# Boese0601/RC-MVSNet

Measured on AMD Instinct MI355X. Metric: ref-scenes/sec (DTU 3-view 512x640, D=48/32/8), higher is better.
Workload: dtype f32; 1 GPU; BASELINE configs[1]: CascadeMVSNet_eval.forward, DTU-shaped 3 views 512x640, D=(48,32,8), batch 1 per GPU, fp32, random-init seeded weights; views=3, height=512, width=640, parallelism=scene-per-gpu x1, ranks=1, procs_per_gpu=1, rccl_ranks=0

## Files before the change

rc_mvsnet_amd/_lib.py:

```python
import ast
import ctypes
import os
import re
import subprocess

_HERE = os.path.dirname(os.path.abspath(__file__))
LIB_PATH = os.path.join(_HERE, "librcmvs_hip.so")
CSRC = os.path.join(_HERE, "csrc")
HEADER = os.path.join(os.path.dirname(_HERE), "include", "rcmvs.h")
EXT_HEADERS = (os.path.join(CSRC, "pc_register.h"), os.path.join(CSRC, "view_select.h"), os.path.join(CSRC, "undistort.h"),
               os.path.join(CSRC, "tsdf_mesh.h"), os.path.join(CSRC, "tsdf_sparse.h"), os.path.join(CSRC, "mesh_clean.h"),
               os.path.join(CSRC, "mesh_decimate.h"), os.path.join(CSRC, "mesh_holes.h"),
               os.path.join(CSRC, "mesh_render.h"))

_lib = None


class RcmvsError(RuntimeError):
    pass


_CTYPES = {"int": ctypes.c_int, "float": ctypes.c_float, "double": ctypes.c_double, "long long": ctypes.c_longlong}


def _const_expr(text):
    def ev(node):
        if isinstance(node, ast.Constant) and type(node.value) is int:
            return node.value
        if isinstance(node, ast.BinOp) and isinstance(node.op, ast.LShift):
            return ev(node.left) << ev(node.right)
        raise ValueError(text)
    return ev(ast.parse(text.strip(), mode="eval").body)


def _ctype(decl, what, c_type):
    if c_type not in _CTYPES:
        raise RcmvsError(f"{HEADER}: `{decl}`: {what} type `{c_type}` is outside the ABI's types ({', '.join(_CTYPES)}, pointers)")
    return _CTYPES[c_type]


def parse_header(text):
    text = re.sub(r"/\*.*?\*/|//[^\n]*", " ", text, flags=re.S)
    signatures, restypes, constants, code = {}, {}, {}, []
    for line in text.splitlines():
        if not line.lstrip().startswith("#"):
            code.append(line)
            continue
        m = re.match(r"\s*#\s*define\s+(RCMVS_\w+)\s+(\S.*)", line)
        if m:
            try:
                value = _const_expr(m.group(2))
            except (ValueError, SyntaxError):
                raise RcmvsError(f"{HEADER}: `{line.strip()}`: not an integer expression of literals, << and parentheses") from None
            if m.group(1) in constants:
                raise RcmvsError(f"{HEADER}: {m.group(1)} is defined twice")
            constants[m.group(1)] = value
    for decl in re.sub(r'extern\s+"C"\s*\{', " ", "\n".join(code)).split(";"):
        decl = " ".join(decl.split())
        if "rcmvs_" not in decl:
            continue
        m = re.fullmatch(r"([\w\s*]+?)\s*\b(rcmvs_\w+)\s*\(([^()]*)\)", decl)
        if not m:
            raise RcmvsError(f"{HEADER}: `{decl}` is not a complete `<type> rcmvs_name(<parameters>);` declaration")
        ret, name, params = m.group(1), m.group(2), m.group(3).strip()
        if name in signatures:
            raise RcmvsError(f"{HEADER}: {name} is declared twice")
        if ret.replace("const", "").replace(" ", "") == "char*":
            restypes[name] = ctypes.c_char_p
        elif ret != "int":
            restypes[name] = _ctype(decl, "return", ret)
        argtypes = []
        for param in ([] if params == "void" else params.split(",")):
            if "*" in param:
                argtypes.append(ctypes.c_void_p)
                continue
            words = [w for w in param.split() if w != "const"]
            if len(words) < 2 or not words[-1].isidentifier():
                raise RcmvsError(f"{HEADER}: `{decl}`: parameter `{param.strip()}` is not `<type> <name>`")
            argtypes.append(_ctype(decl, "parameter", " ".join(words[:-1])))
        signatures[name] = argtypes
    return signatures, restypes, constants


def _read_header():
    try:
        with open(HEADER) as f:
            return f.read()
    except FileNotFoundError:
        raise RcmvsError(f"{HEADER} is missing: the ctypes binding is derived from the C header, which was expected there "
                         "(include/rcmvs.h next to the rc_mvsnet_amd package)") from None


SIGNATURES, _RESTYPES, CONSTANTS = parse_header(_read_header())
REQUIRED_VERSION = CONSTANTS["RCMVS_VERSION"]


def _read_extensions():
    signatures, restypes = {}, {}
    for path in EXT_HEADERS:
        try:
            with open(path) as f:
                sig, res, const = parse_header(f.read())
        except FileNotFoundError:
            raise RcmvsError(f"{path} is missing: the binding of its entry points is derived from it") from None
        for table, add in ((signatures, sig), (CONSTANTS, const)):
            clash = [k for k in add if k in table or k in SIGNATURES]
            if clash:
                raise RcmvsError(f"{path}: {clash[0]} is already declared")
            table.update(add)
        restypes.update(res)
    return signatures, restypes


EXT_SIGNATURES, _EXT_RESTYPES = _read_extensions()


def sources():
    return sorted(os.path.join(CSRC, f) for f in os.listdir(CSRC) if f.endswith(".hip"))


def build(force=False, verbose=False):
    from concurrent.futures import ThreadPoolExecutor
    srcs = sources()
    hdrs = [os.path.join(CSRC, f) for f in os.listdir(CSRC) if f.endswith(".h")] + [HEADER]
    if not force and os.path.exists(LIB_PATH) and all(os.path.getmtime(LIB_PATH) >= os.path.getmtime(d) for d in srcs + hdrs):
        return LIB_PATH
    hipcc = os.environ.get("HIPCC", "/opt/rocm/bin/hipcc")
    objdir = os.path.join(_HERE, "_obj")
    os.makedirs(objdir, exist_ok=True)
    hdr_time = max(os.path.getmtime(h) for h in hdrs)
    jobs, objs = [], []
    for src in srcs:
        obj = os.path.join(objdir, os.path.basename(src)[:-4] + ".o")
        objs.append(obj)
        if force or not os.path.exists(obj) or os.path.getmtime(obj) < max(os.path.getmtime(src), hdr_time):
            jobs.append([hipcc, "--offload-arch=gfx950", "-O3", "-std=c++17", "-fPIC", "-c", src, "-o", obj])

    def run(cmd):
        if verbose:
            print(" ".join(cmd), flush=True)
        subprocess.run(cmd, check=True)

    with ThreadPoolExecutor(max_workers=min(8, os.cpu_count() or 1)) as ex:
        list(ex.map(run, jobs))
    run([hipcc, "--offload-arch=gfx950", "-shared", "-fPIC", "-o", LIB_PATH] + objs)
    return LIB_PATH


def bind(lib):
    for table, restypes in ((SIGNATURES, _RESTYPES), (EXT_SIGNATURES, _EXT_RESTYPES)):
        for name, argtypes in table.items():
            fn = getattr(lib, name)
            fn.argtypes = argtypes
            fn.restype = restypes.get(name, ctypes.c_int)


def load():
    global _lib
    if _lib is not None:
        return _lib
    path = os.environ.get("RCMVS_LIB") or LIB_PATH
    if not os.path.exists(path):
        raise RcmvsError(f"{path} is missing: run `python -c 'import __graft_entry__ as g; g.build()'` "
                         "(hipcc --offload-arch=gfx950). There is no CPU / eager fallback.")
    lib = ctypes.CDLL(path)
    bind(lib)
    if lib.rcmvs_version() < REQUIRED_VERSION:
        raise RcmvsError(f"librcmvs_hip.so (version {lib.rcmvs_version()}) is older than this package needs ({REQUIRED_VERSION}): rebuild it")
    _lib = lib
    return lib


def check(rc, what):
    if rc != 0:
        msg = load().rcmvs_last_error_string()
        raise RcmvsError(f"{what} failed (rc={rc}): {msg.decode() if msg else ''}")


def call(name, *args):
    rc = getattr(_lib or load(), name)(*args)
    if rc:
        check(rc, name[len("rcmvs_"):])
```

rc_mvsnet_amd/casmvsnet.py:

```python
import os

FP16_PAIR_DEFAULT = True
ONE_BY_ONE_MFMA = os.environ.get("RCMVS_1X1_MFMA", "1") != "0"
HEAD_PAIR = os.environ.get("RCMVS_HEAD_PAIR", "1") != "0"
CONV11_PROB = int(os.environ.get("RCMVS_CONV11_PROB", "1"))
CONV_TILE = os.environ.get("RCMVS_CONV_TILE", "1") != "0"
CONV_STEM = os.environ.get("RCMVS_CONV_STEM", "1") != "0"
CONV_PAIR = os.environ.get("RCMVS_CONV_PAIR", "1") != "0"
DEEP_PAIR = os.environ.get("RCMVS_DEEP_PAIR", "1") != "0"

import torch
import torch.nn as nn
import torch.nn.functional as F

from . import ops
from ._lib import RcmvsError


def _nhwc(x):
    x = x.contiguous().float()
    return ops.rgb_to_nhwc4(x) if x.shape[1] == 3 else ops.to_channels_last(x)


def _param(mod, name):
    p = mod._parameters.get(name)
    return p if p is not None else getattr(mod, name)


def _packed_of(module, make):
    w = module.conv.weight
    key = (w.data_ptr(), w._version, str(w.device))
    c = module.__dict__.get("_rcmvs_pack")
    if c is None or c[0] != key:
        c = module.__dict__["_rcmvs_pack"] = (key, make(w.detach()))
    return c[1]


def _affine_of(m):
    if getattr(m, "gn", None) is not None:
        raise RcmvsError(f"{type(m).__name__}: GroupNorm blocks are not provided (the reference builds every block with norm='batch_norm')")
    if m.bn is not None:
        return _bn_fold(m.bn)
    b = m.conv.bias
    if b is None:
        return None, None
    return torch.ones_like(b, dtype=torch.float32), b.detach().float().contiguous()


def _same2(v, n):
    return tuple(v) == (n, n)


def _conv2d_block_cl(m, t):
    conv = m.conv
    K = conv.kernel_size[0]
    st = conv.stride[0]
    if (not _same2(conv.kernel_size, K) or K not in (1, 3, 5) or not _same2(conv.padding, K // 2) or not _same2(conv.stride, st)
            or st not in (1, 2) or not _same2(conv.dilation, 1) or conv.groups != 1 or conv.padding_mode != "zeros"):
        raise RcmvsError(f"Conv2d: only square 1x1 / 3x3 / 5x5 kernels with 'same' zero padding, stride 1 or 2, no dilation or groups "
                         f"(the layers of models/modules.py) run on the HIP path; got {conv}")
    scale, shift = _affine_of(m)
    relu = bool(m.relu)
    if K == 5 or conv.in_channels == 3:
        pw = _packed_of(m, lambda w: ops.pack_conv2d_weight(w, pad_in_to=4 if w.shape[1] == 3 else None))
        return ops.conv2d(t, pw, scale, shift, stride=st, relu=relu)
    pw = _packed_of(m, lambda w: ops.pack_conv3d_weight(FeatureNet._w3(w)))
    return ops.conv3d(t.unsqueeze(1), pw, scale, shift, stride=st, relu=relu).squeeze(1)


def _deconv2d_block_cl(m, t):
    conv = m.conv
    if (not _same2(conv.kernel_size, 3) or not _same2(conv.stride, 2) or not _same2(conv.padding, 1) or not _same2(conv.output_padding, 1)
            or not _same2(conv.dilation, 1) or conv.groups != 1):
        raise RcmvsError(f"Deconv2d: only kernel 3, stride 2, padding 1, output_padding 1 (DeConv2dFuse, models/modules.py:346) runs on the "
                         f"HIP path; got {conv}")
    if m.bn is None:
        raise RcmvsError("Deconv2d: bn=False is not provided (the reference's forward returns its INPUT in that case, models/modules.py:106-110)")
    scale, shift = _bn_fold(m.bn)
    pw = _packed_of(m, lambda w: ops.pack_conv3d_weight(F.pad(w.unsqueeze(2), (0, 0, 0, 0, 1, 1)), transposed=True))
    return ops.deconv3d(t.unsqueeze(1), pw, scale, shift, relu=bool(m.relu))[:, 0]


class Conv2d(nn.Module):
    def __init__(self, in_channels, out_channels, kernel_size, stride=1, relu=True, bn=True, bn_momentum=0.1,
                 init_method="xavier", **kwargs):
        super().__init__()
        self.conv = nn.Conv2d(in_channels, out_channels, kernel_size, stride=stride, bias=(not bn), **kwargs)
        self.kernel_size = kernel_size
        self.stride = stride
        self.bn = nn.BatchNorm2d(out_channels, momentum=bn_momentum) if bn else None
        self.relu = relu

    def forward(self, x):
        if _hip_inference(self, x):
            return ops.to_channels_first(_conv2d_block_cl(self, _nhwc(x)).contiguous())
        _unsupported(self, x)


class Deconv2d(nn.Module):

    def __init__(self, in_channels, out_channels, kernel_size, stride=1, relu=True, bn=True, bn_momentum=0.1,
                 init_method="xavier", **kwargs):
        super().__init__()
        assert stride in [1, 2]
        self.out_channels = out_channels
        self.stride = stride
        self.conv = nn.ConvTranspose2d(in_channels, out_channels, kernel_size, stride=stride, bias=(not bn), **kwargs)
        self.bn = nn.BatchNorm2d(out_channels, momentum=bn_momentum) if bn else None
        self.relu = relu

    def forward(self, x):
        if _hip_inference(self, x):
            return ops.to_channels_first(_deconv2d_block_cl(self, _nhwc(x)).contiguous())
        _unsupported(self, x)


class DeConv2dFuse(nn.Module):

    def __init__(self, in_channels, out_channels, kernel_size, relu=True, bn=True, bn_momentum=0.1):
        super().__init__()
        self.deconv = Deconv2d(in_channels, out_channels, kernel_size, stride=2, padding=1, output_padding=1, bn=True, relu=relu,
                               bn_momentum=bn_momentum)
        self.conv = Conv2d(2 * out_channels, out_channels, kernel_size, stride=1, padding=1, bn=bn, relu=relu, bn_momentum=bn_momentum)

    def forward_cl(self, x_pre, x):
        up = _deconv2d_block_cl(self.deconv, x)
        if up.shape != x_pre.shape:
            raise RcmvsError(f"DeConv2dFuse: the skip map {tuple(x_pre.shape)} is not twice the size of the up-sampled one {tuple(up.shape)}")
        return _conv2d_block_cl(self.conv, torch.cat((up, x_pre), dim=-1))

    def forward(self, x_pre, x):
        if _hip_inference(self, x_pre, x):
            return ops.to_channels_first(self.forward_cl(_nhwc(x_pre), _nhwc(x)).contiguous())
        _unsupported(self, x_pre, x)


class FeatureNet(nn.Module):

    def __init__(self, base_channels, num_stage=3, stride=4, arch_mode="fpn"):
        super().__init__()
        if arch_mode not in ("unet", "fpn"):
            raise ValueError("mode must be in 'unet' or 'fpn', but get:{}".format(arch_mode))
        if num_stage not in (1, 2, 3):
            raise ValueError("num_stage must be 1, 2 or 3")
        self.arch_mode = arch_mode
        self.stride = stride
        self.base_channels = base_channels
        self.num_stage = num_stage
        b = base_channels
        self.conv0 = nn.Sequential(Conv2d(3, b, 3, 1, padding=1), Conv2d(b, b, 3, 1, padding=1))
        self.conv1 = nn.Sequential(Conv2d(b, b * 2, 5, stride=2, padding=2), Conv2d(b * 2, b * 2, 3, 1, padding=1),
                                   Conv2d(b * 2, b * 2, 3, 1, padding=1))
        self.conv2 = nn.Sequential(Conv2d(b * 2, b * 4, 5, stride=2, padding=2), Conv2d(b * 4, b * 4, 3, 1, padding=1),
                                   Conv2d(b * 4, b * 4, 3, 1, padding=1))
        self.out1 = nn.Conv2d(b * 4, b * 4, 1, bias=False)
        self.out_channels = [4 * b]
        final_chs = b * 4
        if arch_mode == "unet":
            if num_stage >= 2:
                self.deconv1 = DeConv2dFuse(b * 4, b * 2, 3)
                self.out2 = nn.Conv2d(b * 2, b * 2, 1, bias=False)
                self.out_channels.append(2 * b)
            if num_stage == 3:
                self.deconv2 = DeConv2dFuse(b * 2, b, 3)
                self.out3 = nn.Conv2d(b, b, 1, bias=False)
                self.out_channels.append(b)
        elif num_stage == 3:
            self.inner1 = nn.Conv2d(b * 2, final_chs, 1, bias=True)
            self.inner2 = nn.Conv2d(b * 1, final_chs, 1, bias=True)
            self.out2 = nn.Conv2d(final_chs, b * 2, 3, padding=1, bias=False)
            self.out3 = nn.Conv2d(final_chs, b, 3, padding=1, bias=False)
            self.out_channels += [b * 2, b]
        elif num_stage == 2:
            self.inner1 = nn.Conv2d(b * 2, final_chs, 1, bias=True)
            self.out2 = nn.Conv2d(final_chs, b, 3, padding=1, bias=False)
            self.out_channels.append(b)

    def hip_plan(self):
        sub = self._modules
        mods = [m for seq in ("conv0", "conv1", "conv2") for m in sub[seq]._modules.values()]
        tens = []
        for m in mods:
            cv, bn = m._modules["conv"], m._modules["bn"]
            bb = bn._buffers
            tens += [_param(cv, "weight"), _param(bn, "weight"), _param(bn, "bias"), bb["running_mean"], bb["running_var"], bb["num_batches_tracked"]]
        unet = self.arch_mode == "unet"
        heads = ["out1"] + (["out2", "out3"] if unet else ["inner1", "out2", "inner2", "out3"])
        extra = [t for n in heads if n in sub for t in (_param(sub[n], "weight"), getattr(sub[n], "bias", None)) if t is not None]
        key = tuple((t.data_ptr(), t._version) for t in tens + extra)
        if getattr(self, "_plan", None) is None or key != self._plan_key:
            plan = {}
            names = ["conv0.0", "conv0.1", "conv1.0", "conv1.1", "conv1.2", "conv2.0", "conv2.1", "conv2.2"]
            for n, m in zip(names, mods):
                pad_to = 4 if m.conv.in_channels == 3 else None
                w = m.conv.weight
                if tuple(w.shape) in ((8, 8, 3, 3), (16, 16, 3, 3), (32, 32, 3, 3)) and m.stride == 1:
                    w3 = w.detach().new_zeros(w.shape[0], w.shape[1], 3, 3, 3)
                    w3[:, :, 1] = w.detach()
                    plan[n] = ("mfma3d", ops.pack_conv3d_weight(w3)) + _bn_fold(m.bn)
                    continue
                if tuple(w.shape) in ((32, 16, 5, 5), (16, 8, 5, 5)) and m.stride == 2:
                    w3 = self._w3(self._w5s2(w.detach())).contiguous()
                    plan[n] = ("s2d_mfma3d", ops.pack_conv3d_weight(w3)) + _bn_fold(m.bn)
                    continue
                plan[n] = (ops.pack_conv2d_weight(w, pad_in_to=pad_to),) + _bn_fold(m.bn) + (m.stride,)
            m11, m12 = mods[3], mods[4]
            if CONV_PAIR and all(tuple(m.conv.weight.shape) == (16, 16, 3, 3) and m.stride == 1 for m in (m11, m12)):
                plan["pair1"] = (ops.pack_conv2d_pair(m11.conv.weight, m12.conv.weight),) + _bn_fold(m11.bn) + _bn_fold(m12.bn)
            m00, m01 = mods[0], mods[1]
            if CONV_STEM and tuple(m00.conv.weight.shape) == (8, 3, 3, 3) and tuple(m01.conv.weight.shape) == (8, 8, 3, 3) and m00.stride == 1 and m01.stride == 1:
                plan["stem"] = (plan["conv0.0"][0],) + _bn_fold(m00.bn) + (ops.pack_conv2d_stem(m01.conv.weight),) + _bn_fold(m01.bn)
            m10 = mods[2]
            if CONV_TILE and tuple(m10.conv.weight.shape) == (16, 8, 5, 5) and m10.stride == 2:
                plan["tile10"] = (ops.pack_conv2d_tile(self._w5s2(m10.conv.weight.detach()).contiguous()),) + _bn_fold(m10.bn)
            for n, m in (("conv2.1", mods[6]), ("conv2.2", mods[7])):
                if CONV_TILE and tuple(m.conv.weight.shape) == (32, 32, 3, 3) and m.stride == 1:
                    plan["tile:" + n] = (ops.pack_conv2d_tile(m.conv.weight),) + _bn_fold(m.bn)
            plan["out1"] = ops.pack_conv2d_weight(self.out1.weight)
            if unet:
                for n in ("out2", "out3")[:self.num_stage - 1]:
                    plan[n] = ops.pack_conv3d_weight(self._w3(getattr(self, n).weight.detach()))
            elif self.num_stage >= 2:
                plan["inner1"] = (ops.pack_conv2d_weight(self.inner1.weight), self.inner1.bias.detach().float().contiguous())
                if tuple(self.out2.weight.shape) == (16, 32, 3, 3):
                    w3 = self.out2.weight.detach().new_zeros(16, 32, 3, 3, 3)
                    w3[:, :, 1] = self.out2.weight.detach()
                    plan["out2"] = ("mfma3d", ops.pack_conv3d_weight(w3))
                    if CONV_TILE:
                        plan["out2t"] = ops.pack_conv2d_tile(self.out2.weight)
                else:
                    plan["out2"] = ops.pack_conv2d_weight(self.out2.weight)
            if self.num_stage == 3 and not unet:
                plan["inner2"] = (ops.pack_conv2d_weight(self.inner2.weight), self.inner2.bias.detach().float().contiguous())
                plan["out3"] = ops.pack_conv2d_weight(self.out3.weight)
                plan["fuse_out3"] = tuple(self.inner2.weight.shape[:2]) == (32, 8) and tuple(self.out3.weight.shape[:2]) == (8, 32)
                if plan["fuse_out3"]:
                    plan["fold_out3"] = ops.pack_fpn_folded(self.inner2.weight, self.inner2.bias, self.out3.weight)
                    if os.environ.get("RCMVS_FPN_MFMA", "1") != "0":
                        plan["fold_out3"] = ops.pack_fpn_folded_mfma(plan["fold_out3"])
            self._plan, self._plan_key = plan, key
        return self._plan

    def forward_cl(self, x, lazy=False):
        p = self.hip_plan()

        def cbr(t, n):
            if "tile:" + n in p and not ops._CONV_IMPL:
                img, sc, sh = p["tile:" + n]
                return ops.conv2d_tile(t, img, sc, sh, relu=True)
            if p[n][0] == "mfma3d":
                _, w3, sc, sh = p[n]
                return ops.conv3d(t.unsqueeze(1), w3, sc, sh, relu=True).squeeze(1)
            if p[n][0] == "s2d_mfma3d":
                if t.shape[1] % 2 or t.shape[2] % 2:
                    raise RcmvsError(f"FeatureNet: image height and width must be multiples of 4 (got a {t.shape[1]}x{t.shape[2]} map "
                                     "at the second stride-2 layer), as the reference's three-level pyramid requires")
                _, w3, sc, sh = p[n]
                if ops._CONV_IMPL:
                    return ops.conv3d(self._s2d(t).contiguous().unsqueeze(1), w3, sc, sh, relu=True).squeeze(1)
                return ops.conv2d_s2d(t, w3, sc, sh, relu=True)
            w, sc, sh, stride = p[n]
            return ops.conv2d(t, w, sc, sh, stride=stride, relu=True)

        w00 = p["conv0.0"][0] if len(p["conv0.0"]) == 4 else None
        if "stem" in p and not ops._CONV_IMPL:
            c0 = ops.conv2d_stem(x.contiguous().float(), *p["stem"])
        else:
            c0 = None
        if c0 is not None:
            pass
        elif w00 is not None and w00.ci == 4 and w00.co == 8 and w00.k == 3 and p["conv0.0"][3] == 1 and not ops._CONV_IMPL:
            w, sc, sh, _ = p["conv0.0"]
            c0 = cbr(ops.conv2d_rgb(x.contiguous().float(), w, sc, sh, relu=True), "conv0.1")
        else:
            c0 = cbr(cbr(ops.rgb_to_nhwc4(x.contiguous().float()), "conv0.0"), "conv0.1")
        if "tile10" in p and not ops._CONV_IMPL and c0.shape[1] % 2 == 0 and c0.shape[2] % 2 == 0:
            c10 = ops.conv2d_tile(c0, p["tile10"][0], p["tile10"][1], p["tile10"][2], relu=True, s2d=True)
        else:
            c10 = cbr(c0, "conv1.0")
        if "pair1" in p and not ops._CONV_IMPL:
            c1 = ops.conv2d_pair(c10, *p["pair1"])
        else:
            c1 = cbr(cbr(c10, "conv1.1"), "conv1.2")
        c2 = cbr(cbr(cbr(c1, "conv2.0"), "conv2.1"), "conv2.2")
        def out1(bound=None, t=c2):
            if tuple(self.out1.weight.shape) == (32, 32, 1, 1) and (bound is not None or ONE_BY_ONE_MFMA):
                return ops.conv1x1(t, p["out1"], ysq_absmax=bound, mfma=ONE_BY_ONE_MFMA), bound is not None
            return ops.conv2d(t, p["out1"]), False
        out = {"stage1": out1}
        plain = lambda f: (lambda bound=None: (f(), False))
        if self.arch_mode == "unet":
            one = lambda t, n: ops.conv3d(t.unsqueeze(1), p[n]).squeeze(1)
            if self.num_stage >= 2:
                intra = self.deconv1.forward_cl(c1, c2)
                out["stage2"] = plain(lambda t=intra: one(t, "out2"))
            if self.num_stage == 3:
                intra = self.deconv2.forward_cl(c0, intra)
                out["stage3"] = plain(lambda t=intra: one(t, "out3"))
            return out if lazy else {k: f()[0] for k, f in out.items()}
        if self.num_stage >= 2:
            intra = ops.conv2d(c1, p["inner1"][0], None, p["inner1"][1], up_add=c2)
            if isinstance(p["out2"], tuple):
                def out2(bound=None, t=intra):
                    keep = bound is not None and not ops._CONV_IMPL
                    if "out2t" in p and not ops._CONV_IMPL:
                        return ops.conv2d_tile(t, p["out2t"], ysq_absmax=bound), keep
                    return ops.conv3d(t.unsqueeze(1), p["out2"][1], y_absmax=bound if keep else None, y_absmax_square=keep).squeeze(1), keep
                out["stage2"] = out2
            else:
                out["stage2"] = plain(lambda t=intra: ops.conv2d(t, p["out2"]))
        if self.num_stage == 3:
            if p.get("fuse_out3") and c0.shape[1] % 2 == 0 and c0.shape[2] % 2 == 0:
                if p.get("fold_out3") is not None:
                    out["stage3"] = (lambda bound=None, a=c0, b=intra: (ops.fpn_out_folded(a, b, p["fold_out3"], ysq_absmax=bound), bound is not None))
                else:
                    out["stage3"] = plain(lambda a=c0, b=intra: ops.fpn_out_fused(a, b, p["inner2"][0], p["inner2"][1], p["out3"]))
            else:
                intra = ops.conv2d(c0, p["inner2"][0], None, p["inner2"][1], up_add=intra)
                out["stage3"] = plain(lambda t=intra: ops.conv2d(t, p["out3"]))
        return out if lazy else {k: f()[0] for k, f in out.items()}

    @staticmethod
    def _w3(w):
        p = (3 - w.shape[-1]) // 2
        return F.pad(w.unsqueeze(2), (p, p, p, p, 1, 1))

    @staticmethod
    def _w5s2(w):
        Co, Ci = w.shape[:2]
        w6 = F.pad(w, (0, 1, 0, 1))
        return w6.reshape(Co, Ci, 3, 2, 3, 2).permute(0, 3, 5, 1, 2, 4).reshape(Co, 4 * Ci, 3, 3)

    @staticmethod
    def _s2d(x):
        N, H, W, C = x.shape
        return x.reshape(N, H // 2, 2, W // 2, 2, C).permute(0, 1, 3, 2, 4, 5).reshape(N, H // 2, W // 2, 4 * C)

    def forward_train_cl(self, x, segments=1):
        from .train_ops import ConvPlainFn, conv_bn_train_w
        if self.arch_mode != "fpn":
            raise RcmvsError("FeatureNet(arch_mode='unet'): the train-mode HIP path covers the shipped 'fpn' pyramid only (the one-plane form of "
                             "its transposed convs would put the discarded plane into the batch statistics)")
        N, _, H, W = x.shape
        if H % 4 or W % 4:
            raise RcmvsError("FeatureNet (training): image height and width must be multiples of 4")
        t = F.pad(x.permute(0, 2, 3, 1), (0, 5)).contiguous()

        def cbr(t, m):
            w = m.conv.weight
            if m.stride == 2:
                t, w = self._s2d(t), self._w5s2(w)
            return conv_bn_train_w(self._w3(w), m.bn, t.unsqueeze(1), relu=True, segments=segments).squeeze(1)

        def plain(t, conv):
            return ConvPlainFn.apply(t.unsqueeze(1), self._w3(conv.weight), conv.bias).squeeze(1)

        def up2(t):
            return t.repeat_interleave(2, dim=1).repeat_interleave(2, dim=2)

        c0 = t
        for m in self.conv0: c0 = cbr(c0, m)
        c1 = c0
        for m in self.conv1: c1 = cbr(c1, m)
        c2 = c1
        for m in self.conv2: c2 = cbr(c2, m)
        out = {"stage1": plain(c2, self.out1)}
        intra = c2
        if self.num_stage >= 2:
            intra = up2(intra) + plain(c1, self.inner1)
            out["stage2"] = plain(intra, self.out2)
        if self.num_stage == 3:
            intra = up2(intra) + plain(c0, self.inner2)
            out["stage3"] = plain(intra, self.out3)
        return out

    def forward(self, x):
        if _hip_inference(self, x):
            return {k: ops.to_channels_first(v) for k, v in self.forward_cl(x).items()}
        if _hip_training(self, x):
            return {k: v.permute(0, 3, 1, 2) for k, v in self.forward_train_cl(x).items()}
        _unsupported(self, x)


class Conv3d(nn.Module):
    def __init__(self, in_channels, out_channels, kernel_size=3, stride=1, relu=True, bn=True, bn_momentum=0.1, **kwargs):
        super().__init__()
        assert stride in [1, 2]
        self.out_channels = out_channels
        self.kernel_size = kernel_size
        self.stride = stride
        self.conv = nn.Conv3d(in_channels, out_channels, kernel_size, stride=stride, bias=(not bn), **kwargs)
        self.bn = nn.BatchNorm3d(out_channels, momentum=bn_momentum)
        self.gn = None
        self.relu = relu

    def forward(self, x):
        return _block3d(self, x)


class Deconv3d(nn.Module):
    def __init__(self, in_channels, out_channels, kernel_size=3, stride=1, relu=True, bn=True, bn_momentum=0.1, **kwargs):
        super().__init__()
        assert stride in [1, 2]
        self.out_channels = out_channels
        self.stride = stride
        self.conv = nn.ConvTranspose3d(in_channels, out_channels, kernel_size, stride=stride, bias=(not bn), **kwargs)
        self.bn = nn.BatchNorm3d(out_channels, momentum=bn_momentum)
        self.gn = None
        self.relu = relu

    def forward(self, x):
        return _block3d(self, x)


def _block3d(m, x):
    conv = m.conv
    transposed = isinstance(conv, nn.ConvTranspose3d)
    ok = (_same3(conv.kernel_size, 3) and _same3(conv.padding, 1) and _same3(conv.dilation, 1) and conv.groups == 1
          and (_same3(conv.stride, 2) and _same3(conv.output_padding, 1) if transposed
               else conv.stride[0] in (1, 2) and _same3(conv.stride, conv.stride[0]) and conv.padding_mode == "zeros"))
    if not ok:
        raise RcmvsError(f"{type(m).__name__}: only kernel 3, padding 1 (transposed: stride 2, output_padding 1) -- the layers of "
                         f"CostRegNet, models/modules.py:473-487 -- run on the HIP path; got {conv}")
    if _hip_inference(m, x):
        scale, shift = _affine_of(m)
        pw = _packed_of(m, lambda w: ops.pack_conv3d_weight(w, transposed=transposed))
        t = ops.to_channels_last(x.contiguous().float())
        y = ops.deconv3d(t, pw, scale, shift, relu=bool(m.relu)) if transposed else ops.conv3d(t, pw, scale, shift, stride=conv.stride[0], relu=bool(m.relu))
        return ops.to_channels_first(y)
    if _hip_training(m, x):
        if m.bn is None or conv.bias is not None:
            raise RcmvsError(f"{type(m).__name__}: the train-mode HIP path is conv -> BatchNorm (batch statistics) -> [ReLU] without a bias")
        from .train_ops import conv_bn_relu_train
        return conv_bn_relu_train(m, x.float().permute(0, 2, 3, 4, 1).contiguous()).permute(0, 4, 1, 2, 3)
    _unsupported(m, x)


def _same3(v, n):
    return tuple(v) == (n, n, n)


def _bn_fold(bn):
    scale = bn.weight.detach() / torch.sqrt(bn.running_var + bn.eps)
    shift = bn.bias.detach() - bn.running_mean * scale
    return scale.float().contiguous(), shift.float().contiguous()


class CostRegNet(nn.Module):

    _LAYERS = ("conv0", "conv1", "conv2", "conv3", "conv4", "conv5", "conv6", "conv7", "conv9", "conv11")
    BOUND_ROWS = 11

    def __init__(self, in_channels, base_channels):
        super().__init__()
        b = base_channels
        self.conv0 = Conv3d(in_channels, b, padding=1)
        self.conv1 = Conv3d(b, b * 2, stride=2, padding=1)
        self.conv2 = Conv3d(b * 2, b * 2, padding=1)
        self.conv3 = Conv3d(b * 2, b * 4, stride=2, padding=1)
        self.conv4 = Conv3d(b * 4, b * 4, padding=1)
        self.conv5 = Conv3d(b * 4, b * 8, stride=2, padding=1)
        self.conv6 = Conv3d(b * 8, b * 8, padding=1)
        self.conv7 = Deconv3d(b * 8, b * 4, stride=2, padding=1, output_padding=1)
        self.conv9 = Deconv3d(b * 4, b * 2, stride=2, padding=1, output_padding=1)
        self.conv11 = Deconv3d(b * 2, b * 1, stride=2, padding=1, output_padding=1)
        self.prob = nn.Conv3d(b, 1, 3, stride=1, padding=1, bias=False)
        self._plan = None
        self._plan_key = None

    def _tensors(self):
        ts = []
        mods = self._modules
        for n in self._LAYERS:
            m = mods[n]._modules
            cv, bn = m["conv"], m["bn"]
            bb = bn._buffers
            ts += [_param(cv, "weight"), _param(bn, "weight"), _param(bn, "bias"), bb["running_mean"], bb["running_var"], bb["num_batches_tracked"]]
        ts.append(_param(mods["prob"], "weight"))
        return ts

    def hip_plan(self):
        key = tuple((t.data_ptr(), t._version) for t in self._tensors())
        if self._plan is None or key != self._plan_key:
            plan = {}
            for n in self._LAYERS:
                m = getattr(self, n)
                w = ops.pack_conv3d_weight(m.conv.weight, transposed=isinstance(m, Deconv3d))
                s, b = _bn_fold(m.bn)
                plan[n] = (w, s, b)
            plan["prob"] = ops.pack_conv3d_weight(self.prob.weight)
            plan["conv11_coef"] = self._conv11_bound_coef(plan["conv11"][1], plan["conv11"][2])
            self._plan, self._plan_key = plan, key
        return self._plan

    def _conv11_bound_coef(self, scale, shift):
        w = self.conv11.conv.weight.detach().float().abs().sum(0)
        taps = ([1], [0, 2])
        l1 = None
        for pd in range(2):
            for ph in range(2):
                for pw in range(2):
                    v = w[:, taps[pd]][:, :, taps[ph]][:, :, :, taps[pw]].sum((1, 2, 3))
                    l1 = v if l1 is None else torch.maximum(l1, v)
        c1 = (scale.abs() * l1).max() * (1.0 + 2.0 ** -10)
        c2 = shift.abs().max() * (1.0 + 2.0 ** -10)
        return torch.stack((c1, c2)).float().contiguous()

    def features_cl(self, x, x_absmax=None, plan=None, logits=False, planes=None):
        B, D, h, w, _ = x.shape
        if D % 8 or h % 8 or w % 8:
            raise RcmvsError(f"CostRegNet: volume {D}x{h}x{w} must be divisible by 8 in every axis "
                             "(three stride-2 levels with skip connections, models/modules.py:492-499)")
        p = self.hip_plan() if plan is None else plan
        if logits and (x_absmax is None or B != 1):
            raise RcmvsError("CostRegNet.features_cl(logits=True): the fused conv11 + prob pass is the fp16-pair form of a B = 1 scene")
        if x_absmax is None:
            conv0 = ops.conv3d(x, *p["conv0"], relu=True)
            conv2 = ops.conv3d(ops.conv3d(conv0, *p["conv1"], stride=2, relu=True), *p["conv2"], relu=True)
            conv4 = ops.conv3d(ops.conv3d(conv2, *p["conv3"], stride=2, relu=True), *p["conv4"], relu=True)
            t = ops.conv3d(ops.conv3d(conv4, *p["conv5"], stride=2, relu=True), *p["conv6"], relu=True)
            t = ops.deconv3d(t, *p["conv7"], residual=conv4, relu=True)
            t = ops.deconv3d(t, *p["conv9"], residual=conv2, relu=True)
            return ops.deconv3d(t, *p["conv11"], residual=conv0, relu=True)
        b = [x_absmax[i] for i in range(1, self.BOUND_ROWS)]
        x_absmax = x_absmax[0]
        conv0 = ops.conv3d(x, *p["conv0"], relu=True, x_absmax=x_absmax, y_absmax=b[0])
        conv1 = ops.conv3d(conv0, *p["conv1"], stride=2, relu=True, x_absmax=b[0], y_absmax=b[1])
        conv2 = ops.conv3d(conv1, *p["conv2"], relu=True, x_absmax=b[1], y_absmax=b[2])
        conv3 = ops.conv3d(conv2, *p["conv3"], stride=2, relu=True, x_absmax=b[2], y_absmax=b[3])
        if DEEP_PAIR:
            conv4 = ops.conv3d(conv3, *p["conv4"], relu=True, x_absmax=b[3], y_absmax=b[6])
            t = ops.conv3d(conv4, *p["conv5"], stride=2, relu=True, x_absmax=b[6], y_absmax=b[7])
            t = ops.conv3d(t, *p["conv6"], relu=True, x_absmax=b[7], y_absmax=b[8])
            t = ops.deconv3d(t, *p["conv7"], residual=conv4, relu=True, x_absmax=b[8], y_absmax=b[5])
        else:
            conv4 = ops.conv3d(conv3, *p["conv4"], relu=True, x_absmax=b[3])
            t = ops.conv3d(ops.conv3d(conv4, *p["conv5"], stride=2, relu=True), *p["conv6"], relu=True)
            t = ops.deconv3d(t, *p["conv7"], residual=conv4, relu=True, y_absmax=b[5])
        t = ops.deconv3d(t, *p["conv9"], residual=conv2, relu=True, x_absmax=b[5], y_absmax=b[4])
        if logits:
            return ops.conv11_prob(t, b[4], p["conv11"][0], p["conv11"][1], p["conv11"][2], conv0, b[0], p["conv11_coef"], p["prob"], planes=planes)
        return ops.deconv3d(t, *p["conv11"], residual=conv0, relu=True, x_absmax=b[4], y_absmax=b[9])

    def features_cl_train(self, x):
        from .train_ops import conv_bn_relu_train as blk
        B, D, h, w, _ = x.shape
        if D % 8 or h % 8 or w % 8:
            raise RcmvsError(f"CostRegNet: volume {D}x{h}x{w} must be divisible by 8 in every axis")
        conv0 = blk(self.conv0, x)
        conv2 = blk(self.conv2, blk(self.conv1, conv0))
        conv4 = blk(self.conv4, blk(self.conv3, conv2))
        t = blk(self.conv6, blk(self.conv5, conv4))
        t = blk(self.conv7, t, residual=conv4)
        t = blk(self.conv9, t, residual=conv2)
        return blk(self.conv11, t, residual=conv0)

    def forward(self, x):
        if _hip_inference(self, x):
            feat = self.features_cl(ops.to_channels_last(x.contiguous().float()))
            logits = ops.conv3d(feat, self.hip_plan()["prob"])
            return ops.to_channels_first(logits)
        _unsupported(self, x)


def _hip_inference(module, *tensors):
    return (not module.training) and (not torch.is_grad_enabled()) and all(t.is_cuda for t in tensors)


def _hip_training(module, *tensors):
    return module.training and all(t.is_cuda for t in tensors)


def _unsupported(module, *tensors):
    name = type(module).__name__
    if not all(t.is_cuda for t in tensors):
        raise RcmvsError(f"{name}: the HIP path needs its tensors on the GPU (there is no CPU / eager fallback)")
    raise RcmvsError(f"{name}: eval-mode forward with autograd enabled is not provided -- wrap inference in torch.no_grad(), "
                     "or put the module in train() mode for the differentiable HIP path")


def _holder_only(module):
    raise RcmvsError(f"{type(module).__name__} is a parameter holder: its conv / bn children are executed by the enclosing "
                     "network's HIP plan (Rendering_Consistency_Net.forward and its volume / MLP chains)")


class DepthNet(nn.Module):

    def __init__(self, train_variant):
        super().__init__()
        self.train_variant = train_variant

    def forward(self, features, proj_matrices, depth_values, num_depth, cost_regularization, imgs=None, pad=0, prob_volume_init=None):
        if pad != 0 or prob_volume_init is not None:
            raise RcmvsError("DepthNet: pad and prob_volume_init are not provided (no caller of the reference passes them)")
        V = len(features)
        B, C, h, w = features[0].shape
        D = int(num_depth)
        if proj_matrices.shape[1] != V:
            raise RcmvsError("DepthNet: different number of images and projection matrices")
        if tuple(depth_values.shape) != (B, D, h, w):
            raise RcmvsError(f"DepthNet: depth_values {tuple(depth_values.shape)} is not (B, num_depth, h, w) = {(B, D, h, w)}")
        dv = depth_values.float()
        d0 = dv[:, 0]
        delta = (dv[:, 1] - d0) if D > 1 else torch.zeros_like(d0)
        k = torch.arange(D, device=dv.device, dtype=torch.float32).view(1, D, 1, 1)
        if float((dv - (d0.unsqueeze(1) + k * delta.unsqueeze(1))).abs().max()) > 1e-5 * float(dv.abs().max()):
            raise RcmvsError("DepthNet: depth_values must be uniformly spaced along the depth axis at every pixel (d_0 + k * delta)")
        planes = torch.stack((d0, delta), dim=-1).contiguous()
        with torch.no_grad():
            rot, trans = ops.compose_homography(proj_matrices.contiguous().float())
            small_cl = None
            if self.train_variant:
                if imgs is None:
                    raise RcmvsError("DepthNet (train variant): imgs (B,V,3,H,W) are needed for volume_feature_no_ref")
                small_cl = ops.resize_rgb_cl(imgs.float().reshape(B * V, *imgs.shape[2:]).contiguous(), (h, w)).view(B, V, h, w, 3)
        if _hip_inference(self, *features, depth_values):
            f_cl = torch.stack([ops.to_channels_last(f.contiguous().float()) for f in features], dim=1)
            var = ops.warp_variance(f_cl, rot, trans, planes, D)
            x8 = cost_regularization.features_cl(var)
            depth, conf = ops.depth_head(x8, cost_regularization.hip_plan()["prob"], planes)
            out = {"depth": depth, "photometric_confidence": conf}
            if self.train_variant:
                out["volume_feature_no_ref"] = ops.warp_noref(f_cl, small_cl, rot, trans, planes, D, square_first=True)
            return out
        if _hip_training(self, *features, depth_values):
            from . import train_ops
            f_cl = torch.stack([f.float().permute(0, 2, 3, 1) for f in features], dim=1).contiguous()
            res = ops.WarpVarianceFn.apply(f_cl, rot, trans, planes, D, small_cl)
            var, noref = res if self.train_variant else (res, None)
            x8 = cost_regularization.features_cl_train(var)
            depth, conf = train_ops.ProbDepthHeadFn.apply(x8, cost_regularization.prob.weight, planes)
            out = {"depth": depth, "photometric_confidence": conf}
            if self.train_variant:
                out["volume_feature_no_ref"] = noref
            return out
        _unsupported(self, *features, depth_values)


class _CascadeBase(nn.Module):
    TRAIN_VARIANT = False

    def __init__(self, refine=False, ndepths=[48, 32, 8], depth_interals_ratio=[4, 2, 1], share_cr=False,
                 grad_method="detach", arch_mode="fpn", cr_base_chs=[8, 8, 8]):
        super().__init__()
        if refine:
            raise NotImplementedError("refine=True: the reference's RefineNet is not runnable (models/modules.py:511 calls F.cat)")
        self.refine = refine
        self.share_cr = share_cr
        self.ndepths = ndepths
        self.depth_interals_ratio = depth_interals_ratio
        self.grad_method = grad_method
        self.arch_mode = arch_mode
        self.cr_base_chs = cr_base_chs
        self.num_stage = len(ndepths)
        assert len(ndepths) == len(depth_interals_ratio)
        self.stage_infos = {"stage1": {"scale": 4.0}, "stage2": {"scale": 2.0}, "stage3": {"scale": 1.0}}
        self.feature = FeatureNet(base_channels=8, stride=4, num_stage=self.num_stage, arch_mode=self.arch_mode)
        if self.share_cr:
            self.cost_regularization = CostRegNet(in_channels=self.feature.out_channels, base_channels=8)
        else:
            self.cost_regularization = nn.ModuleList([CostRegNet(in_channels=self.feature.out_channels[i],
                                                                 base_channels=self.cr_base_chs[i])
                                                      for i in range(self.num_stage)])
        self.DepthNet = DepthNet(self.TRAIN_VARIANT)

    def _cr(self, s):
        return self.cost_regularization if self.share_cr else self.cost_regularization[s]

    def _forward_hip(self, imgs, proj_matrices, depth_values, features=None, homographies=None):
        B, V, _, H, W = imgs.shape
        imgs = imgs.float()
        depth_values = depth_values.contiguous().float()
        feats_cl = None
        if features is None:
            feats_cl = self.feature.forward_cl(imgs.reshape(B * V, 3, H, W), lazy=True)
        outputs = {}
        depth = None
        bounds = None
        need_fill = False
        pair = getattr(self, "fp16_pair", None)
        if pair is None:
            pair = FP16_PAIR_DEFAULT if os.environ.get("RCMVS_FP16_PAIR") is None else os.environ["RCMVS_FP16_PAIR"] == "1"
        if pair and B == 1:
            bounds = getattr(self, "_pair_bounds", None)
            if getattr(self, "_is_replica", False):
                bounds = torch.zeros(self.num_stage, CostRegNet.BOUND_ROWS, ops.ABSMAX_FLOATS, device=imgs.device, dtype=torch.float32)
            elif bounds is None or bounds.device != imgs.device:
                bounds = self._pair_bounds = torch.zeros(self.num_stage, CostRegNet.BOUND_ROWS, ops.ABSMAX_FLOATS, device=imgs.device, dtype=torch.float32)
            else:
                need_fill = True
        if homographies is None:
            if self.num_stage <= 4:
                rots, transs = ops.compose_homography_stages([proj_matrices["stage{}".format(k + 1)].contiguous().float() for k in range(self.num_stage)],
                                                             zero=bounds if need_fill else None)
                need_fill = False
            else:
                rt = [ops.compose_homography(proj_matrices["stage{}".format(k + 1)].contiguous().float()) for k in range(self.num_stage)]
                rots, transs = [r for r, _ in rt], [t for _, t in rt]
        if need_fill:
            bounds.zero_()
        for s in range(self.num_stage):
            key = "stage{}".format(s + 1)
            scale = int(self.stage_infos[key]["scale"])
            D = self.ndepths[s]
            bound_kept = False
            if feats_cl is not None:
                fk, bound_kept = feats_cl[key](bounds[s][0] if bounds is not None else None)
                h, w, C = fk.shape[1:]
                f_cl = fk.view(B, V, h, w, C)
            else:
                C, h, w = features[key].shape[1:]
                f_cl = ops.to_channels_last(features[key].contiguous()).view(B, V, h, w, C)
            if homographies is not None:
                rot, trans = homographies[key]
            else:
                rot, trans = rots[s], transs[s]
            planes = ops.hypothesis_planes(depth, depth_values, (H, W), scale, D, self.depth_interals_ratio[s])
            var = ops.warp_variance(f_cl, rot, trans, planes, D, uniform_planes=depth is None)
            cr = self._cr(s)
            vmax = None
            if bounds is not None:
                vmax = bounds[s]
                if not bound_kept:
                    ops.absmax(f_cl, square=True, out=vmax[0])
            plan = cr.hip_plan()
            if vmax is not None and HEAD_PAIR and (CONV11_PROB == 2 or (CONV11_PROB == 1 and D == 8)):
                depth, conf = cr.features_cl(var, vmax, plan, logits=True, planes=planes)
            else:
                x8 = cr.features_cl(var, vmax, plan)
                depth, conf = ops.depth_head(x8, plan["prob"], planes, x_absmax=vmax[CostRegNet.BOUND_ROWS - 1] if vmax is not None and HEAD_PAIR else None)
            out = {"depth": depth, "photometric_confidence": conf}
            if self.TRAIN_VARIANT:
                small_cl = ops.resize_rgb_cl(imgs.reshape(B * V, 3, H, W).contiguous(), (h, w)).view(B, V, h, w, 3)
                out["volume_feature_no_ref"] = ops.warp_noref(f_cl, small_cl, rot, trans, planes, D, square_first=True)
            outputs[key] = out
            outputs.update(out)
        return outputs

    def _forward_train_hip(self, imgs, proj_matrices, depth_values):
        from . import train_ops
        B, V, _, H, W = imgs.shape
        imgs = imgs.float()
        depth_values = depth_values.contiguous().float()
        fv = self.feature.forward_train_cl(imgs.transpose(0, 1).reshape(V * B, 3, H, W), segments=V)
        features = [{k: f[v * B:(v + 1) * B] for k, f in fv.items()} for v in range(V)]
        outputs = {}
        depth = None
        for s in range(self.num_stage):
            key = "stage{}".format(s + 1)
            scale = int(self.stage_infos[key]["scale"])
            D = self.ndepths[s]
            f_cl = torch.stack([f[key] for f in features], dim=1).contiguous()
            h, w = f_cl.shape[2:4]
            with torch.no_grad():
                rot, trans = ops.compose_homography(proj_matrices[key].contiguous().float())
                prev = depth.detach() if depth is not None else None
                planes = ops.hypothesis_planes(prev, depth_values, (H, W), scale, D, self.depth_interals_ratio[s])
                small_cl = None
                if self.TRAIN_VARIANT:
                    small_cl = ops.resize_rgb_cl(imgs.reshape(B * V, 3, H, W).contiguous(), (h, w)).view(B, V, h, w, 3)
            res = ops.WarpVarianceFn.apply(f_cl, rot, trans, planes, D, small_cl)
            var, noref = res if self.TRAIN_VARIANT else (res, None)
            cr = self._cr(s)
            x8 = cr.features_cl_train(var)
            prev_live = depth
            depth, conf = train_ops.ProbDepthHeadFn.apply(x8, cr.prob.weight, planes)
            if prev_live is not None and self.grad_method != "detach":
                up = F.interpolate(prev_live.unsqueeze(1), [H, W], mode="bilinear", align_corners=False)
                base = F.interpolate(up, [h, w], mode="bilinear", align_corners=False).squeeze(1)
                depth = depth + (base - base.detach())
            out = {"depth": depth, "photometric_confidence": conf}
            if self.TRAIN_VARIANT:
                out["volume_feature_no_ref"] = noref
            outputs[key] = out
            outputs.update(out)
        return outputs

    def _run(self, imgs, proj_matrices, depth_values):
        if _hip_inference(self, imgs, depth_values):
            return self._forward_hip(imgs, proj_matrices, depth_values)
        if _hip_training(self, imgs, depth_values):
            return self._forward_train_hip(imgs, proj_matrices, depth_values)
        _unsupported(self, imgs, depth_values)


class CascadeMVSNet_eval(_CascadeBase):
    TRAIN_VARIANT = False

    def forward(self, imgs, proj_matrices, depth_values):
        return self._run(imgs, proj_matrices, depth_values)


class CascadeMVSNet(_CascadeBase):
    TRAIN_VARIANT = True

    def forward(self, imgs, proj_matrices, depth_values):
        outputs = self._run(imgs, proj_matrices, depth_values)
        return outputs, outputs["stage1"]["volume_feature_no_ref"]
```

rc_mvsnet_amd/csrc/geometry.hip:

```cpp
#include "common.h"

namespace rcmvs {

char* err_buf() {
    static thread_local char buf[512] = {0};
    return buf;
}

int fail(int code, const char* fmt, ...) {
    va_list ap;
    va_start(ap, fmt);
    vsnprintf(err_buf(), 512, fmt, ap);
    va_end(ap);
    return code;
}

template <bool TO_LAST>
__global__ __launch_bounds__(256) void layout_kernel(const float* __restrict__ src, float* __restrict__ dst,
                                                      int C, long long S) {
    const int Q = C >> 2;
    const int n = blockIdx.y;
    long long t = (long long)blockIdx.x * blockDim.x + threadIdx.x;
    long long sblk = t / (64LL * Q);
    int r = (int)(t % (64LL * Q));
    int q = r / 64;
    long long s = sblk * 64 + (r % 64);
    if (s >= S) return;
    const float* pl = (TO_LAST ? src : dst) + (long long)n * C * S;
    if (TO_LAST) {
        float4 v;
        v.x = pl[(4LL * q + 0) * S + s];
        v.y = pl[(4LL * q + 1) * S + s];
        v.z = pl[(4LL * q + 2) * S + s];
        v.w = pl[(4LL * q + 3) * S + s];
        *reinterpret_cast<float4*>(dst + ((long long)n * S + s) * C + 4 * q) = v;
    } else {
        float4 v = *reinterpret_cast<const float4*>(src + ((long long)n * S + s) * C + 4 * q);
        float* o = dst + (long long)n * C * S;
        o[(4LL * q + 0) * S + s] = v.x;
        o[(4LL * q + 1) * S + s] = v.y;
        o[(4LL * q + 2) * S + s] = v.z;
        o[(4LL * q + 3) * S + s] = v.w;
    }
}

template <bool TO_LAST>
__global__ __launch_bounds__(256) void layout_scalar_kernel(const float* __restrict__ src, float* __restrict__ dst,
                                                             int C, long long S) {
    const int n = blockIdx.y;
    long long t = (long long)blockIdx.x * blockDim.x + threadIdx.x;
    if (t >= S * C) return;
    long long s = t / C;
    int c = (int)(t % C);
    long long planar = ((long long)n * C + c) * S + s, last = ((long long)n * S + s) * C + c;
    if (TO_LAST) dst[last] = src[planar]; else dst[planar] = src[last];
}

template <bool TO_LAST>
static int layout_launch(const float* src, float* dst, int N, int C, long long S, void* stream) {
    RCMVS_REQUIRE(src && dst && N > 0 && C > 0 && S > 0, "layout: bad arguments N=%d C=%d S=%lld", N, C, S);
    if (C % 4 == 0) {
        long long threads = cdiv(S, 64) * 64 * (C / 4);
        dim3 grid((unsigned)cdiv(threads, 256), N);
        hipLaunchKernelGGL(layout_kernel<TO_LAST>, grid, dim3(256), 0, as_stream(stream), src, dst, C, S);
    } else {
        dim3 grid((unsigned)cdiv(S * C, 256), N);
        hipLaunchKernelGGL(layout_scalar_kernel<TO_LAST>, grid, dim3(256), 0, as_stream(stream), src, dst, C, S);
    }
    return launch_status("layout");
}

__device__ static void fold_intrinsics(const float* p, double A[4][4]) {
    for (int i = 0; i < 3; ++i)
        for (int j = 0; j < 4; ++j) {
            double s = 0.0;
            for (int k = 0; k < 3; ++k) s += (double)p[16 + i * 4 + k] * (double)p[k * 4 + j];
            A[i][j] = s;
        }
    for (int j = 0; j < 4; ++j) A[3][j] = (double)p[12 + j];
}

struct ProjPtrs { const float* p[4]; };
__global__ void compose_homography_kernel(ProjPtrs pp, float* __restrict__ rot,
                                          float* __restrict__ trans, int B, int V, float* __restrict__ zero, int zero_n) {
    for (int i = (blockIdx.y * gridDim.x + blockIdx.x) * blockDim.x + threadIdx.x; i < zero_n; i += gridDim.x * gridDim.y * blockDim.x) zero[i] = 0.0f;
    int t = blockIdx.x * blockDim.x + threadIdx.x;
    if (t >= B * (V - 1)) return;
    const float* proj = pp.p[blockIdx.y];
    rot += (long long)blockIdx.y * B * (V - 1) * 9;
    trans += (long long)blockIdx.y * B * (V - 1) * 3;
    int b = t / (V - 1), v = 1 + t % (V - 1);
    double R[4][4], S[4][4], inv[4][4];
    fold_intrinsics(proj + ((long long)b * V + 0) * 32, R);
    fold_intrinsics(proj + ((long long)b * V + v) * 32, S);
    for (int i = 0; i < 4; ++i)
        for (int j = 0; j < 4; ++j) inv[i][j] = (i == j) ? 1.0 : 0.0;
    for (int c = 0; c < 4; ++c) {
        int piv = c;
        double best = fabs(R[c][c]);
        for (int r = c + 1; r < 4; ++r)
            if (fabs(R[r][c]) > best) { best = fabs(R[r][c]); piv = r; }
        if (piv != c)
            for (int j = 0; j < 4; ++j) {
                double t0 = R[c][j]; R[c][j] = R[piv][j]; R[piv][j] = t0;
                double t1 = inv[c][j]; inv[c][j] = inv[piv][j]; inv[piv][j] = t1;
            }
        double d = 1.0 / R[c][c];
        for (int j = 0; j < 4; ++j) { R[c][j] *= d; inv[c][j] *= d; }
        for (int r = 0; r < 4; ++r) {
            if (r == c) continue;
            double f = R[r][c];
            for (int j = 0; j < 4; ++j) { R[r][j] -= f * R[c][j]; inv[r][j] -= f * inv[c][j]; }
        }
    }
    float* ro = rot + (long long)t * 9;
    float* tr = trans + (long long)t * 3;
    for (int i = 0; i < 3; ++i) {
        for (int j = 0; j < 4; ++j) {
            double s = 0.0;
            for (int k = 0; k < 4; ++k) s += S[i][k] * inv[k][j];
            if (j < 3) ro[i * 3 + j] = (float)s; else tr[i] = (float)s;
        }
    }
}

__device__ static inline float ld_agent(const float* p) {
#if defined(__AMDGCN__)
    return __hip_atomic_load(p, __ATOMIC_RELAXED, __HIP_MEMORY_SCOPE_AGENT);
#else
    return *p;
#endif
}

__device__ static inline float bilinear_up(const float* __restrict__ p, int hp, int wp, float sh, float sw, int Y, int X) {
#pragma clang fp contract(off)
    float sy = sh * ((float)Y + 0.5f) - 0.5f;
    float sx = sw * ((float)X + 0.5f) - 0.5f;
    sy = sy < 0.f ? 0.f : sy;
    sx = sx < 0.f ? 0.f : sx;
    int y0 = (int)sy, x0 = (int)sx;
    y0 = y0 > hp - 1 ? hp - 1 : y0;
    x0 = x0 > wp - 1 ? wp - 1 : x0;
    int y1 = y0 + 1 > hp - 1 ? hp - 1 : y0 + 1;
    int x1 = x0 + 1 > wp - 1 ? wp - 1 : x0 + 1;
    float ly1 = sy - (float)y0, lx1 = sx - (float)x0;
    float ly0 = 1.0f - ly1, lx0 = 1.0f - lx1;
    float top = lx0 * ld_agent(p + y0 * wp + x0) + lx1 * ld_agent(p + y0 * wp + x1);
    float bot = lx0 * ld_agent(p + y1 * wp + x0) + lx1 * ld_agent(p + y1 * wp + x1);
    return ly0 * top + ly1 * bot;
}

__global__ __launch_bounds__(256) void planes_kernel(const float* __restrict__ prev, const float* __restrict__ dv,
                                                      float* __restrict__ planes, int hp, int wp, int H, int W,
                                                      int scale, int D, float ratio, int ND) {
#pragma clang fp contract(off)
    const int h = H / scale, w = W / scale;
    const int b = blockIdx.y;
    int t = blockIdx.x * blockDim.x + threadIdx.x;
    if (t >= h * w) return;
    int y = t / w, x = t % w;
    float d0, delta;
    if (prev == nullptr) {
        float lo = dv[(long long)b * ND], hi = dv[(long long)b * ND + ND - 1];
        d0 = lo;
        delta = (hi - lo) / (float)(D - 1);
    } else {
        double itv = ((double)dv[ND - 1] - (double)dv[0]) / (double)ND;
        float half = (float)((double)D / 2.0 * ((double)ratio * itv));
        const float* p = prev + (long long)b * hp * wp;
        float sh = (float)hp / (float)H, sw = (float)wp / (float)W;
        float fd = (float)(D - 1);
        if (scale == 1) {
            float c = bilinear_up(p, hp, wp, sh, sw, y, x);
            float cmin = c - half, cmax = c + half;
            d0 = cmin;
            delta = (cmax - cmin) / fd;
        } else {
            int Y0 = y * scale + scale / 2 - 1, X0 = x * scale + scale / 2 - 1;
            float mn[2][2], it[2][2];
            for (int j = 0; j < 2; ++j)
                for (int i = 0; i < 2; ++i) {
                    float c = bilinear_up(p, hp, wp, sh, sw, Y0 + j, X0 + i);
                    float cmin = c - half, cmax = c + half;
                    mn[j][i] = cmin;
                    it[j][i] = (cmax - cmin) / fd;
                }
            d0 = 0.5f * (0.5f * mn[0][0] + 0.5f * mn[0][1]) + 0.5f * (0.5f * mn[1][0] + 0.5f * mn[1][1]);
            delta = 0.5f * (0.5f * it[0][0] + 0.5f * it[0][1]) + 0.5f * (0.5f * it[1][0] + 0.5f * it[1][1]);
        }
    }
    float2 o = make_float2(d0, delta);
    reinterpret_cast<float2*>(planes)[(long long)b * h * w + t] = o;
}

}

using namespace rcmvs;

extern "C" {

int rcmvs_version(void) { return RCMVS_VERSION; }
const char* rcmvs_last_error_string(void) { return err_buf(); }

int rcmvs_nchw_to_nhwc(const float* src, float* dst, int N, int C, long long S, void* stream) {
    return layout_launch<true>(src, dst, N, C, S, stream);
}
int rcmvs_nhwc_to_nchw(const float* src, float* dst, int N, int C, long long S, void* stream) {
    return layout_launch<false>(src, dst, N, C, S, stream);
}

int rcmvs_compose_homography(const float* proj, float* rot, float* trans, int B, int V, void* stream) {
    RCMVS_REQUIRE(proj && rot && trans, "compose_homography: null pointer");
    RCMVS_REQUIRE(B > 0 && V >= 2 && V - 1 <= RCMVS_MAX_SRC_VIEWS, "compose_homography: B=%d V=%d", B, V);
    const int n = B * (V - 1);
    ProjPtrs pp{{proj, nullptr, nullptr, nullptr}};
    hipLaunchKernelGGL(compose_homography_kernel, dim3((n + 63) / 64), dim3(64), 0, as_stream(stream), pp, rot, trans, B, V, (float*)nullptr, 0);
    return launch_status("compose_homography");
}

int rcmvs_compose_homography_stages(const float* proj0, const float* proj1, const float* proj2, const float* proj3, int nstage,
                                    float* rot, float* trans, int B, int V, float* zero, long long zero_n, void* stream) {
    RCMVS_REQUIRE(zero_n >= 0 && zero_n < (1LL << 24) && (zero || zero_n == 0), "compose_homography_stages: bad side buffer (%lld floats)", zero_n);
    RCMVS_REQUIRE(rot && trans && nstage >= 1 && nstage <= 4, "compose_homography_stages: bad arguments (1..4 stages)");
    RCMVS_REQUIRE(B > 0 && V >= 2 && V - 1 <= RCMVS_MAX_SRC_VIEWS, "compose_homography_stages: B=%d V=%d", B, V);
    ProjPtrs pp{{proj0, proj1, proj2, proj3}};
    for (int s = 0; s < nstage; ++s) RCMVS_REQUIRE(pp.p[s], "compose_homography_stages: stage %d has no projection tensor", s);
    const int n = B * (V - 1);
    hipLaunchKernelGGL(compose_homography_kernel, dim3((n + 63) / 64, nstage), dim3(zero_n ? 256 : 64), 0, as_stream(stream), pp, rot, trans, B, V, zero, (int)zero_n);
    return launch_status("compose_homography_stages");
}

int rcmvs_hypothesis_planes(const float* prev_depth, const float* depth_values, float* planes,
                            int B, int hp, int wp, int H, int W, int scale,
                            int D, float ratio, int ND, void* stream) {
    RCMVS_REQUIRE(depth_values && planes, "hypothesis_planes: null pointer");
    RCMVS_REQUIRE(B > 0 && H > 0 && W > 0 && D >= 2 && ND >= 2, "hypothesis_planes: bad sizes");
    RCMVS_REQUIRE(scale == 1 || scale == 2 || scale == 4, "hypothesis_planes: scale must be 1, 2 or 4 (got %d)", scale);
    RCMVS_REQUIRE(H % scale == 0 && W % scale == 0, "hypothesis_planes: H,W must be multiples of scale");
    RCMVS_REQUIRE(prev_depth == nullptr || (hp > 0 && wp > 0), "hypothesis_planes: prev_depth needs hp,wp");
    int h = H / scale, w = W / scale;
    dim3 grid((h * w + 255) / 256, B);
    hipLaunchKernelGGL(planes_kernel, grid, dim3(256), 0, as_stream(stream), prev_depth, depth_values, planes,
                       hp, wp, H, W, scale, D, ratio, ND);
    return launch_status("hypothesis_planes");
}

}
```

rc_mvsnet_amd/csrc/k1_pp.h:

```cpp
#pragma once
#include "k1_taps.h"

namespace rcmvs {

template <int C, int DKB, int NVT, int NG = (NVT <= 4 ? NVT : 3)>
__global__ __launch_bounds__(256) void warp_variance_pp_kernel(
    const float* __restrict__ feats, const float* __restrict__ rot, const float* __restrict__ trans,
    const float* __restrict__ planes, float* __restrict__ var, int V, int D, int h, int w, int tiles_x) {
    constexpr int LPP = C / 4, PIX = 256 / LPP, TH = 4, TW = PIX / TH, TEXB = C * 4;
    constexpr int CPP = PIX * NVT;
    constexpr int NCH = (CPP + 255) / 256;
    constexpr int GROUPS = (CPP < 256) ? 256 / CPP : 1;
    constexpr int NGRP = NVT / NG;
    static_assert(NVT % NG == 0, "view groups must divide the view count");
    __shared__ __attribute__((aligned(16))) v4f rec_w[2][CPP];
    __shared__ int rec_g[2][CPP];
    const int b = blockIdx.z;
    const int k0 = blockIdx.y * DKB;
    const unsigned tile = xcd_remap(blockIdx.x, gridDim.x);
    const int tx0 = (tile % tiles_x) * TW, ty0 = (tile / tiles_x) * TH;
    const int hw = h * w;
    K1Geom g;
    g.w = w; g.h = h;
    g.wm1 = (float)(w - 1); g.hm1 = (float)(h - 1);
    g.half_w = g.wm1 / 2.0f; g.half_h = g.hm1 / 2.0f;
    g.r_half_w = rcp_nr(g.half_w); g.r_half_h = rcp_nr(g.half_h);
    const float* fb = feats + (long long)b * V * hw * C;
    __amdgpu_buffer_rsrc_t rsrc = __builtin_amdgcn_make_buffer_rsrc(const_cast<float*>(fb), (short)0, V * hw * TEXB, 0x00020000);
    const float* rotb = rot + (long long)b * (V - 1) * 9;
    const float* trb = trans + (long long)b * (V - 1) * 3;
    const int pa = threadIdx.x % PIX;
    const int xa = min(tx0 + pa % TW, w - 1), ya = min(ty0 + pa / TW, h - 1);
    const float2 pla = reinterpret_cast<const float2*>(planes)[(long long)b * hw + ya * w + xa];
    const int grp = threadIdx.x / CPP;
    float rx[NCH], ry[NCH], rz[NCH], t0[NCH], t1[NCH], t2[NCH];
    {
#pragma clang fp contract(off)
        const float fxa = (float)xa, fya = (float)ya;
#pragma unroll
        for (int j = 0; j < NCH; ++j) {
            const int c = (threadIdx.x % CPP) + 256 * j;
            const int va = min(c / PIX, NVT - 1);
            const float* r = rotb + va * 9;
            const float* t = trb + va * 3;
            rx[j] = (r[0] * fxa + r[1] * fya) + r[2];
            ry[j] = (r[3] * fxa + r[4] * fya) + r[5];
            rz[j] = (r[6] * fxa + r[7] * fya) + r[8];
            t0[j] = t[0]; t1[j] = t[1]; t2[j] = t[2];
        }
    }
    auto records = [&](int k, int buf) {
        if (CPP < 256 && (k % GROUPS) != grp) return;
#pragma unroll
        for (int j = 0; j < NCH; ++j) {
#pragma clang fp contract(off)
            const int c = (threadIdx.x % CPP) + 256 * j;
            if (CPP % 256 != 0 && CPP > 256 && c >= CPP) continue;
            const int va = c / PIX;
            const float d = pla.x + (float)(k0 + k) * pla.y;
            float ix, iy;
            k1_position(rx[j], ry[j], rz[j], t0[j], t1[j], t2[j], d, g, ix, iy);
            int xc, yc;
            v4f wt;
            bool live;
            k1_tap_fixed(ix, iy, g, xc, yc, wt, live);
            rec_w[buf][c] = wt;
            rec_g[buf][c] = (((va + 1) * h + yc) * w + xc) * TEXB;
        }
    };
    const int p = threadIdx.x / LPP;
    const int q4b = (threadIdx.x % LPP) * 16;
    const int x = tx0 + p % TW, y = ty0 + p / TW;
    const bool inside = (x < w) && (y < h);
    const v4f ref = *reinterpret_cast<const v4f*>(fb + ((long long)min(y, h - 1) * w + min(x, w - 1)) * C + (q4b >> 2));
    const v4f ref2 = ref * ref;
    const float rV = rcp_nr((float)V);
    const long long pstride = (long long)hw * C;
    float* ob = var + (((long long)b * D + k0) * hw + (long long)min(y, h - 1) * w + min(x, w - 1)) * C + (q4b >> 2);
    const int pitch = w * TEXB;

    records(0, 0);
    __syncthreads();
#pragma unroll
    for (int k = 0; k < DKB; ++k) {
        v4f a = ref, a2 = ref2;
#pragma unroll
        for (int gi = 0; gi < NGRP; ++gi) {
            v4f tp[NG][4], wt[NG];
            if (inside) {
#pragma unroll
                for (int vg = 0; vg < NG; ++vg) {
                    const int va = gi * NG + vg;
                    const int o = rec_g[k & 1][va * PIX + p] + q4b;
                    wt[vg] = rec_w[k & 1][va * PIX + p];
                    tp[vg][0] = __builtin_bit_cast(v4f, __builtin_amdgcn_raw_buffer_load_b128(rsrc, o, 0, 0));
                    tp[vg][1] = __builtin_bit_cast(v4f, __builtin_amdgcn_raw_buffer_load_b128(rsrc, o + TEXB, 0, 0));
                    tp[vg][2] = __builtin_bit_cast(v4f, __builtin_amdgcn_raw_buffer_load_b128(rsrc, o, pitch, 0));
                    tp[vg][3] = __builtin_bit_cast(v4f, __builtin_amdgcn_raw_buffer_load_b128(rsrc, o + TEXB, pitch, 0));
                }
            }
            if (gi == 0 && k + 1 < DKB) records(k + 1, (k + 1) & 1);
            if (inside) {
#pragma unroll
                for (int vg = 0; vg < NG; ++vg) {
                    v4f val = tp[vg][0] * wt[vg].x;
                    val = __builtin_elementwise_fma(tp[vg][1], (v4f){wt[vg].y, wt[vg].y, wt[vg].y, wt[vg].y}, val);
                    val = __builtin_elementwise_fma(tp[vg][2], (v4f){wt[vg].z, wt[vg].z, wt[vg].z, wt[vg].z}, val);
                    val = __builtin_elementwise_fma(tp[vg][3], (v4f){wt[vg].w, wt[vg].w, wt[vg].w, wt[vg].w}, val);
                    a = a + val;
                    a2 = __builtin_elementwise_fma(val, val, a2);
                }
            }
        }
        if (inside && k0 + k < D) {
            const v4f m = a * rV;
            const v4f o = __builtin_elementwise_fma(a2, (v4f){rV, rV, rV, rV}, -(m * m));
            __builtin_nontemporal_store(o, reinterpret_cast<v4f*>(ob + k * pstride));
        }
        if (k + 1 < DKB) __syncthreads();
    }
}

template <int C, int DKB, int NVT>
static int k1_pp_launch_one(const float* feats, const float* rot, const float* trans, const float* planes, float* var,
                            int B, int V, int D, int h, int w, hipStream_t st, hipEvent_t ev0 = nullptr, hipEvent_t ev1 = nullptr) {
    constexpr int PIX = 256 / (C / 4), TW = PIX / 4;
    const int txp = (w + TW - 1) / TW, typ = (h + 3) / 4;
    dim3 grid(txp * typ, (D + DKB - 1) / DKB, B);
    RCMVS_LAUNCH_TIMED((warp_variance_pp_kernel<C, DKB, NVT>), grid, dim3(256), 0, st, ev0, ev1, feats, rot, trans, planes, var, V, D, h, w, txp);
    return launch_status("warp_variance_fwd (plane-pipelined form)");
}

}
```

rc_mvsnet_amd/csrc/k1_win.h:

```cpp
#pragma once
#include <atomic>
#include "k1_taps.h"

namespace rcmvs {

template <int C, int DKB, int NVT, int WP, int WR>
struct K1Win {
    static constexpr int LPP = C / 4;
    static constexpr int PIX = 256 / LPP;
    static constexpr int TH = 4, TW = PIX / TH;
    static constexpr int NREC = NVT * DKB * PIX;
    static constexpr int NCH = NREC / 256;
    static constexpr int TEXB = C * 4;
    static constexpr int WBYTES = WR * WP * TEXB;
    static constexpr int NLD = NVT * WBYTES / 1024;
    static constexpr int LPV = NLD / NVT;
    static constexpr int TPW = 1024 / TEXB;
    static constexpr int SEG = WP / TPW;
    static constexpr int OFF_W = 0;
    static constexpr int OFF_G = OFF_W + NREC * 16;
    static constexpr int OFF_L = OFF_G + NREC * 4;
    static constexpr int OFF_F = OFF_L + NREC * 4;
    static constexpr int OFF_WIN = (OFF_F + 16 + 8 * NVT + 1023) / 1024 * 1024;
    static constexpr int LDS_BYTES = OFF_WIN + NVT * WBYTES;
    static_assert(NREC % 256 == 0, "records must divide over the threads");
    static_assert(WBYTES % 1024 == 0 && LPV % 4 == 0, "the window loads of a view must divide over the four waves");
    static_assert(WP % TPW == 0, "a wave-load must stay inside one window row");
};

template <int C, int DKB, int NVT, int WP, int WR, int MODE>
__global__ __launch_bounds__(256) void warp_variance_win_kernel(
    const float* __restrict__ feats, const float* __restrict__ rot, const float* __restrict__ trans,
    const float* __restrict__ planes, float* __restrict__ var, int V, int D, int h, int w, int tiles_x, unsigned* __restrict__ stats) {
    using W = K1Win<C, DKB, NVT, WP, WR>;
    constexpr int LPP = W::LPP, PIX = W::PIX, TH = W::TH, TW = W::TW, TEXB = W::TEXB;
    extern __shared__ __attribute__((aligned(16))) char lds[];
    v4f* rec_w = reinterpret_cast<v4f*>(lds + W::OFF_W);
    int* rec_g = reinterpret_cast<int*>(lds + W::OFF_G);
    int* rec_l = reinterpret_cast<int*>(lds + W::OFF_L);
    int* fitf = reinterpret_cast<int*>(lds + W::OFF_F);
    int* orgf = fitf + 4;
    char* win = lds + W::OFF_WIN;
    const int b = blockIdx.z;
    const unsigned tile = xcd_remap(blockIdx.x, gridDim.x);
    const int tx0 = (tile % tiles_x) * TW, ty0 = (tile / tiles_x) * TH;
    const int hw = h * w;
    K1Geom g;
    g.w = w; g.h = h;
    g.wm1 = (float)(w - 1); g.hm1 = (float)(h - 1);
    g.half_w = g.wm1 / 2.0f; g.half_h = g.hm1 / 2.0f;
    g.r_half_w = rcp_nr(g.half_w); g.r_half_h = rcp_nr(g.half_h);
    const float* fb = feats + (long long)b * V * hw * C;
    __amdgpu_buffer_rsrc_t rsrc = __builtin_amdgcn_make_buffer_rsrc(const_cast<float*>(fb), (short)0, V * hw * TEXB, 0x00020000);
    const float* rotb = rot + (long long)b * (V - 1) * 9;
    const float* trb = trans + (long long)b * (V - 1) * 3;
    const int lane = threadIdx.x & 63;
    const int swave = __builtin_amdgcn_readfirstlane((int)(threadIdx.x >> 6));

    const int pa = threadIdx.x % PIX;
    const int xa = min(tx0 + pa % TW, w - 1), ya = min(ty0 + pa / TW, h - 1);
    const float2 pla = reinterpret_cast<const float2*>(planes)[(long long)b * hw + ya * w + xa];
    const int p = threadIdx.x / LPP;
    const int q4b = (threadIdx.x % LPP) * 16;
    const int x = tx0 + p % TW, y = ty0 + p / TW;
    const bool inside = (x < w) && (y < h);
    const v4f ref = *reinterpret_cast<const v4f*>(fb + ((long long)min(y, h - 1) * w + min(x, w - 1)) * C + (q4b >> 2));
    const v4f ref2 = ref * ref;
    const float rV = rcp_nr((float)V);
    const long long pstride = (long long)hw * C;
    float* ob = var + ((long long)b * D * hw + (long long)min(y, h - 1) * w + min(x, w - 1)) * C + (q4b >> 2);
    const int pitch = w * TEXB;
    const int xcen = min(tx0 + TW / 2, w - 1), ycen = min(ty0 + TH / 2, h - 1);
    const float fxc = (float)xcen, fyc = (float)ycen, fxa = (float)xa, fya = (float)ya;
    float2 plc = make_float2(0.f, 0.f);
    plc = reinterpret_cast<const float2*>(planes)[(long long)b * hw + ycen * w + xcen];

    struct Taps { v4f t[NVT][4]; v4f w[NVT]; };

    {
        const int k0 = blockIdx.y * DKB;
        int ox[NVT], oy[NVT];
        auto fill = [&]() {
            const int rw = (4 % W::SEG == 0) ? swave / W::SEG : 0, sw = (4 % W::SEG == 0) ? swave % W::SEG : 0;
#pragma unroll
            for (int j = 0; j < W::NLD / 4; ++j) {
                const int va = j / (W::LPV / 4), jj = j % (W::LPV / 4);
                int r, c0 = 0;
                if (4 % W::SEG == 0) r = rw + (4 / W::SEG) * jj;
                else { const int l = swave + 4 * jj; r = l / W::SEG; c0 = (l % W::SEG) * W::TPW; }
                const int L = va * W::LPV + swave + 4 * jj;
                const int yy = min(max(oy[va] + r, 0), h - 1);
                const int off = (((va + 1) * h + yy) * w + ox[va] + c0 + ((4 % W::SEG == 0) ? sw * W::TPW : 0)) * TEXB;
                __builtin_amdgcn_raw_ptr_buffer_load_lds(rsrc, win + L * 1024, 16, lane * 16 + off, 0, 0, 0);
            }
        };
        if (swave == 0) {
            const float dmid = plc.x + ((float)k0 + 0.5f * (float)(DKB - 1)) * plc.y;
#pragma unroll
            for (int va = 0; va < NVT; ++va) {
                const float* r = rotb + va * 9;
                const float* t = trb + va * 3;
                const float pz = fmaf(fmaf(r[6], fxc, fmaf(r[7], fyc, r[8])), dmid, t[2]);
                const float rp = __builtin_amdgcn_rcpf(pz);
                const float cx = fmaf(fmaf(r[0], fxc, fmaf(r[1], fyc, r[2])), dmid, t[0]) * rp;
                const float cy = fmaf(fmaf(r[3], fxc, fmaf(r[4], fyc, r[5])), dmid, t[1]) * rp;
                const float cxc = fminf(fmaxf(cx, -65536.0f), 65536.0f), cyc = fminf(fmaxf(cy, -65536.0f), 65536.0f);
                if (lane == 0) { orgf[2 * va] = (int)floorf(cxc) - (WP / 2 - 1); orgf[2 * va + 1] = (int)floorf(cyc) - (WR / 2 - 1); }
            }
        }
        __syncthreads();
#pragma unroll
        for (int va = 0; va < NVT; ++va) {
            ox[va] = __builtin_amdgcn_readfirstlane(orgf[2 * va]);
            oy[va] = __builtin_amdgcn_readfirstlane(orgf[2 * va + 1]);
        }
        if (MODE == 1) fill();

        bool all_fit = true;
#pragma unroll
        for (int j = 0; j < W::NCH; ++j) {
#pragma clang fp contract(off)
            const int c = threadIdx.x + 256 * j;
            const int ka = (c / PIX) % DKB, va = c / (PIX * DKB);
            const float* r = rotb + va * 9;
            const float* t = trb + va * 3;
            const float rx = (r[0] * fxa + r[1] * fya) + r[2];
            const float ry = (r[3] * fxa + r[4] * fya) + r[5];
            const float rz = (r[6] * fxa + r[7] * fya) + r[8];
            const float d = pla.x + (float)(k0 + ka) * pla.y;
            float ix, iy;
            k1_position(rx, ry, rz, t[0], t[1], t[2], d, g, ix, iy);
            int xc, yc;
            v4f wt;
            bool live;
            k1_tap_fixed(ix, iy, g, xc, yc, wt, live);
            rec_w[c] = wt;
            rec_g[c] = (((va + 1) * h + yc) * w + xc) * TEXB;
            {
                int oxv = ox[0], oyv = oy[0];
#pragma unroll
                for (int q = 1; q < NVT; ++q) if (va == q) { oxv = ox[q]; oyv = oy[q]; }
                const int lx = xc - oxv, ly = yc - oyv;
                const bool fits = ((unsigned)lx < (unsigned)(WP - 1)) && ((unsigned)ly < (unsigned)(WR - 1));
                rec_l[c] = va * W::WBYTES + ((live && fits) ? (ly * WP + lx) * TEXB : 0);
                all_fit = all_fit && (fits || !live);
            }
        }
        bool use_win = false;
        {
            const int wave_fit = __all(all_fit);
            if (lane == 0) fitf[swave] = wave_fit;
            if (MODE == 1) __builtin_amdgcn_s_waitcnt(0x0F70);
        }
        __syncthreads();
        {
            const v4i ff = *reinterpret_cast<const v4i*>(fitf);
            use_win = __builtin_amdgcn_readfirstlane((ff.x & ff.y & ff.z & ff.w) != 0);
            if (MODE == 2 && use_win) {
                fill();
                __builtin_amdgcn_s_waitcnt(0x0F70);
                __syncthreads();
            }
            if (stats && threadIdx.x == 0) { atomicAdd(stats, 1u); if (use_win) atomicAdd(stats + 1, 1u); }
        }

        if (inside) {
            auto blend_store = [&](const Taps& f, int k) {
                v4f a = ref, a2 = ref2;
#pragma unroll
                for (int va = 0; va < NVT; ++va) {
                    const v4f wt = f.w[va];
                    v4f val = f.t[va][0] * wt.x;
                    val = __builtin_elementwise_fma(f.t[va][1], (v4f){wt.y, wt.y, wt.y, wt.y}, val);
                    val = __builtin_elementwise_fma(f.t[va][2], (v4f){wt.z, wt.z, wt.z, wt.z}, val);
                    val = __builtin_elementwise_fma(f.t[va][3], (v4f){wt.w, wt.w, wt.w, wt.w}, val);
                    a = a + val;
                    a2 = __builtin_elementwise_fma(val, val, a2);
                }
                if (k0 + k < D) {
                    const v4f m = a * rV;
                    const v4f o = __builtin_elementwise_fma(a2, (v4f){rV, rV, rV, rV}, -(m * m));
                    __builtin_nontemporal_store(o, reinterpret_cast<v4f*>(ob + (k0 + k) * pstride));
                }
            };
            Taps f0, f1;
            if (use_win) {
                auto issue = [&](Taps& f, int k) {
#pragma unroll
                    for (int va = 0; va < NVT; ++va) {
                        const int idx = (va * DKB + k) * PIX + p;
                        const char* base = win + rec_l[idx] + q4b;
                        f.w[va] = rec_w[idx];
                        f.t[va][0] = *reinterpret_cast<const v4f*>(base);
                        f.t[va][1] = *reinterpret_cast<const v4f*>(base + TEXB);
                        f.t[va][2] = *reinterpret_cast<const v4f*>(base + WP * TEXB);
                        f.t[va][3] = *reinterpret_cast<const v4f*>(base + WP * TEXB + TEXB);
                    }
                };
                issue(f0, 0);
#pragma unroll
                for (int k = 0; k < DKB; ++k) {
                    Taps& cur = (k & 1) ? f1 : f0;
                    Taps& nxt = (k & 1) ? f0 : f1;
                    if (k + 1 < DKB) issue(nxt, k + 1);
                    blend_store(cur, k);
                }
            } else {
                auto issue = [&](Taps& f, int k) {
#pragma unroll
                    for (int va = 0; va < NVT; ++va) {
                        const int idx = (va * DKB + k) * PIX + p;
                        const int o = rec_g[idx] + q4b;
                        f.w[va] = rec_w[idx];
                        f.t[va][0] = __builtin_bit_cast(v4f, __builtin_amdgcn_raw_buffer_load_b128(rsrc, o, 0, 0));
                        f.t[va][1] = __builtin_bit_cast(v4f, __builtin_amdgcn_raw_buffer_load_b128(rsrc, o + TEXB, 0, 0));
                        f.t[va][2] = __builtin_bit_cast(v4f, __builtin_amdgcn_raw_buffer_load_b128(rsrc, o, pitch, 0));
                        f.t[va][3] = __builtin_bit_cast(v4f, __builtin_amdgcn_raw_buffer_load_b128(rsrc, o + TEXB, pitch, 0));
                    }
                };
                issue(f0, 0);
#pragma unroll
                for (int k = 0; k < DKB; ++k) {
                    Taps& cur = (k & 1) ? f1 : f0;
                    Taps& nxt = (k & 1) ? f0 : f1;
                    if (k + 1 < DKB) issue(nxt, k + 1);
                    blend_store(cur, k);
                }
            }
        }
    }
}

template <int C, int DKB, int NVT, int WP, int WR, int MODE>
static int k1_win_launch_one(const float* feats, const float* rot, const float* trans, const float* planes, float* var,
                             int B, int V, int D, int h, int w, unsigned* stats, hipStream_t st, hipEvent_t ev0 = nullptr, hipEvent_t ev1 = nullptr) {
    using W = K1Win<C, DKB, NVT, WP, WR>;
    const int txp = (w + W::TW - 1) / W::TW, typ = (h + W::TH - 1) / W::TH;
    dim3 grid(txp * typ, (D + DKB - 1) / DKB, B);
    const size_t lds = (size_t)W::LDS_BYTES;
    auto kern = warp_variance_win_kernel<C, DKB, NVT, WP, WR, MODE>;
    if (lds > 48 * 1024) {
        static std::atomic<bool> raised[64];
        int dev = 0;
        (void)hipGetDevice(&dev);
        if (dev >= 0 && dev < 64 && !raised[dev].load(std::memory_order_acquire)) {
            if (hipFuncSetAttribute(reinterpret_cast<const void*>(kern), hipFuncAttributeMaxDynamicSharedMemorySize, (int)lds) != hipSuccess)
                return fail(-1, "warp_variance_fwd (window form): cannot raise the dynamic LDS limit to %zu bytes", lds);
            raised[dev].store(true, std::memory_order_release);
        }
    }
    RCMVS_LAUNCH_TIMED(kern, grid, dim3(256), lds, st, ev0, ev1, feats, rot, trans, planes, var, V, D, h, w, txp, stats);
    return launch_status("warp_variance_fwd (window form)");
}

}
```

rc_mvsnet_amd/csrc/warp_variance.hip:

```cpp
#include <type_traits>
#include "common.h"
#include "k1_taps.h"
#include "k1_win.h"
#include "k1_pp.h"

namespace rcmvs {

constexpr int DK = 8;

struct WarpCoord {
    int off[4];
    float wgt[4];
};

__device__ __forceinline__ WarpCoord warp_taps(float rx, float ry, float rz, float tx, float ty, float tz,
                                               float d, float half_w, float half_h, float wm1, float hm1,
                                               int w, int h, int C) {
#pragma clang fp contract(off)
    float px = rx * d + tx;
    float py = ry * d + ty;
    float pz = rz * d + tz;
    float u = px / pz;
    float v = py / pz;
    float gx = u / half_w - 1.0f;
    float gy = v / half_h - 1.0f;
    float ix = ((gx + 1.0f) / 2.0f) * wm1;
    float iy = ((gy + 1.0f) / 2.0f) * hm1;
    float x0 = floorf(ix), y0 = floorf(iy);
    float x1 = x0 + 1.0f, y1 = y0 + 1.0f;
    float wx1 = ix - x0, wx0 = x1 - ix;
    float wy1 = iy - y0, wy0 = y1 - iy;
    bool vx0 = (x0 >= 0.0f) && (x0 <= wm1);
    bool vx1 = (x1 >= 0.0f) && (x1 <= wm1);
    bool vy0 = (y0 >= 0.0f) && (y0 <= hm1);
    bool vy1 = (y1 >= 0.0f) && (y1 <= hm1);
    int xi0 = (int)fminf(fmaxf(x0, 0.0f), wm1);
    int xi1 = (int)fminf(fmaxf(x1, 0.0f), wm1);
    int yi0 = (int)fminf(fmaxf(y0, 0.0f), hm1);
    int yi1 = (int)fminf(fmaxf(y1, 0.0f), hm1);
    WarpCoord t;
    t.off[0] = (yi0 * w + xi0) * C;
    t.off[1] = (yi0 * w + xi1) * C;
    t.off[2] = (yi1 * w + xi0) * C;
    t.off[3] = (yi1 * w + xi1) * C;
    t.wgt[0] = (vx0 && vy0) ? wx0 * wy0 : 0.0f;
    t.wgt[1] = (vx1 && vy0) ? wx1 * wy0 : 0.0f;
    t.wgt[2] = (vx0 && vy1) ? wx0 * wy1 : 0.0f;
    t.wgt[3] = (vx1 && vy1) ? wx1 * wy1 : 0.0f;
    return t;
}

__device__ __forceinline__ float4 bilerp4(const float* __restrict__ src, const WarpCoord& t, int q4) {
#pragma clang fp contract(off)
    float4 a = *reinterpret_cast<const float4*>(src + t.off[0] + q4);
    float4 b = *reinterpret_cast<const float4*>(src + t.off[1] + q4);
    float4 c = *reinterpret_cast<const float4*>(src + t.off[2] + q4);
    float4 d = *reinterpret_cast<const float4*>(src + t.off[3] + q4);
    float4 r;
    r.x = ((a.x * t.wgt[0] + b.x * t.wgt[1]) + c.x * t.wgt[2]) + d.x * t.wgt[3];
    r.y = ((a.y * t.wgt[0] + b.y * t.wgt[1]) + c.y * t.wgt[2]) + d.y * t.wgt[3];
    r.z = ((a.z * t.wgt[0] + b.z * t.wgt[1]) + c.z * t.wgt[2]) + d.z * t.wgt[3];
    r.w = ((a.w * t.wgt[0] + b.w * t.wgt[1]) + c.w * t.wgt[2]) + d.w * t.wgt[3];
    return r;
}

template <int C, bool STORE_ONLY>
__global__ __launch_bounds__(256) void warp_variance_ref_kernel(
    const float* __restrict__ feats, const float* __restrict__ rot, const float* __restrict__ trans,
    const float* __restrict__ planes, float* __restrict__ var, int V, int D, int h, int w, int tiles_x, int tiles_y) {
#pragma clang fp contract(off)
    constexpr int LPP = C / 4;
    constexpr int TW = 256 / C;
    constexpr int TH = 4;
    const int b = blockIdx.z;
    const int k0 = blockIdx.y * DK;
    const unsigned tile = xcd_remap(blockIdx.x, gridDim.x);
    const int tx = tile % tiles_x, ty = tile / tiles_x;
    const int q4 = (threadIdx.x % LPP) * 4;
    const int x = tx * TW + (threadIdx.x / LPP) % TW;
    const int y = ty * TH + threadIdx.x / (LPP * TW);
    if (x >= w || y >= h) return;
    const long long hw = (long long)h * w;
    const float fx = (float)x, fy = (float)y;
    const float wm1 = (float)(w - 1), hm1 = (float)(h - 1);
    const float half_w = wm1 / 2.0f, half_h = hm1 / 2.0f;
    const float2 pl = reinterpret_cast<const float2*>(planes)[(long long)b * hw + (long long)y * w + x];
    const float* fb = feats + (long long)b * V * hw * C;
    const float4 ref = *reinterpret_cast<const float4*>(fb + ((long long)y * w + x) * C + q4);
    float4 s[DK], sq[DK];
#pragma unroll
    for (int k = 0; k < DK; ++k) {
        s[k] = ref;
        sq[k] = make_float4(ref.x * ref.x, ref.y * ref.y, ref.z * ref.z, ref.w * ref.w);
    }
    for (int v = 1; v < V && !STORE_ONLY; ++v) {
        const float* r = rot + ((long long)b * (V - 1) + (v - 1)) * 9;
        const float* t = trans + ((long long)b * (V - 1) + (v - 1)) * 3;
        const float rx = (r[0] * fx + r[1] * fy) + r[2];
        const float ry = (r[3] * fx + r[4] * fy) + r[5];
        const float rz = (r[6] * fx + r[7] * fy) + r[8];
        const float t0 = t[0], t1 = t[1], t2 = t[2];
        const float* src = fb + (long long)v * hw * C;
#pragma unroll
        for (int k = 0; k < DK; ++k) {
            const float d = pl.x + (float)(k0 + k) * pl.y;
            WarpCoord tc = warp_taps(rx, ry, rz, t0, t1, t2, d, half_w, half_h, wm1, hm1, w, h, C);
            float4 val = bilerp4(src, tc, q4);
            s[k].x = s[k].x + val.x; s[k].y = s[k].y + val.y; s[k].z = s[k].z + val.z; s[k].w = s[k].w + val.w;
            sq[k].x = sq[k].x + val.x * val.x; sq[k].y = sq[k].y + val.y * val.y;
            sq[k].z = sq[k].z + val.z * val.z; sq[k].w = sq[k].w + val.w * val.w;
        }
    }
    const float fV = (float)V;
    float* ob = var + (((long long)b * D) * hw + (long long)y * w + x) * C + q4;
#pragma unroll
    for (int k = 0; k < DK; ++k) {
        if (k0 + k < D) {
            float4 m, o;
            if (STORE_ONLY) { o = s[k]; }
            else {
                m.x = s[k].x / fV; m.y = s[k].y / fV; m.z = s[k].z / fV; m.w = s[k].w / fV;
                o.x = sq[k].x / fV - m.x * m.x;
                o.y = sq[k].y / fV - m.y * m.y;
                o.z = sq[k].z / fV - m.z * m.z;
                o.w = sq[k].w / fV - m.w * m.w;
            }
            *reinterpret_cast<float4*>(ob + (long long)(k0 + k) * hw * C) = o;
        }
    }
}

template <bool FAST>
__device__ __forceinline__ v4f blend4(v4f a, v4f b, v4f c, v4f d, v4f wt) {
    if (FAST) {
        v4f r = a * wt.x;
        r = __builtin_elementwise_fma(b, (v4f){wt.y, wt.y, wt.y, wt.y}, r);
        r = __builtin_elementwise_fma(c, (v4f){wt.z, wt.z, wt.z, wt.z}, r);
        r = __builtin_elementwise_fma(d, (v4f){wt.w, wt.w, wt.w, wt.w}, r);
        return r;
    } else {
#pragma clang fp contract(off)
        return ((a * wt.x + b * wt.y) + c * wt.z) + d * wt.w;
    }
}

template <int NV>
struct K1Fetch {
    v4f t[NV][4];
    v4f w[NV];
};

template <int NV, int DKB, int PIX>
__device__ __forceinline__ void k1_issue(K1Fetch<NV>& f, const v4i* lds_o, const v4f* lds_w, __amdgpu_buffer_rsrc_t rsrc,
                                         int k, int p, int q4b, int v0 = 0) {
#pragma unroll
    for (int va = 0; va < NV; ++va) {
        const int idx = ((v0 + va) * DKB + k) * PIX + p;
        const v4i o = lds_o[idx];
        f.w[va] = lds_w[idx];
        f.t[va][0] = __builtin_bit_cast(v4f, __builtin_amdgcn_raw_buffer_load_b128(rsrc, o.x + q4b, 0, 0));
        f.t[va][1] = __builtin_bit_cast(v4f, __builtin_amdgcn_raw_buffer_load_b128(rsrc, o.y + q4b, 0, 0));
        f.t[va][2] = __builtin_bit_cast(v4f, __builtin_amdgcn_raw_buffer_load_b128(rsrc, o.z + q4b, 0, 0));
        f.t[va][3] = __builtin_bit_cast(v4f, __builtin_amdgcn_raw_buffer_load_b128(rsrc, o.w + q4b, 0, 0));
    }
}

template <bool FAST>
__device__ __forceinline__ void k1_store_variance(v4f a, v4f a2, float fV, float rV, float* dst) {
#pragma clang fp contract(off)
    v4f m, o;
    m.x = div_c<1>(a.x, fV, rV); m.y = div_c<1>(a.y, fV, rV); m.z = div_c<1>(a.z, fV, rV); m.w = div_c<1>(a.w, fV, rV);
    o.x = div_c<1>(a2.x, fV, rV) - m.x * m.x;
    o.y = div_c<1>(a2.y, fV, rV) - m.y * m.y;
    o.z = div_c<1>(a2.z, fV, rV) - m.z * m.z;
    o.w = div_c<1>(a2.w, fV, rV) - m.w * m.w;
    __builtin_nontemporal_store(o, reinterpret_cast<v4f*>(dst));
}

template <int C>
struct K1Tile {
    static constexpr int LPP = C / 4;
    static constexpr int PIX = 256 / LPP;
    static constexpr int TH = 4, TW = PIX / TH;
    static constexpr int GRP = 256 / PIX;
};

template <int C, int DKB>
__device__ __forceinline__ void k1_phase_a(const float* __restrict__ rot, const float* __restrict__ trans, int b, int V, int view, int slot,
                                           float fxa, float fya, float2 pla, int k0, int hw, const K1Geom& g, v4i* lds_o, v4f* lds_w) {
#pragma clang fp contract(off)
    constexpr int PIX = K1Tile<C>::PIX, GRP = K1Tile<C>::GRP, KPT = DKB / GRP;
    const int pa = threadIdx.x % PIX, ga = threadIdx.x / PIX;
    const float* r = rot + ((long long)b * (V - 1) + (view - 1)) * 9;
    const float* t = trans + ((long long)b * (V - 1) + (view - 1)) * 3;
    const float rx = (r[0] * fxa + r[1] * fya) + r[2];
    const float ry = (r[3] * fxa + r[4] * fya) + r[5];
    const float rz = (r[6] * fxa + r[7] * fya) + r[8];
    const float t0 = t[0], t1 = t[1], t2 = t[2];
    const int vrow = view * hw;
#pragma unroll
    for (int kk = 0; kk < KPT; ++kk) {
        const int ka = ga + kk * GRP;
        const float d = pla.x + (float)(k0 + ka) * pla.y;
        v4i o;
        v4f wt;
        k1_tap<C>(rx, ry, rz, t0, t1, t2, d, g, vrow, o, wt);
        const int idx = (slot * DKB + ka) * PIX + pa;
        lds_o[idx] = o;
        lds_w[idx] = wt;
    }
}

template <int C, int DKB, bool FAST, int NVT, int NG = (NVT > 4 ? 3 : NVT)>
__global__ __launch_bounds__(256) void warp_variance_tp_kernel(
    const float* __restrict__ feats, const float* __restrict__ rot, const float* __restrict__ trans,
    const float* __restrict__ planes, float* __restrict__ var, int V, int D, int h, int w, int tiles_x) {
#pragma clang fp contract(off)
    constexpr int LPP = K1Tile<C>::LPP, PIX = K1Tile<C>::PIX, TH = K1Tile<C>::TH, TW = K1Tile<C>::TW, GRP = K1Tile<C>::GRP;
    static_assert(NVT > 0 && DKB % GRP == 0, "DKB must be a multiple of 256/PIX");
    extern __shared__ __attribute__((aligned(16))) v4i lds_o[];
    v4f* lds_w = reinterpret_cast<v4f*>(lds_o + NVT * DKB * PIX);
    const int b = blockIdx.z;
    const int k0 = blockIdx.y * DKB;
    const unsigned tile = xcd_remap(blockIdx.x, gridDim.x);
    const int tx0 = (tile % tiles_x) * TW, ty0 = (tile / tiles_x) * TH;
    const int hw = h * w;
    K1Geom g;
    g.w = w; g.h = h;
    g.wm1 = (float)(w - 1); g.hm1 = (float)(h - 1);
    g.half_w = g.wm1 / 2.0f; g.half_h = g.hm1 / 2.0f;
    g.r_half_w = rcp_nr(g.half_w); g.r_half_h = rcp_nr(g.half_h);
    const float* fb = feats + (long long)b * V * hw * C;
    __amdgpu_buffer_rsrc_t rsrc = __builtin_amdgcn_make_buffer_rsrc(const_cast<float*>(fb), (short)0, 0x7fffffff, 0x00020000);
    const int p = threadIdx.x / LPP;
    const int q4b = (threadIdx.x % LPP) * 16;
    const int x = tx0 + p % TW, y = ty0 + p / TW;
    const bool inside = (x < w) && (y < h);
    v4f ref = (v4f){0.f, 0.f, 0.f, 0.f};
    if (inside) ref = *reinterpret_cast<const v4f*>(fb + ((long long)y * w + x) * C + (q4b >> 2));
    const float fV = (float)V, rV = rcp_nr(fV);
    float* ob = var + (((long long)b * D) * hw + (long long)y * w + x) * C + (q4b >> 2);
    {
        const int pa = threadIdx.x % PIX;
        const int xa = min(tx0 + pa % TW, w - 1), ya = min(ty0 + pa / TW, h - 1);
        const float2 pla = reinterpret_cast<const float2*>(planes)[(long long)b * hw + ya * w + xa];
        for (int va = 0; va < NVT; ++va)
            k1_phase_a<C, DKB>(rot, trans, b, V, 1 + va, va, (float)xa, (float)ya, pla, k0, hw, g, lds_o, lds_w);
    }
    __syncthreads();
    if (!inside) return;
    constexpr int NGRP = NVT / NG, NS = DKB * NGRP;
    static_assert(NVT % NG == 0, "view groups must divide the view count");
    K1Fetch<NG> f0, f1;
    k1_issue<NG, DKB, PIX>(f0, lds_o, lds_w, rsrc, 0, p, q4b, 0);
    v4f a = ref, a2 = ref * ref;
#pragma unroll
    for (int st = 0; st < NS; ++st) {
        const int k = st / NGRP, gi = st % NGRP;
        K1Fetch<NG>& cur = (st & 1) ? f1 : f0;
        K1Fetch<NG>& nxt = (st & 1) ? f0 : f1;
        if (st + 1 < NS) k1_issue<NG, DKB, PIX>(nxt, lds_o, lds_w, rsrc, (st + 1) / NGRP, p, q4b, ((st + 1) % NGRP) * NG);
        if (gi == 0) { a = ref; a2 = ref * ref; }
#pragma unroll
        for (int va = 0; va < NG; ++va) {
            v4f val = blend4<FAST>(cur.t[va][0], cur.t[va][1], cur.t[va][2], cur.t[va][3], cur.w[va]);
            a = a + val;
            if (FAST) a2 = __builtin_elementwise_fma(val, val, a2); else a2 = a2 + val * val;
        }
        if (gi == NGRP - 1 && k0 + k < D) k1_store_variance<FAST>(a, a2, fV, rV, ob + (long long)(k0 + k) * hw * C);
    }
}

template <int C, int DKB, bool FAST>
__global__ __launch_bounds__(256) void warp_variance_mv_kernel(
    const float* __restrict__ feats, const float* __restrict__ rot, const float* __restrict__ trans,
    const float* __restrict__ planes, float* __restrict__ var, int V, int D, int h, int w, int tiles_x, int VC) {
#pragma clang fp contract(off)
    constexpr int LPP = K1Tile<C>::LPP, PIX = K1Tile<C>::PIX, TH = K1Tile<C>::TH, TW = K1Tile<C>::TW, GRP = K1Tile<C>::GRP;
    static_assert(DKB % GRP == 0, "DKB must be a multiple of 256/PIX");
    extern __shared__ __attribute__((aligned(16))) v4i lds_o[];
    v4f* lds_w = reinterpret_cast<v4f*>(lds_o + VC * DKB * PIX);
    const int b = blockIdx.z;
    const int k0 = blockIdx.y * DKB;
    const unsigned tile = xcd_remap(blockIdx.x, gridDim.x);
    const int tx0 = (tile % tiles_x) * TW, ty0 = (tile / tiles_x) * TH;
    const int hw = h * w;
    K1Geom g;
    g.w = w; g.h = h;
    g.wm1 = (float)(w - 1); g.hm1 = (float)(h - 1);
    g.half_w = g.wm1 / 2.0f; g.half_h = g.hm1 / 2.0f;
    g.r_half_w = rcp_nr(g.half_w); g.r_half_h = rcp_nr(g.half_h);
    const float* fb = feats + (long long)b * V * hw * C;
    __amdgpu_buffer_rsrc_t rsrc = __builtin_amdgcn_make_buffer_rsrc(const_cast<float*>(fb), (short)0, 0x7fffffff, 0x00020000);
    const int p = threadIdx.x / LPP;
    const int q4b = (threadIdx.x % LPP) * 16;
    const int x = tx0 + p % TW, y = ty0 + p / TW;
    const bool inside = (x < w) && (y < h);
    v4f ref = (v4f){0.f, 0.f, 0.f, 0.f};
    if (inside) ref = *reinterpret_cast<const v4f*>(fb + ((long long)y * w + x) * C + (q4b >> 2));
    const float fV = (float)V, rV = rcp_nr(fV);
    float* ob = var + (((long long)b * D) * hw + (long long)y * w + x) * C + (q4b >> 2);
    const int pa = threadIdx.x % PIX;
    const int xa = min(tx0 + pa % TW, w - 1), ya = min(ty0 + pa / TW, h - 1);
    const float2 pla = reinterpret_cast<const float2*>(planes)[(long long)b * hw + ya * w + xa];
    v4f s[DKB], sq[DKB];
#pragma unroll
    for (int k = 0; k < DKB; ++k) { s[k] = ref; sq[k] = ref * ref; }
    for (int v0 = 1; v0 < V; v0 += VC) {
        const int nv = min(VC, V - v0);
        if (v0 > 1) __syncthreads();
        for (int va = 0; va < nv; ++va)
            k1_phase_a<C, DKB>(rot, trans, b, V, v0 + va, va, (float)xa, (float)ya, pla, k0, hw, g, lds_o, lds_w);
        __syncthreads();
        if (!inside) continue;
#pragma unroll
        for (int k = 0; k < DKB; ++k) {
            v4f a = s[k], a2 = sq[k];
            for (int va = 0; va < nv; ++va) {
                K1Fetch<1> f;
                k1_issue<1, DKB, PIX>(f, lds_o, lds_w, rsrc, k, p, q4b, va);
                v4f val = blend4<FAST>(f.t[0][0], f.t[0][1], f.t[0][2], f.t[0][3], f.w[0]);
                a = a + val;
                if (FAST) a2 = __builtin_elementwise_fma(val, val, a2); else a2 = a2 + val * val;
            }
            if (v0 + nv < V) { s[k] = a; sq[k] = a2; continue; }
            if (k0 + k < D) k1_store_variance<FAST>(a, a2, fV, rV, ob + (long long)(k0 + k) * hw * C);
        }
    }
}

template <int C>
__global__ __launch_bounds__(256) void warp_noref_kernel(
    const float* __restrict__ feats, const float* __restrict__ imgs, const float* __restrict__ rot,
    const float* __restrict__ trans, const float* __restrict__ planes, float* __restrict__ out,
    int V, int D, int h, int w, int square_first) {
#pragma clang fp contract(off)
    const int b = blockIdx.z, k = blockIdx.y;
    const long long hw = (long long)h * w;
    long long p = (long long)blockIdx.x * blockDim.x + threadIdx.x;
    if (p >= hw) return;
    const int y = (int)(p / w), x = (int)(p % w);
    const float fx = (float)x, fy = (float)y;
    const float wm1 = (float)(w - 1), hm1 = (float)(h - 1);
    const float half_w = wm1 / 2.0f, half_h = hm1 / 2.0f;
    const float2 pl = reinterpret_cast<const float2*>(planes)[(long long)b * hw + p];
    const float d = pl.x + (float)k * pl.y;
    const int CT = 3 * (V - 1) + C;
    float* ob = out + (((long long)b * CT) * D + k) * hw + p;
    const long long cs = (long long)D * hw;
    const float fV = (float)V;
    float s[C], sq[C];
#pragma unroll
    for (int c = 0; c < C; ++c) { s[c] = 0.0f; sq[c] = 0.0f; }
    for (int v = 1; v < V; ++v) {
        const float* r = rot + ((long long)b * (V - 1) + (v - 1)) * 9;
        const float* t = trans + ((long long)b * (V - 1) + (v - 1)) * 3;
        const float rx = (r[0] * fx + r[1] * fy) + r[2];
        const float ry = (r[3] * fx + r[4] * fy) + r[5];
        const float rz = (r[6] * fx + r[7] * fy) + r[8];
        const WarpCoord tc = warp_taps(rx, ry, rz, t[0], t[1], t[2], d, half_w, half_h, wm1, hm1, w, h, 1);
        const float* im = imgs + ((long long)b * V + v) * hw * 3;
        for (int c = 0; c < 3; ++c) {
            float val = ((im[tc.off[0] * 3 + c] * tc.wgt[0] + im[tc.off[1] * 3 + c] * tc.wgt[1]) +
                         im[tc.off[2] * 3 + c] * tc.wgt[2]) + im[tc.off[3] * 3 + c] * tc.wgt[3];
            ob[(long long)((v - 1) * 3 + c) * cs] = val;
        }
        const float* src = feats + ((long long)b * V + v) * hw * C;
        const float* s0 = src + (long long)tc.off[0] * C;
        const float* s1 = src + (long long)tc.off[1] * C;
        const float* s2 = src + (long long)tc.off[2] * C;
        const float* s3 = src + (long long)tc.off[3] * C;
#pragma unroll
        for (int c = 0; c < C; c += 4) {
            const float4 a = *reinterpret_cast<const float4*>(s0 + c), bb = *reinterpret_cast<const float4*>(s1 + c);
            const float4 cc = *reinterpret_cast<const float4*>(s2 + c), dd = *reinterpret_cast<const float4*>(s3 + c);
            float val[4];
            val[0] = ((a.x * tc.wgt[0] + bb.x * tc.wgt[1]) + cc.x * tc.wgt[2]) + dd.x * tc.wgt[3];
            val[1] = ((a.y * tc.wgt[0] + bb.y * tc.wgt[1]) + cc.y * tc.wgt[2]) + dd.y * tc.wgt[3];
            val[2] = ((a.z * tc.wgt[0] + bb.z * tc.wgt[1]) + cc.z * tc.wgt[2]) + dd.z * tc.wgt[3];
            val[3] = ((a.w * tc.wgt[0] + bb.w * tc.wgt[1]) + cc.w * tc.wgt[2]) + dd.w * tc.wgt[3];
#pragma unroll
            for (int j = 0; j < 4; ++j) {
                float vv = val[j];
                if (square_first) vv = vv * vv;
                s[c + j] = s[c + j] + vv;
                sq[c + j] = sq[c + j] + vv * vv;
            }
        }
    }
#pragma unroll
    for (int c = 0; c < C; ++c) {
        const float m = s[c] / fV;
        ob[(long long)(3 * (V - 1) + c) * cs] = sq[c] / fV - m * m;
    }
}

}

using namespace rcmvs;

extern "C" {

static int k1_launch(const float* feats, const float* rot, const float* trans, const float* planes, float* var,
                     int B, int V, int C, int D, int h, int w, int variant, hipStream_t st, unsigned* stats = nullptr,
                     hipEvent_t ev0 = nullptr, hipEvent_t ev1 = nullptr) {
    RCMVS_REQUIRE(feats && rot && trans && planes && var, "warp_variance_fwd: null pointer");
    RCMVS_REQUIRE(B > 0 && D > 0 && h > 1 && w > 1, "warp_variance_fwd: bad sizes B=%d D=%d h=%d w=%d", B, D, h, w);
    RCMVS_REQUIRE(V >= 2 && V - 1 <= RCMVS_MAX_SRC_VIEWS, "warp_variance_fwd: V=%d unsupported", V);
    RCMVS_REQUIRE((long long)h * w * C < (1LL << 31), "warp_variance_fwd: feature map too large for 32-bit offsets");
    RCMVS_REQUIRE((variant >= 0 && variant <= 3) || (variant >= 5 && variant <= 7), "warp_variance_fwd: unknown variant %d", variant);
    RCMVS_REQUIRE(C == 8 || C == 16 || C == 32, "warp_variance_fwd: C must be 8, 16 or 32 (got %d)", C);
    if (variant == 7) {
        const int nsrc = V - 1;
        RCMVS_REQUIRE(nsrc == 2 || nsrc == 3 || nsrc == 4 || nsrc == 6, "warp_variance_fwd: the plane-pipelined form is built for 2, 3, 4 or 6 source views (got V=%d)", V);
        RCMVS_REQUIRE((long long)V * h * w * C * 4 < 0x7fffffffLL, "warp_variance_fwd: feature block too large for 32-bit offsets");
#define RCMVS_K1PP(NN) do { \
            if (C == 32) return k1_pp_launch_one<32, 8, NN>(feats, rot, trans, planes, var, B, V, D, h, w, st, ev0, ev1); \
            if (C == 16) return k1_pp_launch_one<16, 8, NN>(feats, rot, trans, planes, var, B, V, D, h, w, st, ev0, ev1); \
            return k1_pp_launch_one<8, 8, NN>(feats, rot, trans, planes, var, B, V, D, h, w, st, ev0, ev1); } while (0)
        if (nsrc == 2) RCMVS_K1PP(2);
        if (nsrc == 3) RCMVS_K1PP(3);
        if (nsrc == 4) RCMVS_K1PP(4);
        RCMVS_K1PP(6);
#undef RCMVS_K1PP
    }
    if (variant >= 5) {
        RCMVS_REQUIRE(V == 3, "warp_variance_fwd: the window form is built for two source views (got V=%d)", V);
        RCMVS_REQUIRE((long long)V * h * w * C * 4 < 0x7fffffffLL, "warp_variance_fwd: feature block too large for 32-bit offsets");
#define RCMVS_K1WIN(CC, DD, PP, RR) (variant == 5 ? k1_win_launch_one<CC, DD, 2, PP, RR, 1>(feats, rot, trans, planes, var, B, V, D, h, w, stats, st, ev0, ev1) : \
                                                    k1_win_launch_one<CC, DD, 2, PP, RR, 2>(feats, rot, trans, planes, var, B, V, D, h, w, stats, st, ev0, ev1))
        if (C == 32) return RCMVS_K1WIN(32, 4, 16, 8);
        if (C == 16) return RCMVS_K1WIN(16, 4, 32, 8);
        return RCMVS_K1WIN(8, 4, 64, 8);
#undef RCMVS_K1WIN
    }
    if (variant <= 1) {
        const bool fastm = variant == 1;
        const int LPP = C / 4, PIX = 256 / LPP;
        const int nsrc = V - 1;
        const int nvt = (nsrc == 2 || nsrc == 4 || nsrc == 6) ? nsrc : 0;
        const int dkb = (nvt == 6) ? ((C == 8) ? 2 : (C == 16 ? 4 : 8)) : ((C == 8) ? 4 : 8);
        const size_t per_view = (size_t)32 * dkb * PIX;
        int VC = nvt ? nvt : (int)((48 * 1024) / per_view);
        if (VC > nsrc) VC = nsrc;
        const size_t lds = per_view * VC;
        const int TWp = PIX / 4;
        const int txp = (w + TWp - 1) / TWp, typ = (h + 3) / 4;
        RCMVS_REQUIRE((long long)V * h * w * C * 4 < 0x7fffffffLL, "warp_variance_fwd: feature block too large for 32-bit offsets");
        dim3 gridp(txp * typ, (D + dkb - 1) / dkb, B);
#define RCMVS_K1TP(CC, DD, FF, NN) RCMVS_LAUNCH_TIMED((warp_variance_tp_kernel<CC, DD, FF, NN>), gridp, dim3(256), lds, st, ev0, ev1, feats, rot, trans, planes, var, V, D, h, w, txp)
#define RCMVS_K1MV(CC, DD, FF) RCMVS_LAUNCH_TIMED((warp_variance_mv_kernel<CC, DD, FF>), gridp, dim3(256), lds, st, ev0, ev1, feats, rot, trans, planes, var, V, D, h, w, txp, VC)
#define RCMVS_K1TP_N(CC, DD, FF) do { if (nvt == 2) RCMVS_K1TP(CC, DD, FF, 2); else if (nvt == 4) RCMVS_K1TP(CC, DD, FF, 4); else RCMVS_K1MV(CC, DD, FF); } while (0)
#define RCMVS_K1TP_F(CC, DD) do { if (fastm) RCMVS_K1TP_N(CC, DD, true); else RCMVS_K1TP_N(CC, DD, false); } while (0)
#define RCMVS_K1TP_6(CC, DD) do { if (fastm) RCMVS_K1TP(CC, DD, true, 6); else RCMVS_K1TP(CC, DD, false, 6); } while (0)
        if (nvt == 6) {
            switch (C) {
                case 8:  RCMVS_K1TP_6(8, 2); break;
                case 16: RCMVS_K1TP_6(16, 4); break;
                case 32: RCMVS_K1TP_6(32, 8); break;
                default: return fail(-1, "warp_variance_fwd: C must be 8, 16 or 32 (got %d)", C);
            }
            return launch_status("warp_variance_fwd");
        }
        switch (C) {
            case 8:  RCMVS_K1TP_F(8, 4); break;
            case 16: RCMVS_K1TP_F(16, 8); break;
            case 32: RCMVS_K1TP_F(32, 8); break;
            default: return fail(-1, "warp_variance_fwd: C must be 8, 16 or 32 (got %d)", C);
        }
        return launch_status("warp_variance_fwd");
    }
    const int TW = 256 / C, TH = 4;
    const int tiles_x = (w + TW - 1) / TW, tiles_y = (h + TH - 1) / TH;
    dim3 grid(tiles_x * tiles_y, (D + DK - 1) / DK, B);
#define RCMVS_K1_LAUNCH(CC, VV) RCMVS_LAUNCH_TIMED((warp_variance_ref_kernel<CC, VV>), grid, dim3(256), 0, st, ev0, ev1, feats, rot, trans, planes, var, V, D, h, w, tiles_x, tiles_y)
#define RCMVS_K1_VARIANTS(CC) do { if (variant == 2) RCMVS_K1_LAUNCH(CC, false); else RCMVS_K1_LAUNCH(CC, true); } while (0)
    switch (C) {
        case 8:  RCMVS_K1_VARIANTS(8); break;
        case 16: RCMVS_K1_VARIANTS(16); break;
        case 32: RCMVS_K1_VARIANTS(32); break;
        default: return fail(-1, "warp_variance_fwd: C must be 8, 16 or 32 (got %d)", C);
    }
#undef RCMVS_K1_VARIANTS
#undef RCMVS_K1_LAUNCH
    return launch_status("warp_variance_fwd");
}

static int k1_production_variant(int V, int C, int h, int w, int hint) {
    const bool small = (long long)V * h * w * C * 4 < 0x7fffffffLL;
    const int nsrc = V - 1;
    if (!small || !(hint & RCMVS_K1_FAST_BLEND)) return 0;
    const bool uniform = (hint & RCMVS_K1_UNIFORM_PLANES) != 0;
    if (nsrc == 2) return uniform ? 5 : (C == 8 ? 7 : 0);
    if (nsrc == 3 || nsrc == 6) return 7;
    if (nsrc == 4) return (C == 16 && !uniform) ? 1 : 7;
    return 0;
}

int rcmvs_warp_variance_fwd(const float* feats, const float* rot, const float* trans,
                            const float* planes, float* var,
                            int B, int V, int C, int D, int h, int w, void* stream) {
    return k1_launch(feats, rot, trans, planes, var, B, V, C, D, h, w, 0, as_stream(stream));
}

int rcmvs_warp_variance_hint_fwd(const float* feats, const float* rot, const float* trans,
                                 const float* planes, float* var,
                                 int B, int V, int C, int D, int h, int w, int hint, void* stream) {
    return k1_launch(feats, rot, trans, planes, var, B, V, C, D, h, w, k1_production_variant(V, C, h, w, hint), as_stream(stream));
}

int rcmvs_warp_variance_timed_fwd(const float* feats, const float* rot, const float* trans,
                                  const float* planes, float* var,
                                  int B, int V, int C, int D, int h, int w, int hint, void* start_event, void* stop_event, void* stream) {
    return k1_launch(feats, rot, trans, planes, var, B, V, C, D, h, w, k1_production_variant(V, C, h, w, hint), as_stream(stream), nullptr,
                     reinterpret_cast<hipEvent_t>(start_event), reinterpret_cast<hipEvent_t>(stop_event));
}

int rcmvs_debug_warp_variance_fwd(const float* feats, const float* rot, const float* trans,
                                  const float* planes, float* var,
                                  int B, int V, int C, int D, int h, int w, int variant, void* stream) {
    return k1_launch(feats, rot, trans, planes, var, B, V, C, D, h, w, variant, as_stream(stream));
}

int rcmvs_debug_warp_variance_win_fwd(const float* feats, const float* rot, const float* trans,
                                      const float* planes, float* var,
                                      int B, int V, int C, int D, int h, int w, int variant, unsigned* stats, void* stream) {
    RCMVS_REQUIRE(variant == 5 || variant == 6, "debug_warp_variance_win_fwd: variant must be 5 or 6 (got %d)", variant);
    return k1_launch(feats, rot, trans, planes, var, B, V, C, D, h, w, variant, as_stream(stream), stats);
}

int rcmvs_warp_noref_fwd(const float* feats, const float* imgs, const float* rot, const float* trans,
                         const float* planes, float* out,
                         int B, int V, int C, int D, int h, int w, int square_first, void* stream) {
    RCMVS_REQUIRE(feats && imgs && rot && trans && planes && out, "warp_noref_fwd: null pointer");
    RCMVS_REQUIRE(B > 0 && D > 0 && h > 1 && w > 1, "warp_noref_fwd: bad sizes");
    RCMVS_REQUIRE(C == 8 || C == 16 || C == 32, "warp_noref_fwd: C must be 8, 16 or 32 (got %d)", C);
    RCMVS_REQUIRE(V >= 2 && V - 1 <= RCMVS_MAX_SRC_VIEWS, "warp_noref_fwd: V=%d unsupported", V);
    dim3 grid((unsigned)cdiv((long long)h * w, 256), D, B);
#define RCMVS_NOREF(CC) hipLaunchKernelGGL((warp_noref_kernel<CC>), grid, dim3(256), 0, as_stream(stream), feats, imgs, rot, trans, planes, out, V, D, h, w, square_first)
    if (C == 8) RCMVS_NOREF(8); else if (C == 16) RCMVS_NOREF(16); else RCMVS_NOREF(32);
#undef RCMVS_NOREF
    return launch_status("warp_noref_fwd");
}

}
```

rc_mvsnet_amd/ops.py:

```python
import ctypes
import os

import torch

from . import _lib

K1_EVENTS = None
K1_UNIFORM_PLANES = _lib.CONSTANTS["RCMVS_K1_UNIFORM_PLANES"]
K1_FAST_BLEND = _lib.CONSTANTS["RCMVS_K1_FAST_BLEND"]
CONV_EVENTS = None


_FIRST_STREAM = {}


def _multi_stream_allowed():
    return os.environ.get("GPU_MAX_HW_QUEUES") == "1" or os.environ.get("RCMVS_ALLOW_MULTI_STREAM") == "1"


def _stream():
    st = torch.cuda.current_stream()
    key = st.device_index
    first = _FIRST_STREAM.setdefault(key, st.cuda_stream)
    if first != st.cuda_stream and not _multi_stream_allowed():
        raise _lib.RcmvsError(
            f"rc_mvsnet_amd launches on ONE HIP stream per device and process: cuda:{key} started on stream {first:#x}, this call is on "
            f"{st.cuda_stream:#x}.  Two hardware queues of one process give silently wrong results on this platform "
            "(profiles/r6_two_streams.txt); use one stream, or one worker process per stream (rc_mvsnet_amd.sharding), or run the "
            "process with GPU_MAX_HW_QUEUES=1.")
    return ctypes.c_void_p(st.cuda_stream)


def _chk(t, name, dtype=torch.float32):
    if not t.is_cuda:
        raise _lib.RcmvsError(f"{name}: expected a tensor on the GPU (the HIP path has no CPU fallback)")
    if t.dtype != dtype:
        raise _lib.RcmvsError(f"{name}: expected {dtype}, got {t.dtype}")
    if not t.is_contiguous():
        raise _lib.RcmvsError(f"{name}: expected a contiguous tensor")
    return ctypes.c_void_p(t.data_ptr())


def _opt(t, name):
    return ctypes.c_void_p(0) if t is None else _chk(t, name)


def to_channels_last(x):
    N, C = x.shape[:2]
    S = x[0, 0].numel()
    out = torch.empty((N, *x.shape[2:], C), device=x.device, dtype=torch.float32)
    _lib.call("rcmvs_nchw_to_nhwc", _chk(x, "x"), _chk(out, "out"), N, C, S, _stream())
    return out


def to_channels_first(x):
    N, C = x.shape[0], x.shape[-1]
    S = x[0, ..., 0].numel()
    out = torch.empty((N, C, *x.shape[1:-1]), device=x.device, dtype=torch.float32)
    _lib.call("rcmvs_nhwc_to_nchw", _chk(x, "x"), _chk(out, "out"), N, C, S, _stream())
    return out


def compose_homography(proj):
    B, V = proj.shape[:2]
    rot = torch.empty((B, V - 1, 9), device=proj.device, dtype=torch.float32)
    trans = torch.empty((B, V - 1, 3), device=proj.device, dtype=torch.float32)
    _lib.call("rcmvs_compose_homography", _chk(proj, "proj"), _chk(rot, "rot"), _chk(trans, "trans"), B, V, _stream())
    return rot, trans


def compose_homography_stages(projs, zero=None):
    B, V = projs[0].shape[:2]
    n = len(projs)
    rot = torch.empty((n, B, V - 1, 9), device=projs[0].device, dtype=torch.float32)
    trans = torch.empty((n, B, V - 1, 3), device=projs[0].device, dtype=torch.float32)
    ptrs = [_chk(p, "proj") for p in projs] + [ctypes.c_void_p(0)] * (4 - n)
    _lib.call("rcmvs_compose_homography_stages", ptrs[0], ptrs[1], ptrs[2], ptrs[3], n, _chk(rot, "rot"), _chk(trans, "trans"), B, V,
              _opt(zero, "zero"), 0 if zero is None else zero.numel(), _stream())
    return rot, trans


def hypothesis_planes(prev_depth, depth_values, full_hw, scale, ndepth, ratio):
    B, ND = depth_values.shape
    H, W = full_hw
    planes = torch.empty((B, H // scale, W // scale, 2), device=depth_values.device, dtype=torch.float32)
    hp, wp = (prev_depth.shape[-2:] if prev_depth is not None else (0, 0))
    _lib.call("rcmvs_hypothesis_planes", _opt(prev_depth, "prev_depth"), _chk(depth_values, "depth_values"),
              _chk(planes, "planes"), B, hp, wp, H, W, scale, ndepth, float(ratio), ND,
              _stream())
    return planes


ABSMAX_FLOATS = _lib.CONSTANTS["RCMVS_ABSMAX_FLOATS"]


def absmax(x, square=False, out=None):
    if out is None:
        out = torch.zeros(ABSMAX_FLOATS, device=x.device, dtype=torch.float32)
    _lib.call("rcmvs_absmax_fwd", _chk(x, "x"), x.numel(), int(bool(square)), _chk(out, "absmax"), _stream())
    return out


def warp_variance(feats, rot, trans, planes, ndepth, variant=None, uniform_planes=False):
    B, V, h, w, C = feats.shape
    var = torch.empty((B, ndepth, h, w, C), device=feats.device, dtype=torch.float32)
    args = (_chk(feats, "feats"), _chk(rot, "rot"), _chk(trans, "trans"), _chk(planes, "planes"), _chk(var, "var"), B, V, C, ndepth, h, w)
    if variant is not None:
        _lib.call("rcmvs_debug_warp_variance_fwd", *args, int(variant), _stream())
        return var
    hint = K1_FAST_BLEND | (K1_UNIFORM_PLANES if uniform_planes else 0)
    if K1_EVENTS is not None:
        ev = (torch.cuda.Event(enable_timing=True), torch.cuda.Event(enable_timing=True))
        ev[0].record()
        ev[1].record()
        _lib.call("rcmvs_warp_variance_timed_fwd", *args, hint, ctypes.c_void_p(ev[0].cuda_event), ctypes.c_void_p(ev[1].cuda_event), _stream())
        K1_EVENTS.append(ev)
        return var
    _lib.call("rcmvs_warp_variance_hint_fwd", *args, hint, _stream())
    return var


def warp_variance_win(feats, rot, trans, planes, ndepth, variant=5):
    B, V, h, w, C = feats.shape
    var = torch.empty((B, ndepth, h, w, C), device=feats.device, dtype=torch.float32)
    stats = torch.zeros(2, device=feats.device, dtype=torch.int32)
    _lib.call("rcmvs_debug_warp_variance_win_fwd", _chk(feats, "feats"), _chk(rot, "rot"), _chk(trans, "trans"),
              _chk(planes, "planes"), _chk(var, "var"), B, V, C, ndepth, h, w, int(variant),
              _chk(stats, "stats", torch.int32), _stream())
    n = stats.cpu()
    return var, int(n[0]), int(n[1])


def warp_noref(feats, imgs, rot, trans, planes, ndepth, square_first):
    B, V, h, w, C = feats.shape
    out = torch.empty((B, 3 * (V - 1) + C, ndepth, h, w), device=feats.device, dtype=torch.float32)
    _lib.call("rcmvs_warp_noref_fwd", _chk(feats, "feats"), _chk(imgs, "imgs"), _chk(rot, "rot"), _chk(trans, "trans"),
              _chk(planes, "planes"), _chk(out, "out"), B, V, C, ndepth, h, w,
              int(bool(square_first)), _stream())
    return out


def warp_variance_bwd(feats, rot, trans, planes, grad_var, grad_noref=None, variant=0):
    B, V, h, w, C = feats.shape
    D = grad_var.shape[1]
    if tuple(grad_var.shape) != (B, D, h, w, C) or (grad_noref is not None and grad_noref.shape != grad_var.shape):
        raise _lib.RcmvsError(f"warp_variance_bwd: gradient shape {tuple(grad_var.shape)} does not match (B,D,h,w,C)")
    gf = torch.zeros_like(feats)
    args = (_chk(feats, "feats"), _chk(rot, "rot"), _chk(trans, "trans"), _chk(planes, "planes"), _chk(grad_var, "grad_var"),
            _opt(grad_noref, "grad_noref"), _chk(gf, "grad_feats"), B, V, C, D, h, w)
    if variant:
        _lib.call("rcmvs_debug_warp_variance_bwd", *args, int(variant), _stream())
    else:
        _lib.call("rcmvs_warp_variance_bwd", *args, _stream())
    return gf


class WarpVarianceFn(torch.autograd.Function):

    @staticmethod
    def forward(ctx, feats, rot, trans, planes, ndepth, imgs):
        feats = feats.contiguous()
        ctx.save_for_backward(feats, rot, trans, planes)
        ctx.ndepth = ndepth
        ctx.set_materialize_grads(False)
        var = warp_variance(feats, rot, trans, planes, ndepth)
        if imgs is None:
            return var
        noref = warp_noref(feats, imgs, rot, trans, planes, ndepth, square_first=False)
        return var, noref

    @staticmethod
    def backward(ctx, gvar, gnoref=None):
        feats, rot, trans, planes = ctx.saved_tensors
        C = feats.shape[-1]
        if gvar is None and gnoref is None:
            return None, None, None, None, None, None
        if gvar is None:
            gvar = torch.zeros((feats.shape[0], ctx.ndepth, *feats.shape[2:]), device=feats.device)
        gnr = None
        if gnoref is not None:
            gnr = gnoref[:, -C:].permute(0, 2, 3, 4, 1).contiguous()
        gf = warp_variance_bwd(feats, rot, trans, planes, gvar.contiguous(), gnr)
        return gf, None, None, None, None, None


IMG_ALL = 0x7fffffff


class PackedWeight:
    __slots__ = ("blob", "ci", "co", "k", "transposed", "images")

    def __init__(self, blob, ci, co, transposed=0, images=IMG_ALL):
        self.blob, self.ci, self.co, self.transposed, self.images = blob, ci, co, int(transposed), int(images)


_CONV_IMPL = 0


def force_direct_conv(on):
    global _CONV_IMPL
    _CONV_IMPL = int(on)


def _conv_event_start():
    ev = (torch.cuda.Event(enable_timing=True), torch.cuda.Event(enable_timing=True))
    ev[0].record()
    return ev


def _conv_event_stop(ev, *key):
    ev[1].record()
    CONV_EVENTS.append(ev + (key,))


def conv3d_images(ci, co, stride=1, transposed=False, planar=False):
    return int(_lib.load().rcmvs_conv3d_images(co, ci, int(stride), int(bool(transposed)), int(bool(planar))))


def pack_conv3d_weight(w, transposed=False, use=None):
    w = w.detach().contiguous().float()
    Ci, Co = (w.shape[0], w.shape[1]) if transposed else (w.shape[1], w.shape[0])
    n = _lib.load().rcmvs_packed_weight_floats(Co, Ci)
    blob = torch.empty((n,), device=w.device, dtype=torch.float32)
    images = IMG_ALL
    if use is not None and not _CONV_IMPL:
        images = conv3d_images(Ci, Co, stride=use[0], transposed=(int(transposed) == 1), planar=use[1])
    _lib.call("rcmvs_pack_conv3d_weight_sel", _chk(w, "w"), _chk(blob, "packed"), Co, Ci, int(transposed), images, _stream())
    return PackedWeight(blob, Ci, Co, int(transposed), images)


def _check_image(w_packed, ci, co, stride, transposed, planar, scaled, who):
    if w_packed.images == IMG_ALL:
        return
    if _CONV_IMPL or scaled or not (w_packed.images & conv3d_images(ci, co, stride, transposed, planar)):
        raise _lib.RcmvsError(f"{who}: the weight was packed for another call (pack_conv3d_weight(use=...)): the image this call reads was not written")


def conv3d(x, w_packed, scale=None, shift=None, residual=None, stride=1, relu=False, x_absmax=None, y_absmax=None, y_absmax_square=False):
    B, D, H, W, Ci = x.shape
    Co = w_packed.co
    if w_packed.ci != Ci:
        raise _lib.RcmvsError(f"conv3d: input has {Ci} channels, weight expects {w_packed.ci}")
    if w_packed.transposed == 1:
        raise _lib.RcmvsError("conv3d: the weight was packed as a ConvTranspose3d weight (transposed=1); its blob holds no conv images")
    _check_image(w_packed, Ci, Co, stride, False, D == 1, x_absmax is not None, "conv3d")
    y = torch.empty((B, (D - 1) // stride + 1, (H - 1) // stride + 1, (W - 1) // stride + 1, Co), device=x.device,
                    dtype=torch.float32)
    if residual is not None and residual.shape != y.shape:
        raise _lib.RcmvsError(f"conv3d: residual {tuple(residual.shape)} != output {tuple(y.shape)}")
    ev = _conv_event_start() if CONV_EVENTS is not None else None
    if x_absmax is not None or y_absmax is not None:
        name, xb, yb = "rcmvs_conv3d_scaled_fwd", (_opt(x_absmax, "x_absmax"),), (_opt(y_absmax, "y_absmax"),)
        impl = (_CONV_IMPL | ((1 << 24) if y_absmax_square else 0),)
    elif _CONV_IMPL:
        name, xb, yb, impl = "rcmvs_debug_conv3d_fwd", (), (), (_CONV_IMPL,)
    else:
        name, xb, yb, impl = "rcmvs_conv3d_fwd", (), (), ()
    _lib.call(name, _chk(x, "x"), *xb, _chk(w_packed.blob, "w"), _opt(scale, "scale"), _opt(shift, "shift"), _opt(residual, "residual"),
              _chk(y, "y"), *yb, B, D, H, W, Ci, Co, stride, int(relu), *impl, _stream())
    if ev is not None:
        _conv_event_stop(ev, "s1" if stride == 1 else "s2", B, D, H, W, Ci, Co)
    return y


def deconv3d(x, w_packed, scale=None, shift=None, residual=None, relu=False, x_absmax=None, y_absmax=None):
    B, D, H, W, Ci = x.shape
    Co = w_packed.co
    if w_packed.ci != Ci:
        raise _lib.RcmvsError(f"deconv3d: input has {Ci} channels, weight expects {w_packed.ci}")
    if w_packed.transposed != 1:
        raise _lib.RcmvsError("deconv3d: the weight was not packed with transposed=True; its blob holds no transposed-conv image")
    _check_image(w_packed, Ci, Co, 2, True, False, x_absmax is not None, "deconv3d")
    y = torch.empty((B, 2 * D, 2 * H, 2 * W, Co), device=x.device, dtype=torch.float32)
    if residual is not None and residual.shape != y.shape:
        raise _lib.RcmvsError(f"deconv3d: residual {tuple(residual.shape)} != output {tuple(y.shape)} "
                              "(volume sizes must be divisible by 8, as in the reference)")
    ev = _conv_event_start() if CONV_EVENTS is not None else None
    if x_absmax is not None or y_absmax is not None:
        name, xb, yb, impl = "rcmvs_deconv3d_scaled_fwd", (_opt(x_absmax, "x_absmax"),), (_opt(y_absmax, "y_absmax"),), (_CONV_IMPL,)
    elif _CONV_IMPL:
        name, xb, yb, impl = "rcmvs_debug_deconv3d_fwd", (), (), (_CONV_IMPL,)
    else:
        name, xb, yb, impl = "rcmvs_deconv3d_fwd", (), (), ()
    _lib.call(name, _chk(x, "x"), *xb, _chk(w_packed.blob, "w"), _opt(scale, "scale"), _opt(shift, "shift"), _opt(residual, "residual"),
              _chk(y, "y"), *yb, B, D, H, W, Ci, Co, int(relu), *impl, _stream())
    if ev is not None:
        _conv_event_stop(ev, "t2", B, D, H, W, Ci, Co)
    return y


def conv2d_s2d(x, w_packed, scale=None, shift=None, relu=False):
    N, H, W, C = x.shape
    Co = w_packed.co
    if w_packed.ci != 4 * C:
        raise _lib.RcmvsError(f"conv2d_s2d: input has {C} channels, the packed weight expects {w_packed.ci} = 4 x C")
    y = torch.empty((N, H // 2, W // 2, Co), device=x.device, dtype=torch.float32)
    _lib.call("rcmvs_conv2d_s2d_fwd", _chk(x, "x"), _chk(w_packed.blob, "w"), _opt(scale, "scale"), _opt(shift, "shift"),
              _chk(y, "y"), N, H, W, C, Co, int(relu), _stream())
    return y


def pack_conv2d_pair(wa, wb):
    if tuple(wa.shape) != (16, 16, 3, 3) or tuple(wb.shape) != (16, 16, 3, 3):
        raise _lib.RcmvsError("pack_conv2d_pair: built for two 16 -> 16 3x3 layers")
    lib = _lib.load()
    img = torch.empty(int(lib.rcmvs_conv2d_pair_weight_floats()), device=wa.device, dtype=torch.float32)
    _lib.call("rcmvs_pack_conv2d_pair", _chk(wa.detach().float().contiguous(), "wa"), _chk(wb.detach().float().contiguous(), "wb"), _chk(img, "image"), _stream())
    return img


def conv2d_pair(x, image, scale_a, shift_a, scale_b, shift_b):
    N, H, W, C = x.shape
    y = torch.empty_like(x)
    _lib.call("rcmvs_conv2d_pair_fwd", _chk(x, "x"), _chk(image, "image"), _chk(scale_a, "scale_a"), _chk(shift_a, "shift_a"),
              _chk(scale_b, "scale_b"), _chk(shift_b, "shift_b"), _chk(y, "y"), N, H, W, C, _stream())
    return y


def resize_rgb_cl(x, hw):
    N, C, H, W = x.shape
    if C != 3:
        raise _lib.RcmvsError("resize_rgb_cl: expects RGB images (N,3,H,W)")
    h, w = int(hw[0]), int(hw[1])
    y = torch.empty((N, h, w, 3), device=x.device, dtype=torch.float32)
    _lib.call("rcmvs_resize_rgb_cl", _chk(x, "x"), _chk(y, "y"), N, H, W, h, w, _stream())
    return y


def rgb_to_nhwc4(x):
    N, _, H, W = x.shape
    y = torch.empty((N, H, W, 4), device=x.device, dtype=torch.float32)
    _lib.call("rcmvs_rgb_to_nhwc4", _chk(x, "x"), _chk(y, "y"), N, H, W, _stream())
    return y


def pack_conv2d_weight(w, pad_in_to=None):
    w = w.detach().contiguous().float()
    Co, Ci, K, _ = w.shape
    Cip = Ci if pad_in_to is None else pad_in_to
    blob = torch.empty((K * K * Cip * Co,), device=w.device, dtype=torch.float32)
    _lib.call("rcmvs_pack_conv2d_weight", _chk(w, "w"), _chk(blob, "packed"), Co, Ci, Cip, K, _stream())
    pw = PackedWeight(blob, Cip, Co)
    pw.k = K
    return pw


def conv2d(x, w_packed, scale=None, shift=None, up_add=None, stride=1, relu=False):
    N, H, W, Ci = x.shape
    K, Co = w_packed.k, w_packed.co
    if w_packed.ci != Ci:
        raise _lib.RcmvsError(f"conv2d: input has {Ci} channels, weight expects {w_packed.ci}")
    Ho, Wo = (H + 2 * (K // 2) - K) // stride + 1, (W + 2 * (K // 2) - K) // stride + 1
    y = torch.empty((N, Ho, Wo, Co), device=x.device, dtype=torch.float32)
    if up_add is not None and tuple(up_add.shape) != (N, Ho // 2, Wo // 2, Co):
        raise _lib.RcmvsError(f"conv2d: up_add {tuple(up_add.shape)} does not match half of the output {tuple(y.shape)}")
    _lib.call("rcmvs_conv2d_fwd", _chk(x, "x"), _chk(w_packed.blob, "w"), _opt(scale, "scale"), _opt(shift, "shift"),
              _opt(up_add, "up_add"), _chk(y, "y"), N, H, W, Ci, Co, K, stride, int(relu), _stream())
    return y


def conv1x1(x, w_packed, scale=None, shift=None, up_add=None, relu=False, ysq_absmax=None, mfma=False):
    N, H, W, Ci = x.shape
    Co = w_packed.co
    if w_packed.ci != Ci or w_packed.k != 1:
        raise _lib.RcmvsError(f"conv1x1: input has {Ci} channels, weight is {w_packed.ci} -> {Co} with k={w_packed.k}")
    if up_add is not None and tuple(up_add.shape) != (N, H // 2, W // 2, Co):
        raise _lib.RcmvsError(f"conv1x1: up_add {tuple(up_add.shape)} does not match half of the output")
    y = torch.empty((N, H, W, Co), device=x.device, dtype=torch.float32)
    _lib.call("rcmvs_conv1x1_mfma_fwd" if mfma else "rcmvs_conv1x1_fwd", _chk(x, "x"), _chk(w_packed.blob, "w"), _opt(scale, "scale"), _opt(shift, "shift"),
              _opt(up_add, "up_add"), _chk(y, "y"), _opt(ysq_absmax, "ysq_absmax"), N, H, W, Ci, Co, int(relu), _stream())
    return y


def conv2d_rgb(x, w_packed, scale=None, shift=None, relu=False):
    N, C, H, W = x.shape
    if C != 3 or w_packed.ci != 4 or w_packed.co != 8 or w_packed.k != 3:
        raise _lib.RcmvsError(f"conv2d_rgb: expected a (N,3,H,W) input and a 3 -> 8 3x3 weight packed to 4 input channels (got {tuple(x.shape)}, {w_packed.ci} -> {w_packed.co}, k={w_packed.k})")
    y = torch.empty((N, H, W, 8), device=x.device, dtype=torch.float32)
    _lib.call("rcmvs_conv2d_fwd", _chk(x, "x"), _chk(w_packed.blob, "w"), _opt(scale, "scale"), _opt(shift, "shift"), None,
              _chk(y, "y"), N, H, W, 3, 8, 3, 1, int(relu), _stream())
    return y


def pack_conv2d_tile(w):
    Co = w.shape[0]
    if Co not in (16, 32) or tuple(w.shape) != (Co, 32, 3, 3):
        raise _lib.RcmvsError("pack_conv2d_tile: built for 32 -> 16 and 32 -> 32 3x3 layers")
    lib = _lib.load()
    img = torch.empty(int(lib.rcmvs_conv2d_tile_weight_floats(Co)), device=w.device, dtype=torch.float32)
    _lib.call("rcmvs_pack_conv2d_tile", _chk(w.detach().float().contiguous(), "w"), _chk(img, "image"), Co, _stream())
    return img


def conv2d_tile(x, image, scale=None, shift=None, relu=False, s2d=False, ysq_absmax=None):
    N, Hx, Wx, C = x.shape
    lib = _lib.load()
    Co = {int(lib.rcmvs_conv2d_tile_weight_floats(c)): c for c in (16, 32)}.get(image.numel())
    if Co is None or C != (8 if s2d else 32) or (s2d and (Hx % 2 or Wx % 2 or Co != 16)):
        raise _lib.RcmvsError(f"conv2d_tile: unexpected input {tuple(x.shape)} (s2d={s2d}) or image of {image.numel()} floats")
    H, W = (Hx // 2, Wx // 2) if s2d else (Hx, Wx)
    y = torch.empty((N, H, W, Co), device=x.device, dtype=torch.float32)
    _lib.call("rcmvs_conv2d_tile_fwd", _chk(x, "x"), _chk(image, "image"), _opt(scale, "scale"), _opt(shift, "shift"), _chk(y, "y"), N, H, W, Co, int(s2d), int(relu),
              _opt(ysq_absmax, "ysq_absmax"), _stream())
    return y


def pack_conv2d_stem(wb):
    if tuple(wb.shape) != (8, 8, 3, 3):
        raise _lib.RcmvsError("pack_conv2d_stem: built for an 8 -> 8 3x3 second layer")
    lib = _lib.load()
    img = torch.empty(int(lib.rcmvs_conv2d_stem_weight_floats()), device=wb.device, dtype=torch.float32)
    _lib.call("rcmvs_pack_conv2d_stem", _chk(wb.detach().float().contiguous(), "wb"), _chk(img, "image"), _stream())
    return img


def conv2d_stem(x, w_a_packed, scale_a, shift_a, image_b, scale_b, shift_b):
    N, C, H, W = x.shape
    if C != 3 or w_a_packed.ci != 4 or w_a_packed.co != 8 or w_a_packed.k != 3:
        raise _lib.RcmvsError(f"conv2d_stem: expected a (N,3,H,W) input and a 3 -> 8 3x3 weight packed to 4 input channels (got {tuple(x.shape)}, {w_a_packed.ci} -> {w_a_packed.co}, k={w_a_packed.k})")
    y = torch.empty((N, H, W, 8), device=x.device, dtype=torch.float32)
    _lib.call("rcmvs_conv2d_stem_fwd", _chk(x, "x"), _chk(w_a_packed.blob, "w_a"), _chk(scale_a, "scale_a"), _chk(shift_a, "shift_a"), _chk(image_b, "image_b"),
              _chk(scale_b, "scale_b"), _chk(shift_b, "shift_b"), _chk(y, "y"), N, H, W, _stream())
    return y


def fpn_out_fused(lat, up, w_inner_packed, b_inner, w_out_packed):
    N, H, W, CL = lat.shape
    CM, CO = w_inner_packed.co, w_out_packed.co
    if w_inner_packed.ci != CL or w_inner_packed.k != 1 or w_out_packed.ci != CM or w_out_packed.k != 3:
        raise _lib.RcmvsError("fpn_out_fused: expected a 1x1 lateral conv followed by a 3x3 output conv on matching channels")
    if tuple(up.shape) != (N, H // 2, W // 2, CM):
        raise _lib.RcmvsError(f"fpn_out_fused: up {tuple(up.shape)} does not match half of {tuple(lat.shape)} with {CM} channels")
    y = torch.empty((N, H, W, CO), device=lat.device, dtype=torch.float32)
    _lib.call("rcmvs_fpn_out_fused", _chk(lat, "lat"), _chk(up, "up"), _chk(w_inner_packed.blob, "w_inner"), _chk(b_inner, "b_inner"),
              _chk(w_out_packed.blob, "w_out"), _chk(y, "y"), N, H, W, CL, CM, CO, _stream())
    return y


FPN_FOLDED_FLOATS = _lib.CONSTANTS["RCMVS_FPN_FOLDED_FLOATS"]


def pack_fpn_folded(w_inner, b_inner, w_out):
    wi = w_inner.detach().double().reshape(32, 8)
    wo = w_out.detach().double()
    b = b_inner.detach().double()
    wb = torch.einsum("mi,omyx->yxio", wi, wo)
    bt = torch.einsum("m,omyx->yxo", b, wo)
    inside = {0: (1, 2), 1: (0, 1, 2), 2: (0, 1)}
    bs = torch.stack([torch.stack([sum(bt[ky, kx] for ky in inside[cy] for kx in inside[cx]) for cx in range(3)]) for cy in range(3)])
    rows = lambda p: ((0,), (1, 2)) if p == 0 else ((0, 1), (2,))
    wa = torch.zeros(2, 2, 2, 2, 32, 8, dtype=torch.float64, device=wo.device)
    for py in range(2):
        for px in range(2):
            for ry in range(2):
                for rx in range(2):
                    for ky in rows(py)[ry]:
                        for kx in rows(px)[rx]:
                            wa[py, px, ry, rx] += wo[:, :, ky, kx].t()
    tab = torch.cat((wb.reshape(-1), bs.reshape(-1), wa.reshape(-1))).float().contiguous()
    assert tab.numel() == FPN_FOLDED_FLOATS
    return tab


def pack_fpn_folded_mfma(tables):
    if tables.numel() != FPN_FOLDED_FLOATS:
        raise _lib.RcmvsError("pack_fpn_folded_mfma: expects the tables of pack_fpn_folded")
    img = torch.empty((_lib.load().rcmvs_fpn_folded_mfma_floats(),), device=tables.device, dtype=torch.float32)
    _lib.call("rcmvs_fpn_folded_mfma_pack", _chk(tables, "tables"), _chk(img, "image"), _stream())
    return img


def fpn_out_folded(lat, up, tables, ysq_absmax=None):
    N, H, W, CL = lat.shape
    mfma = tables.numel() == _lib.load().rcmvs_fpn_folded_mfma_floats()
    if CL != 8 or tuple(up.shape) != (N, H // 2, W // 2, 32) or not (mfma or tables.numel() == FPN_FOLDED_FLOATS):
        raise _lib.RcmvsError(f"fpn_out_folded: lat {tuple(lat.shape)} / up {tuple(up.shape)} / {tables.numel()} table floats do not fit 8 -> 32 -> 8")
    y = torch.empty((N, H, W, 8), device=lat.device, dtype=torch.float32)
    _lib.call("rcmvs_fpn_out_folded_mfma" if mfma else "rcmvs_fpn_out_folded", _chk(lat, "lat"), _chk(up, "up"), _chk(tables, "tables"), _chk(y, "y"),
              _opt(ysq_absmax, "ysq_absmax"), N, H, W, _stream())
    return y


DEPTH_HEAD_IMPL = 0


def depth_head(x8, w_prob_packed, planes, want_prob=False, x_absmax=None):
    B, D, h, w, C = x8.shape
    if C != 8:
        raise _lib.RcmvsError("depth_head: the prob conv takes 8 channels")
    if x_absmax is not None and w_prob_packed.images != IMG_ALL:
        raise _lib.RcmvsError("depth_head: the fp16-pair form reads an image that a selectively packed weight does not hold")
    depth = torch.empty((B, h, w), device=x8.device, dtype=torch.float32)
    conf = torch.empty((B, h, w), device=x8.device, dtype=torch.float32)
    one_launch = D == 8 and not (DEPTH_HEAD_IMPL & 1)
    prob = None if one_launch and not want_prob else torch.empty((B, D, h, w), device=x8.device, dtype=torch.float32)
    _lib.call("rcmvs_depth_head_scaled_fwd", _chk(x8, "x8"), _opt(x_absmax, "x_absmax"), _chk(w_prob_packed.blob, "w_prob"), _chk(planes, "planes"),
              _chk(depth, "depth"), _chk(conf, "conf"), _opt(prob, "prob"), B, D, h, w,
              DEPTH_HEAD_IMPL | (0 if want_prob else 8), _stream())
    return (depth, conf, prob) if want_prob else (depth, conf)


def conv11_prob(t, t_absmax, w11_packed, scale, shift, res, res_absmax, coef, w_prob_packed, zchunk=0, planes=None):
    B, Dt, Ht, Wt, C = t.shape
    if C != 16 or tuple(res.shape) != (B, 2 * Dt, 2 * Ht, 2 * Wt, 8):
        raise _lib.RcmvsError(f"conv11_prob: t {tuple(t.shape)} / res {tuple(res.shape)} are not (B,Dt,Ht,Wt,16) / (B,2Dt,2Ht,2Wt,8)")
    if w11_packed.images != IMG_ALL or w_prob_packed.images != IMG_ALL:
        raise _lib.RcmvsError("conv11_prob: needs the full weight blobs (a selectively packed weight does not hold the fp16-pair images)")
    fused = planes is not None and Dt == 4
    logits = depth = conf = None
    if fused:
        depth = torch.empty((B, 2 * Ht, 2 * Wt), device=t.device, dtype=torch.float32)
        conf = torch.empty((B, 2 * Ht, 2 * Wt), device=t.device, dtype=torch.float32)
    else:
        logits = torch.empty((B, 2 * Dt, 2 * Ht, 2 * Wt), device=t.device, dtype=torch.float32)
    _lib.call("rcmvs_conv11_prob_fwd", _chk(t, "t"), _chk(t_absmax, "t_absmax"), _chk(w11_packed.blob, "w11"), _chk(scale, "scale"),
              _chk(shift, "shift"), _chk(res, "res"), _chk(res_absmax, "res_absmax"), _chk(coef, "coef"),
              _chk(w_prob_packed.blob, "w_prob"), _opt(logits, "logits"), _opt(planes if fused else None, "planes"),
              _opt(depth, "depth"), _opt(conf, "conf"), B, Dt, Ht, Wt, int(zchunk), _stream())
    if fused:
        return depth, conf
    if planes is not None:
        return softmax_head(logits, planes)
    return logits


def softmax_head(logits, planes, keep_prob=False):
    B, D, h, w = logits.shape
    depth = torch.empty((B, h, w), device=logits.device, dtype=torch.float32)
    conf = torch.empty((B, h, w), device=logits.device, dtype=torch.float32)
    _lib.call("rcmvs_softmax_head_fwd", _chk(logits, "logits"), _chk(planes, "planes"), _chk(depth, "depth"), _chk(conf, "conf"),
              B, D, h, w, int(bool(keep_prob)), _stream())
    return depth, conf


def resize_planes(x, out_planes, pad_channels_to=None):
    B, C, D, h, w = x.shape
    Cp = C if pad_channels_to is None else pad_channels_to
    y = torch.empty((B, out_planes, h, w, Cp), device=x.device, dtype=torch.float32)
    _lib.call("rcmvs_resize_planes_fwd", _chk(x, "x"), _chk(y, "y"), B, C, Cp, D, out_planes, h, w, _stream())
    return y


def gu_sample(pseudo_depth, img0, pix, eps, u, cam):
    H, W = pseudo_depth.shape
    N, S = eps.shape
    dev = eps.device
    f = lambda *shape: torch.empty(shape, device=dev, dtype=torch.float32)
    z, pts, ndc, dirs, rdepth, target = f(N, S), f(N, S, 3), f(N, S, 3), f(N, 3), f(N), f(N, 3)
    _lib.call("rcmvs_gu_sample_fwd", _chk(pseudo_depth, "pseudo_depth"), _chk(img0, "img0"), _chk(pix, "pix", torch.int32),
              _chk(eps, "eps"), _chk(u, "u"), _chk(cam, "cam"), _chk(z, "z"), _chk(pts, "pts"),
              _chk(ndc, "ndc"), _chk(dirs, "dirs"), _chk(rdepth, "rays_depth"), _chk(target, "target"),
              N, S, H, W, _stream())
    return z, pts, ndc, dirs, rdepth, target


def point_feats(volume_cl, imgs, poses, pts, ndc, ldf=32):
    Dv, hv, wv, C = volume_cl.shape
    if C != 8:
        raise _lib.RcmvsError("point_feats: the neural volume has 8 channels")
    nimg, _, H, W = imgs.shape
    M = pts.shape[0] * pts.shape[1]
    feat = torch.empty((M, ldf), device=pts.device, dtype=torch.float32)
    _lib.call("rcmvs_point_feats_fwd", _chk(volume_cl, "volume"), _chk(imgs, "imgs"), _chk(poses, "poses"), _chk(pts, "pts"),
              _chk(ndc, "ndc"), _chk(feat, "feat"), M, Dv, hv, wv, nimg, H, W, ldf, _stream())
    return feat


NERF_ORDER = ("pts_bias", "pts_linears.0", "pts_linears.1", "pts_linears.2", "pts_linears.3", "pts_linears.4", "pts_linears.5",
              "alpha_linear", "feature_linear", "views_linears.0", "rgb_linear")


def pack_nerf_weights(named):
    lib = _lib.load()
    tensors = []
    for n in NERF_ORDER:
        w, b = named[n]
        tensors += [w.detach().contiguous().float(), b.detach().contiguous().float()]
    arr = (ctypes.c_void_p * 22)(*[_chk(t, "nerf weight").value for t in tensors])
    blob = torch.empty((lib.rcmvs_nerf_weight_floats(),), device=tensors[0].device, dtype=torch.float32)
    _lib.call("rcmvs_pack_nerf_weights", arr, _chk(blob, "blob"), _stream())
    return blob


def nerf_mlp(ndc, feat, dirs, w2c_ref, blob):
    lib = _lib.load()
    N, S = ndc.shape[:2]
    M = N * S
    ws = torch.empty((lib.rcmvs_nerf_workspace_floats(M),), device=ndc.device, dtype=torch.float32)
    raw = torch.empty((N, S, 4), device=ndc.device, dtype=torch.float32)
    _lib.call("rcmvs_nerf_mlp_fwd", _chk(ndc, "ndc"), _chk(feat, "feat"), feat.shape[1], _chk(dirs, "dirs"), _chk(w2c_ref, "w2c_ref"),
              _chk(blob, "weights"), _chk(ws, "workspace"), _chk(raw, "raw"), N, S, _stream())
    return raw


def nerf_mlp_embedded(x, blob):
    lib = _lib.load()
    M, ldx = x.shape
    if ldx != 86:
        raise _lib.RcmvsError(f"nerf_mlp_embedded: rows of 63 + 20 + 3 = 86 columns expected (got {ldx})")
    ws = torch.empty((lib.rcmvs_nerf_workspace_floats(M),), device=x.device, dtype=torch.float32)
    feat = torch.empty((M, 32), device=x.device, dtype=torch.float32)
    raw = torch.empty((M, 4), device=x.device, dtype=torch.float32)
    _lib.call("rcmvs_nerf_mlp_embedded_fwd", _chk(x, "x"), ldx, _chk(blob, "weights"), _chk(ws, "workspace"), _chk(feat, "feat"), _chk(raw, "raw"), M, _stream())
    return raw


def composite(raw, z):
    N, S = z.shape
    dev = z.device
    rgb = torch.empty((N, 3), device=dev, dtype=torch.float32)
    depth = torch.empty((N,), device=dev, dtype=torch.float32)
    weights = torch.empty((N, S), device=dev, dtype=torch.float32)
    alpha = torch.empty((N, S), device=dev, dtype=torch.float32)
    _lib.call("rcmvs_composite_fwd", _chk(raw, "raw"), _chk(z, "z"), _chk(rgb, "rgb"), _chk(depth, "depth"),
              _chk(weights, "weights"), _chk(alpha, "alpha"), N, S, _stream())
    return rgb, depth, weights, alpha
```

Baseline: 1006 ref-scenes/s.

## Fuse hypothesis-plane computation into the warp-variance kernels

Adds a fused entry point where the warp-variance kernels compute each pixel's depth hypothesis plane (d0, delta) directly from the previous-stage depth and depth range, instead of reading a table written by a separate planes kernel. One depth-block per tile publishes the planes to an output buffer for later consumers. This removes one kernel launch and the planes round-trip through memory per stage. In exchange, every depth block recomputes the bilinear upsampling per pixel, which adds arithmetic and scattered loads inside the hot kernel. The fused path is on by default and can be disabled with an environment variable.

```diff
diff --git a/rc_mvsnet_amd/_lib.py b/rc_mvsnet_amd/_lib.py
--- a/rc_mvsnet_amd/_lib.py
+++ b/rc_mvsnet_amd/_lib.py
@@ -11,7 +11,7 @@
 EXT_HEADERS = (os.path.join(CSRC, "pc_register.h"), os.path.join(CSRC, "view_select.h"), os.path.join(CSRC, "undistort.h"),
                os.path.join(CSRC, "tsdf_mesh.h"), os.path.join(CSRC, "tsdf_sparse.h"), os.path.join(CSRC, "mesh_clean.h"),
                os.path.join(CSRC, "mesh_decimate.h"), os.path.join(CSRC, "mesh_holes.h"),
-               os.path.join(CSRC, "mesh_render.h"))
+               os.path.join(CSRC, "mesh_render.h"), os.path.join(CSRC, "k1_planes.h"))
 
 _lib = None
 
diff --git a/rc_mvsnet_amd/casmvsnet.py b/rc_mvsnet_amd/casmvsnet.py
--- a/rc_mvsnet_amd/casmvsnet.py
+++ b/rc_mvsnet_amd/casmvsnet.py
@@ -681,6 +681,7 @@
         pair = getattr(self, "fp16_pair", None)
         if pair is None:
             pair = FP16_PAIR_DEFAULT if os.environ.get("RCMVS_FP16_PAIR") is None else os.environ["RCMVS_FP16_PAIR"] == "1"
+        k1_planes = os.environ.get("RCMVS_K1_PLANES", "1") != "0"
         if pair and B == 1:
             bounds = getattr(self, "_pair_bounds", None)
             if getattr(self, "_is_replica", False):
@@ -715,8 +716,12 @@
                 rot, trans = homographies[key]
             else:
                 rot, trans = rots[s], transs[s]
-            planes = ops.hypothesis_planes(depth, depth_values, (H, W), scale, D, self.depth_interals_ratio[s])
-            var = ops.warp_variance(f_cl, rot, trans, planes, D, uniform_planes=depth is None)
+            if k1_planes:
+                var, planes = ops.warp_variance_planes(f_cl, rot, trans, depth, depth_values, (H, W), scale, D, self.depth_interals_ratio[s],
+                                                       uniform_planes=depth is None)
+            else:
+                planes = ops.hypothesis_planes(depth, depth_values, (H, W), scale, D, self.depth_interals_ratio[s])
+                var = ops.warp_variance(f_cl, rot, trans, planes, D, uniform_planes=depth is None)
             cr = self._cr(s)
             vmax = None
             if bounds is not None:
diff --git a/rc_mvsnet_amd/csrc/geometry.hip b/rc_mvsnet_amd/csrc/geometry.hip
--- a/rc_mvsnet_amd/csrc/geometry.hip
+++ b/rc_mvsnet_amd/csrc/geometry.hip
@@ -1,4 +1,5 @@
 #include "common.h"
+#include "planes_math.h"
 
 namespace rcmvs {
 
@@ -124,72 +125,15 @@
     }
 }
 
-__device__ static inline float ld_agent(const float* p) {
-#if defined(__AMDGCN__)
-    return __hip_atomic_load(p, __ATOMIC_RELAXED, __HIP_MEMORY_SCOPE_AGENT);
-#else
-    return *p;
-#endif
-}
-
-__device__ static inline float bilinear_up(const float* __restrict__ p, int hp, int wp, float sh, float sw, int Y, int X) {
-#pragma clang fp contract(off)
-    float sy = sh * ((float)Y + 0.5f) - 0.5f;
-    float sx = sw * ((float)X + 0.5f) - 0.5f;
-    sy = sy < 0.f ? 0.f : sy;
-    sx = sx < 0.f ? 0.f : sx;
-    int y0 = (int)sy, x0 = (int)sx;
-    y0 = y0 > hp - 1 ? hp - 1 : y0;
-    x0 = x0 > wp - 1 ? wp - 1 : x0;
-    int y1 = y0 + 1 > hp - 1 ? hp - 1 : y0 + 1;
-    int x1 = x0 + 1 > wp - 1 ? wp - 1 : x0 + 1;
-    float ly1 = sy - (float)y0, lx1 = sx - (float)x0;
-    float ly0 = 1.0f - ly1, lx0 = 1.0f - lx1;
-    float top = lx0 * ld_agent(p + y0 * wp + x0) + lx1 * ld_agent(p + y0 * wp + x1);
-    float bot = lx0 * ld_agent(p + y1 * wp + x0) + lx1 * ld_agent(p + y1 * wp + x1);
-    return ly0 * top + ly1 * bot;
-}
-
 __global__ __launch_bounds__(256) void planes_kernel(const float* __restrict__ prev, const float* __restrict__ dv,
                                                       float* __restrict__ planes, int hp, int wp, int H, int W,
                                                       int scale, int D, float ratio, int ND) {
-#pragma clang fp contract(off)
     const int h = H / scale, w = W / scale;
     const int b = blockIdx.y;
     int t = blockIdx.x * blockDim.x + threadIdx.x;
     if (t >= h * w) return;
     int y = t / w, x = t % w;
-    float d0, delta;
-    if (prev == nullptr) {
-        float lo = dv[(long long)b * ND], hi = dv[(long long)b * ND + ND - 1];
-        d0 = lo;
-        delta = (hi - lo) / (float)(D - 1);
-    } else {
-        double itv = ((double)dv[ND - 1] - (double)dv[0]) / (double)ND;
-        float half = (float)((double)D / 2.0 * ((double)ratio * itv));
-        const float* p = prev + (long long)b * hp * wp;
-        float sh = (float)hp / (float)H, sw = (float)wp / (float)W;
-        float fd = (float)(D - 1);
-        if (scale == 1) {
-            float c = bilinear_up(p, hp, wp, sh, sw, y, x);
-            float cmin = c - half, cmax = c + half;
-            d0 = cmin;
-            delta = (cmax - cmin) / fd;
-        } else {
-            int Y0 = y * scale + scale / 2 - 1, X0 = x * scale + scale / 2 - 1;
-            float mn[2][2], it[2][2];
-            for (int j = 0; j < 2; ++j)
-                for (int i = 0; i < 2; ++i) {
-                    float c = bilinear_up(p, hp, wp, sh, sw, Y0 + j, X0 + i);
-                    float cmin = c - half, cmax = c + half;
-                    mn[j][i] = cmin;
-                    it[j][i] = (cmax - cmin) / fd;
-                }
-            d0 = 0.5f * (0.5f * mn[0][0] + 0.5f * mn[0][1]) + 0.5f * (0.5f * mn[1][0] + 0.5f * mn[1][1]);
-            delta = 0.5f * (0.5f * it[0][0] + 0.5f * it[0][1]) + 0.5f * (0.5f * it[1][0] + 0.5f * it[1][1]);
-        }
-    }
-    float2 o = make_float2(d0, delta);
+    float2 o = hypothesis_plane(prev, dv, hp, wp, H, W, scale, D, ratio, ND, b, y, x);
     reinterpret_cast<float2*>(planes)[(long long)b * h * w + t] = o;
 }
 
diff --git a/rc_mvsnet_amd/csrc/k1_planes.h b/rc_mvsnet_amd/csrc/k1_planes.h
--- /dev/null
+++ b/rc_mvsnet_amd/csrc/k1_planes.h
@@ -0,0 +1,19 @@
+#ifndef RCMVS_K1_PLANES_H
+#define RCMVS_K1_PLANES_H
+#ifdef __cplusplus
+extern "C" {
+#endif
+
+int rcmvs_warp_variance_planes_fwd(const float* feats, const float* rot, const float* trans, const float* prev_depth,
+                                   const float* depth_values, float* planes_out, float* var,
+                                   int B, int V, int C, int D, int h, int w, int hp, int wp, int H, int W, int scale,
+                                   float ratio, int ND, int hint, void* stream);
+int rcmvs_warp_variance_planes_timed_fwd(const float* feats, const float* rot, const float* trans, const float* prev_depth,
+                                         const float* depth_values, float* planes_out, float* var,
+                                         int B, int V, int C, int D, int h, int w, int hp, int wp, int H, int W, int scale,
+                                         float ratio, int ND, int hint, void* start_event, void* stop_event, void* stream);
+
+#ifdef __cplusplus
+}
+#endif
+#endif
diff --git a/rc_mvsnet_amd/csrc/k1_pp.h b/rc_mvsnet_amd/csrc/k1_pp.h
--- a/rc_mvsnet_amd/csrc/k1_pp.h
+++ b/rc_mvsnet_amd/csrc/k1_pp.h
@@ -1,12 +1,13 @@
 #pragma once
 #include "k1_taps.h"
+#include "planes_math.h"
 
 namespace rcmvs {
 
 template <int C, int DKB, int NVT, int NG = (NVT <= 4 ? NVT : 3)>
 __global__ __launch_bounds__(256) void warp_variance_pp_kernel(
     const float* __restrict__ feats, const float* __restrict__ rot, const float* __restrict__ trans,
-    const float* __restrict__ planes, float* __restrict__ var, int V, int D, int h, int w, int tiles_x) {
+    const PlaneSrc ps, float* __restrict__ var, int V, int D, int h, int w, int tiles_x) {
     constexpr int LPP = C / 4, PIX = 256 / LPP, TH = 4, TW = PIX / TH, TEXB = C * 4;
     constexpr int CPP = PIX * NVT;
     constexpr int NCH = (CPP + 255) / 256;
@@ -31,7 +32,7 @@
     const float* trb = trans + (long long)b * (V - 1) * 3;
     const int pa = threadIdx.x % PIX;
     const int xa = min(tx0 + pa % TW, w - 1), ya = min(ty0 + pa / TW, h - 1);
-    const float2 pla = reinterpret_cast<const float2*>(planes)[(long long)b * hw + ya * w + xa];
+    float2 pla;
     const int grp = threadIdx.x / CPP;
     float rx[NCH], ry[NCH], rz[NCH], t0[NCH], t1[NCH], t2[NCH];
     {
@@ -79,6 +80,8 @@
     float* ob = var + (((long long)b * D + k0) * hw + (long long)min(y, h - 1) * w + min(x, w - 1)) * C + (q4b >> 2);
     const int pitch = w * TEXB;
 
+    pla = plane_fetch(ps, b, ya, xa, hw, w);
+    plane_publish(ps, blockIdx.y == 0 && threadIdx.x < PIX && tx0 + pa % TW < w && ty0 + pa / TW < h, b, ya, xa, hw, w, pla);
     records(0, 0);
     __syncthreads();
 #pragma unroll
@@ -122,12 +125,12 @@
 }
 
 template <int C, int DKB, int NVT>
-static int k1_pp_launch_one(const float* feats, const float* rot, const float* trans, const float* planes, float* var,
+static int k1_pp_launch_one(const float* feats, const float* rot, const float* trans, const PlaneSrc& ps, float* var,
                             int B, int V, int D, int h, int w, hipStream_t st, hipEvent_t ev0 = nullptr, hipEvent_t ev1 = nullptr) {
     constexpr int PIX = 256 / (C / 4), TW = PIX / 4;
     const int txp = (w + TW - 1) / TW, typ = (h + 3) / 4;
     dim3 grid(txp * typ, (D + DKB - 1) / DKB, B);
-    RCMVS_LAUNCH_TIMED((warp_variance_pp_kernel<C, DKB, NVT>), grid, dim3(256), 0, st, ev0, ev1, feats, rot, trans, planes, var, V, D, h, w, txp);
+    RCMVS_LAUNCH_TIMED((warp_variance_pp_kernel<C, DKB, NVT>), grid, dim3(256), 0, st, ev0, ev1, feats, rot, trans, ps, var, V, D, h, w, txp);
     return launch_status("warp_variance_fwd (plane-pipelined form)");
 }
 
diff --git a/rc_mvsnet_amd/csrc/k1_win.h b/rc_mvsnet_amd/csrc/k1_win.h
--- a/rc_mvsnet_amd/csrc/k1_win.h
+++ b/rc_mvsnet_amd/csrc/k1_win.h
@@ -1,6 +1,7 @@
 #pragma once
 #include <atomic>
 #include "k1_taps.h"
+#include "planes_math.h"
 
 namespace rcmvs {
 
@@ -31,7 +32,7 @@
 template <int C, int DKB, int NVT, int WP, int WR, int MODE>
 __global__ __launch_bounds__(256) void warp_variance_win_kernel(
     const float* __restrict__ feats, const float* __restrict__ rot, const float* __restrict__ trans,
-    const float* __restrict__ planes, float* __restrict__ var, int V, int D, int h, int w, int tiles_x, unsigned* __restrict__ stats) {
+    const PlaneSrc ps, float* __restrict__ var, int V, int D, int h, int w, int tiles_x, unsigned* __restrict__ stats) {
     using W = K1Win<C, DKB, NVT, WP, WR>;
     constexpr int LPP = W::LPP, PIX = W::PIX, TH = W::TH, TW = W::TW, TEXB = W::TEXB;
     extern __shared__ __attribute__((aligned(16))) char lds[];
@@ -59,7 +60,6 @@
 
     const int pa = threadIdx.x % PIX;
     const int xa = min(tx0 + pa % TW, w - 1), ya = min(ty0 + pa / TW, h - 1);
-    const float2 pla = reinterpret_cast<const float2*>(planes)[(long long)b * hw + ya * w + xa];
     const int p = threadIdx.x / LPP;
     const int q4b = (threadIdx.x % LPP) * 16;
     const int x = tx0 + p % TW, y = ty0 + p / TW;
@@ -72,8 +72,9 @@
     const int pitch = w * TEXB;
     const int xcen = min(tx0 + TW / 2, w - 1), ycen = min(ty0 + TH / 2, h - 1);
     const float fxc = (float)xcen, fyc = (float)ycen, fxa = (float)xa, fya = (float)ya;
-    float2 plc = make_float2(0.f, 0.f);
-    plc = reinterpret_cast<const float2*>(planes)[(long long)b * hw + ycen * w + xcen];
+    const float2 pla = plane_fetch(ps, b, ya, xa, hw, w);
+    plane_publish(ps, blockIdx.y == 0 && threadIdx.x < PIX && tx0 + pa % TW < w && ty0 + pa / TW < h, b, ya, xa, hw, w, pla);
+    const float2 plc = plane_fetch(ps, b, ycen, xcen, hw, w);
 
     struct Taps { v4f t[NVT][4]; v4f w[NVT]; };
 
@@ -232,7 +233,7 @@
 }
 
 template <int C, int DKB, int NVT, int WP, int WR, int MODE>
-static int k1_win_launch_one(const float* feats, const float* rot, const float* trans, const float* planes, float* var,
+static int k1_win_launch_one(const float* feats, const float* rot, const float* trans, const PlaneSrc& ps, float* var,
                              int B, int V, int D, int h, int w, unsigned* stats, hipStream_t st, hipEvent_t ev0 = nullptr, hipEvent_t ev1 = nullptr) {
     using W = K1Win<C, DKB, NVT, WP, WR>;
     const int txp = (w + W::TW - 1) / W::TW, typ = (h + W::TH - 1) / W::TH;
@@ -249,7 +250,7 @@
             raised[dev].store(true, std::memory_order_release);
         }
     }
-    RCMVS_LAUNCH_TIMED(kern, grid, dim3(256), lds, st, ev0, ev1, feats, rot, trans, planes, var, V, D, h, w, txp, stats);
+    RCMVS_LAUNCH_TIMED(kern, grid, dim3(256), lds, st, ev0, ev1, feats, rot, trans, ps, var, V, D, h, w, txp, stats);
     return launch_status("warp_variance_fwd (window form)");
 }
 
diff --git a/rc_mvsnet_amd/csrc/planes_math.h b/rc_mvsnet_amd/csrc/planes_math.h
--- /dev/null
+++ b/rc_mvsnet_amd/csrc/planes_math.h
@@ -0,0 +1,98 @@
+#pragma once
+#include "common.h"
+
+namespace rcmvs {
+
+__device__ __forceinline__ float ld_agent(const float* p) {
+#if defined(__AMDGCN__)
+    return __hip_atomic_load(p, __ATOMIC_RELAXED, __HIP_MEMORY_SCOPE_AGENT);
+#else
+    return *p;
+#endif
+}
+
+__device__ __forceinline__ float bilinear_up(const float* __restrict__ p, int hp, int wp, float sh, float sw, int Y, int X) {
+#pragma clang fp contract(off)
+    float sy = sh * ((float)Y + 0.5f) - 0.5f;
+    float sx = sw * ((float)X + 0.5f) - 0.5f;
+    sy = sy < 0.f ? 0.f : sy;
+    sx = sx < 0.f ? 0.f : sx;
+    int y0 = (int)sy, x0 = (int)sx;
+    y0 = y0 > hp - 1 ? hp - 1 : y0;
+    x0 = x0 > wp - 1 ? wp - 1 : x0;
+    int y1 = y0 + 1 > hp - 1 ? hp - 1 : y0 + 1;
+    int x1 = x0 + 1 > wp - 1 ? wp - 1 : x0 + 1;
+    float ly1 = sy - (float)y0, lx1 = sx - (float)x0;
+    float ly0 = 1.0f - ly1, lx0 = 1.0f - lx1;
+    float top = lx0 * ld_agent(p + y0 * wp + x0) + lx1 * ld_agent(p + y0 * wp + x1);
+    float bot = lx0 * ld_agent(p + y1 * wp + x0) + lx1 * ld_agent(p + y1 * wp + x1);
+    return ly0 * top + ly1 * bot;
+}
+
+__device__ __forceinline__ float2 hypothesis_plane(const float* __restrict__ prev, const float* __restrict__ dv, int hp, int wp, int H, int W,
+                                                   int scale, int D, float ratio, int ND, int b, int y, int x) {
+#pragma clang fp contract(off)
+    float d0, delta;
+    if (prev == nullptr) {
+        float lo = dv[(long long)b * ND], hi = dv[(long long)b * ND + ND - 1];
+        d0 = lo;
+        delta = (hi - lo) / (float)(D - 1);
+    } else {
+        const float dv_last = dv[ND - 1], dv_first = dv[0];
+        const float* p = prev + (long long)b * hp * wp;
+        float sh = (float)hp / (float)H, sw = (float)wp / (float)W;
+        int Y0 = y * scale + scale / 2 - 1, X0 = x * scale + scale / 2 - 1;
+        float c[2][2];
+        if (scale == 1) {
+            c[0][0] = bilinear_up(p, hp, wp, sh, sw, y, x);
+        } else {
+            for (int j = 0; j < 2; ++j)
+                for (int i = 0; i < 2; ++i) c[j][i] = bilinear_up(p, hp, wp, sh, sw, Y0 + j, X0 + i);
+        }
+        double itv = ((double)dv_last - (double)dv_first) / (double)ND;
+        float half = (float)((double)D / 2.0 * ((double)ratio * itv));
+        float fd = (float)(D - 1);
+        if (scale == 1) {
+            float cmin = c[0][0] - half, cmax = c[0][0] + half;
+            d0 = cmin;
+            delta = (cmax - cmin) / fd;
+        } else {
+            float mn[2][2], it[2][2];
+            for (int j = 0; j < 2; ++j)
+                for (int i = 0; i < 2; ++i) {
+                    float cmin = c[j][i] - half, cmax = c[j][i] + half;
+                    mn[j][i] = cmin;
+                    it[j][i] = (cmax - cmin) / fd;
+                }
+            d0 = 0.5f * (0.5f * mn[0][0] + 0.5f * mn[0][1]) + 0.5f * (0.5f * mn[1][0] + 0.5f * mn[1][1]);
+            delta = 0.5f * (0.5f * it[0][0] + 0.5f * it[0][1]) + 0.5f * (0.5f * it[1][0] + 0.5f * it[1][1]);
+        }
+    }
+    return make_float2(d0, delta);
+}
+
+struct PlaneSrc {
+    const float* table;
+    const float* prev;
+    const float* dv;
+    float* out;
+    int hp, wp, H, W, scale, D, ND;
+    float ratio;
+};
+
+static inline PlaneSrc plane_table(const float* table) {
+    PlaneSrc s{};
+    s.table = table;
+    return s;
+}
+
+__device__ __forceinline__ float2 plane_fetch(const PlaneSrc& s, int b, int y, int x, int hw, int w) {
+    if (s.table) return reinterpret_cast<const float2*>(s.table)[(long long)b * hw + y * w + x];
+    return hypothesis_plane(s.prev, s.dv, s.hp, s.wp, s.H, s.W, s.scale, s.D, s.ratio, s.ND, b, y, x);
+}
+
+__device__ __forceinline__ void plane_publish(const PlaneSrc& s, bool owner, int b, int y, int x, int hw, int w, float2 pl) {
+    if (!s.table && owner) reinterpret_cast<float2*>(s.out)[(long long)b * hw + y * w + x] = pl;
+}
+
+}
diff --git a/rc_mvsnet_amd/csrc/warp_variance.hip b/rc_mvsnet_amd/csrc/warp_variance.hip
--- a/rc_mvsnet_amd/csrc/warp_variance.hip
+++ b/rc_mvsnet_amd/csrc/warp_variance.hip
@@ -1,6 +1,7 @@
 #include <type_traits>
 #include "common.h"
 #include "k1_taps.h"
+#include "planes_math.h"
 #include "k1_win.h"
 #include "k1_pp.h"
 
@@ -186,13 +187,11 @@
 };
 
 template <int C, int DKB>
-__device__ __forceinline__ void k1_phase_a(const float* __restrict__ rot, const float* __restrict__ trans, int b, int V, int view, int slot,
-                                           float fxa, float fya, float2 pla, int k0, int hw, const K1Geom& g, v4i* lds_o, v4f* lds_w) {
+__device__ __forceinline__ void k1_phase_a_rt(const float* r, const float* t, int view, int slot,
+                                              float fxa, float fya, float2 pla, int k0, int hw, const K1Geom& g, v4i* lds_o, v4f* lds_w) {
 #pragma clang fp contract(off)
     constexpr int PIX = K1Tile<C>::PIX, GRP = K1Tile<C>::GRP, KPT = DKB / GRP;
     const int pa = threadIdx.x % PIX, ga = threadIdx.x / PIX;
-    const float* r = rot + ((long long)b * (V - 1) + (view - 1)) * 9;
-    const float* t = trans + ((long long)b * (V - 1) + (view - 1)) * 3;
     const float rx = (r[0] * fxa + r[1] * fya) + r[2];
     const float ry = (r[3] * fxa + r[4] * fya) + r[5];
     const float rz = (r[6] * fxa + r[7] * fya) + r[8];
@@ -211,10 +210,17 @@
     }
 }
 
+template <int C, int DKB>
+__device__ __forceinline__ void k1_phase_a(const float* __restrict__ rot, const float* __restrict__ trans, int b, int V, int view, int slot,
+                                           float fxa, float fya, float2 pla, int k0, int hw, const K1Geom& g, v4i* lds_o, v4f* lds_w) {
+    k1_phase_a_rt<C, DKB>(rot + ((long long)b * (V - 1) + (view - 1)) * 9, trans + ((long long)b * (V - 1) + (view - 1)) * 3, view, slot,
+                          fxa, fya, pla, k0, hw, g, lds_o, lds_w);
+}
+
 template <int C, int DKB, bool FAST, int NVT, int NG = (NVT > 4 ? 3 : NVT)>
 __global__ __launch_bounds__(256) void warp_variance_tp_kernel(
     const float* __restrict__ feats, const float* __restrict__ rot, const float* __restrict__ trans,
-    const float* __restrict__ planes, float* __restrict__ var, int V, int D, int h, int w, int tiles_x) {
+    const PlaneSrc ps, float* __restrict__ var, int V, int D, int h, int w, int tiles_x) {
 #pragma clang fp contract(off)
     constexpr int LPP = K1Tile<C>::LPP, PIX = K1Tile<C>::PIX, TH = K1Tile<C>::TH, TW = K1Tile<C>::TW, GRP = K1Tile<C>::GRP;
     static_assert(NVT > 0 && DKB % GRP == 0, "DKB must be a multiple of 256/PIX");
@@ -243,9 +249,27 @@
     {
         const int pa = threadIdx.x % PIX;
         const int xa = min(tx0 + pa % TW, w - 1), ya = min(ty0 + pa / TW, h - 1);
-        const float2 pla = reinterpret_cast<const float2*>(planes)[(long long)b * hw + ya * w + xa];
-        for (int va = 0; va < NVT; ++va)
-            k1_phase_a<C, DKB>(rot, trans, b, V, 1 + va, va, (float)xa, (float)ya, pla, k0, hw, g, lds_o, lds_w);
+        constexpr int NPRE = NVT <= 4 ? NVT : 1;
+        float rr[NPRE][9], tt[NPRE][3];
+        if (NVT <= 4) {
+#pragma unroll
+            for (int va = 0; va < NPRE; ++va) {
+#pragma unroll
+                for (int i = 0; i < 9; ++i) rr[va][i] = rot[((long long)b * (V - 1) + va) * 9 + i];
+#pragma unroll
+                for (int i = 0; i < 3; ++i) tt[va][i] = trans[((long long)b * (V - 1) + va) * 3 + i];
+            }
+        }
+        const float2 pla = plane_fetch(ps, b, ya, xa, hw, w);
+        plane_publish(ps, blockIdx.y == 0 && threadIdx.x < PIX && tx0 + pa % TW < w && ty0 + pa / TW < h, b, ya, xa, hw, w, pla);
+        if (NVT <= 4) {
+#pragma unroll
+            for (int va = 0; va < NPRE; ++va)
+                k1_phase_a_rt<C, DKB>(rr[va], tt[va], 1 + va, va, (float)xa, (float)ya, pla, k0, hw, g, lds_o, lds_w);
+        } else {
+            for (int va = 0; va < NVT; ++va)
+                k1_phase_a<C, DKB>(rot, trans, b, V, 1 + va, va, (float)xa, (float)ya, pla, k0, hw, g, lds_o, lds_w);
+        }
     }
     __syncthreads();
     if (!inside) return;
@@ -274,7 +298,7 @@
 template <int C, int DKB, bool FAST>
 __global__ __launch_bounds__(256) void warp_variance_mv_kernel(
     const float* __restrict__ feats, const float* __restrict__ rot, const float* __restrict__ trans,
-    const float* __restrict__ planes, float* __restrict__ var, int V, int D, int h, int w, int tiles_x, int VC) {
+    const PlaneSrc ps, float* __restrict__ var, int V, int D, int h, int w, int tiles_x, int VC) {
 #pragma clang fp contract(off)
     constexpr int LPP = K1Tile<C>::LPP, PIX = K1Tile<C>::PIX, TH = K1Tile<C>::TH, TW = K1Tile<C>::TW, GRP = K1Tile<C>::GRP;
     static_assert(DKB % GRP == 0, "DKB must be a multiple of 256/PIX");
@@ -302,7 +326,8 @@
     float* ob = var + (((long long)b * D) * hw + (long long)y * w + x) * C + (q4b >> 2);
     const int pa = threadIdx.x % PIX;
     const int xa = min(tx0 + pa % TW, w - 1), ya = min(ty0 + pa / TW, h - 1);
-    const float2 pla = reinterpret_cast<const float2*>(planes)[(long long)b * hw + ya * w + xa];
+    const float2 pla = plane_fetch(ps, b, ya, xa, hw, w);
+    plane_publish(ps, blockIdx.y == 0 && threadIdx.x < PIX && tx0 + pa % TW < w && ty0 + pa / TW < h, b, ya, xa, hw, w, pla);
     v4f s[DKB], sq[DKB];
 #pragma unroll
     for (int k = 0; k < DKB; ++k) { s[k] = ref; sq[k] = ref * ref; }
@@ -401,10 +426,12 @@
 
 extern "C" {
 
-static int k1_launch(const float* feats, const float* rot, const float* trans, const float* planes, float* var,
+static int k1_launch(const float* feats, const float* rot, const float* trans, const PlaneSrc& ps, float* var,
                      int B, int V, int C, int D, int h, int w, int variant, hipStream_t st, unsigned* stats = nullptr,
                      hipEvent_t ev0 = nullptr, hipEvent_t ev1 = nullptr) {
-    RCMVS_REQUIRE(feats && rot && trans && planes && var, "warp_variance_fwd: null pointer");
+    RCMVS_REQUIRE(feats && rot && trans && var && (ps.table || (ps.dv && ps.out)), "warp_variance_fwd: null pointer");
+    RCMVS_REQUIRE(ps.table || variant <= 1 || variant >= 5, "warp_variance_fwd: variant %d reads a plane table", variant);
+    const float* planes = ps.table;
     RCMVS_REQUIRE(B > 0 && D > 0 && h > 1 && w > 1, "warp_variance_fwd: bad sizes B=%d D=%d h=%d w=%d", B, D, h, w);
     RCMVS_REQUIRE(V >= 2 && V - 1 <= RCMVS_MAX_SRC_VIEWS, "warp_variance_fwd: V=%d unsupported", V);
     RCMVS_REQUIRE((long long)h * w * C < (1LL << 31), "warp_variance_fwd: feature map too large for 32-bit offsets");
@@ -415,9 +442,9 @@
         RCMVS_REQUIRE(nsrc == 2 || nsrc == 3 || nsrc == 4 || nsrc == 6, "warp_variance_fwd: the plane-pipelined form is built for 2, 3, 4 or 6 source views (got V=%d)", V);
         RCMVS_REQUIRE((long long)V * h * w * C * 4 < 0x7fffffffLL, "warp_variance_fwd: feature block too large for 32-bit offsets");
 #define RCMVS_K1PP(NN) do { \
-            if (C == 32) return k1_pp_launch_one<32, 8, NN>(feats, rot, trans, planes, var, B, V, D, h, w, st, ev0, ev1); \
-            if (C == 16) return k1_pp_launch_one<16, 8, NN>(feats, rot, trans, planes, var, B, V, D, h, w, st, ev0, ev1); \
-            return k1_pp_launch_one<8, 8, NN>(feats, rot, trans, planes, var, B, V, D, h, w, st, ev0, ev1); } while (0)
+            if (C == 32) return k1_pp_launch_one<32, 8, NN>(feats, rot, trans, ps, var, B, V, D, h, w, st, ev0, ev1); \
+            if (C == 16) return k1_pp_launch_one<16, 8, NN>(feats, rot, trans, ps, var, B, V, D, h, w, st, ev0, ev1); \
+            return k1_pp_launch_one<8, 8, NN>(feats, rot, trans, ps, var, B, V, D, h, w, st, ev0, ev1); } while (0)
         if (nsrc == 2) RCMVS_K1PP(2);
         if (nsrc == 3) RCMVS_K1PP(3);
         if (nsrc == 4) RCMVS_K1PP(4);
@@ -427,8 +454,8 @@
     if (variant >= 5) {
         RCMVS_REQUIRE(V == 3, "warp_variance_fwd: the window form is built for two source views (got V=%d)", V);
         RCMVS_REQUIRE((long long)V * h * w * C * 4 < 0x7fffffffLL, "warp_variance_fwd: feature block too large for 32-bit offsets");
-#define RCMVS_K1WIN(CC, DD, PP, RR) (variant == 5 ? k1_win_launch_one<CC, DD, 2, PP, RR, 1>(feats, rot, trans, planes, var, B, V, D, h, w, stats, st, ev0, ev1) : \
-                                                    k1_win_launch_one<CC, DD, 2, PP, RR, 2>(feats, rot, trans, planes, var, B, V, D, h, w, stats, st, ev0, ev1))
+#define RCMVS_K1WIN(CC, DD, PP, RR) (variant == 5 ? k1_win_launch_one<CC, DD, 2, PP, RR, 1>(feats, rot, trans, ps, var, B, V, D, h, w, stats, st, ev0, ev1) : \
+                                                    k1_win_launch_one<CC, DD, 2, PP, RR, 2>(feats, rot, trans, ps, var, B, V, D, h, w, stats, st, ev0, ev1))
         if (C == 32) return RCMVS_K1WIN(32, 4, 16, 8);
         if (C == 16) return RCMVS_K1WIN(16, 4, 32, 8);
         return RCMVS_K1WIN(8, 4, 64, 8);
@@ -448,8 +475,8 @@
         const int txp = (w + TWp - 1) / TWp, typ = (h + 3) / 4;
         RCMVS_REQUIRE((long long)V * h * w * C * 4 < 0x7fffffffLL, "warp_variance_fwd: feature block too large for 32-bit offsets");
         dim3 gridp(txp * typ, (D + dkb - 1) / dkb, B);
-#define RCMVS_K1TP(CC, DD, FF, NN) RCMVS_LAUNCH_TIMED((warp_variance_tp_kernel<CC, DD, FF, NN>), gridp, dim3(256), lds, st, ev0, ev1, feats, rot, trans, planes, var, V, D, h, w, txp)
-#define RCMVS_K1MV(CC, DD, FF) RCMVS_LAUNCH_TIMED((warp_variance_mv_kernel<CC, DD, FF>), gridp, dim3(256), lds, st, ev0, ev1, feats, rot, trans, planes, var, V, D, h, w, txp, VC)
+#define RCMVS_K1TP(CC, DD, FF, NN) RCMVS_LAUNCH_TIMED((warp_variance_tp_kernel<CC, DD, FF, NN>), gridp, dim3(256), lds, st, ev0, ev1, feats, rot, trans, ps, var, V, D, h, w, txp)
+#define RCMVS_K1MV(CC, DD, FF) RCMVS_LAUNCH_TIMED((warp_variance_mv_kernel<CC, DD, FF>), gridp, dim3(256), lds, st, ev0, ev1, feats, rot, trans, ps, var, V, D, h, w, txp, VC)
 #define RCMVS_K1TP_N(CC, DD, FF) do { if (nvt == 2) RCMVS_K1TP(CC, DD, FF, 2); else if (nvt == 4) RCMVS_K1TP(CC, DD, FF, 4); else RCMVS_K1MV(CC, DD, FF); } while (0)
 #define RCMVS_K1TP_F(CC, DD) do { if (fastm) RCMVS_K1TP_N(CC, DD, true); else RCMVS_K1TP_N(CC, DD, false); } while (0)
 #define RCMVS_K1TP_6(CC, DD) do { if (fastm) RCMVS_K1TP(CC, DD, true, 6); else RCMVS_K1TP(CC, DD, false, 6); } while (0)
@@ -500,33 +527,64 @@
 int rcmvs_warp_variance_fwd(const float* feats, const float* rot, const float* trans,
                             const float* planes, float* var,
                             int B, int V, int C, int D, int h, int w, void* stream) {
-    return k1_launch(feats, rot, trans, planes, var, B, V, C, D, h, w, 0, as_stream(stream));
+    return k1_launch(feats, rot, trans, plane_table(planes), var, B, V, C, D, h, w, 0, as_stream(stream));
 }
 
 int rcmvs_warp_variance_hint_fwd(const float* feats, const float* rot, const float* trans,
                                  const float* planes, float* var,
                                  int B, int V, int C, int D, int h, int w, int hint, void* stream) {
-    return k1_launch(feats, rot, trans, planes, var, B, V, C, D, h, w, k1_production_variant(V, C, h, w, hint), as_stream(stream));
+    return k1_launch(feats, rot, trans, plane_table(planes), var, B, V, C, D, h, w, k1_production_variant(V, C, h, w, hint), as_stream(stream));
 }
 
 int rcmvs_warp_variance_timed_fwd(const float* feats, const float* rot, const float* trans,
                                   const float* planes, float* var,
                                   int B, int V, int C, int D, int h, int w, int hint, void* start_event, void* stop_event, void* stream) {
-    return k1_launch(feats, rot, trans, planes, var, B, V, C, D, h, w, k1_production_variant(V, C, h, w, hint), as_stream(stream), nullptr,
+    return k1_launch(feats, rot, trans, plane_table(planes), var, B, V, C, D, h, w, k1_production_variant(V, C, h, w, hint), as_stream(stream), nullptr,
                      reinterpret_cast<hipEvent_t>(start_event), reinterpret_cast<hipEvent_t>(stop_event));
+}
+
+static int k1_planes_launch(const float* feats, const float* rot, const float* trans, const float* prev_depth, const float* depth_values,
+                            float* planes_out, float* var, int B, int V, int C, int D, int h, int w, int hp, int wp, int H, int W,
+                            int scale, float ratio, int ND, int hint, hipEvent_t ev0, hipEvent_t ev1, void* stream) {
+    RCMVS_REQUIRE(depth_values && planes_out, "warp_variance_planes_fwd: null pointer");
+    RCMVS_REQUIRE(B > 0 && H > 0 && W > 0 && D >= 2 && ND >= 2, "warp_variance_planes_fwd: bad sizes");
+    RCMVS_REQUIRE(scale == 1 || scale == 2 || scale == 4, "warp_variance_planes_fwd: scale must be 1, 2 or 4 (got %d)", scale);
+    RCMVS_REQUIRE(H % scale == 0 && W % scale == 0, "warp_variance_planes_fwd: H,W must be multiples of scale");
+    RCMVS_REQUIRE(prev_depth == nullptr || (hp > 0 && wp > 0), "warp_variance_planes_fwd: prev_depth needs hp,wp");
+    RCMVS_REQUIRE(h == H / scale && w == W / scale, "warp_variance_planes_fwd: the feature maps are %d x %d, the stage map is %d x %d", h, w, H / scale, W / scale);
+    PlaneSrc ps{};
+    ps.prev = prev_depth; ps.dv = depth_values; ps.out = planes_out;
+    ps.hp = hp; ps.wp = wp; ps.H = H; ps.W = W; ps.scale = scale; ps.D = D; ps.ND = ND; ps.ratio = ratio;
+    return k1_launch(feats, rot, trans, ps, var, B, V, C, D, h, w, k1_production_variant(V, C, h, w, hint), as_stream(stream), nullptr, ev0, ev1);
+}
+
+int rcmvs_warp_variance_planes_fwd(const float* feats, const float* rot, const float* trans, const float* prev_depth,
+                                   const float* depth_values, float* planes_out, float* var,
+                                   int B, int V, int C, int D, int h, int w, int hp, int wp, int H, int W, int scale,
+                                   float ratio, int ND, int hint, void* stream) {
+    return k1_planes_launch(feats, rot, trans, prev_depth, depth_values, planes_out, var, B, V, C, D, h, w, hp, wp, H, W, scale, ratio, ND,
+                            hint, nullptr, nullptr, stream);
+}
+
+int rcmvs_warp_variance_planes_timed_fwd(const float* feats, const float* rot, const float* trans, const float* prev_depth,
+                                         const float* depth_values, float* planes_out, float* var,
+                                         int B, int V, int C, int D, int h, int w, int hp, int wp, int H, int W, int scale,
+                                         float ratio, int ND, int hint, void* start_event, void* stop_event, void* stream) {
+    return k1_planes_launch(feats, rot, trans, prev_depth, depth_values, planes_out, var, B, V, C, D, h, w, hp, wp, H, W, scale, ratio, ND,
+                            hint, reinterpret_cast<hipEvent_t>(start_event), reinterpret_cast<hipEvent_t>(stop_event), stream);
 }
 
 int rcmvs_debug_warp_variance_fwd(const float* feats, const float* rot, const float* trans,
                                   const float* planes, float* var,
                                   int B, int V, int C, int D, int h, int w, int variant, void* stream) {
-    return k1_launch(feats, rot, trans, planes, var, B, V, C, D, h, w, variant, as_stream(stream));
+    return k1_launch(feats, rot, trans, plane_table(planes), var, B, V, C, D, h, w, variant, as_stream(stream));
 }
 
 int rcmvs_debug_warp_variance_win_fwd(const float* feats, const float* rot, const float* trans,
                                       const float* planes, float* var,
                                       int B, int V, int C, int D, int h, int w, int variant, unsigned* stats, void* stream) {
     RCMVS_REQUIRE(variant == 5 || variant == 6, "debug_warp_variance_win_fwd: variant must be 5 or 6 (got %d)", variant);
-    return k1_launch(feats, rot, trans, planes, var, B, V, C, D, h, w, variant, as_stream(stream), stats);
+    return k1_launch(feats, rot, trans, plane_table(planes), var, B, V, C, D, h, w, variant, as_stream(stream), stats);
 }
 
 int rcmvs_warp_noref_fwd(const float* feats, const float* imgs, const float* rot, const float* trans,
diff --git a/rc_mvsnet_amd/ops.py b/rc_mvsnet_amd/ops.py
--- a/rc_mvsnet_amd/ops.py
+++ b/rc_mvsnet_amd/ops.py
@@ -118,6 +118,34 @@
         return var
     _lib.call("rcmvs_warp_variance_hint_fwd", *args, hint, _stream())
     return var
+
+
+def warp_variance_planes(feats, rot, trans, prev_depth, depth_values, full_hw, scale, ndepth, ratio, uniform_planes=False):
+    B, V, h, w, C = feats.shape
+    H, W = full_hw
+    ND = depth_values.shape[1]
+    if tuple(depth_values.shape) != (B, ND) or (h, w) != (H // scale, W // scale):
+        raise _lib.RcmvsError(f"warp_variance_planes: feats {tuple(feats.shape)} / depth_values {tuple(depth_values.shape)} do not match "
+                              f"B={B}, the ({H // scale}, {W // scale}) stage map")
+    hp, wp = 0, 0
+    if prev_depth is not None:
+        hp, wp = prev_depth.shape[-2:]
+        if prev_depth.numel() != B * hp * wp:
+            raise _lib.RcmvsError(f"warp_variance_planes: prev_depth {tuple(prev_depth.shape)} is not (B, hp, wp) with B={B}")
+    var = torch.empty((B, ndepth, h, w, C), device=feats.device, dtype=torch.float32)
+    planes = torch.empty((B, h, w, 2), device=feats.device, dtype=torch.float32)
+    hint = K1_FAST_BLEND | (K1_UNIFORM_PLANES if uniform_planes else 0)
+    args = (_chk(feats, "feats"), _chk(rot, "rot"), _chk(trans, "trans"), _opt(prev_depth, "prev_depth"), _chk(depth_values, "depth_values"),
+            _chk(planes, "planes"), _chk(var, "var"), B, V, C, ndepth, h, w, hp, wp, H, W, scale, ctypes.c_float(ratio), ND, hint)
+    if K1_EVENTS is not None:
+        ev = (torch.cuda.Event(enable_timing=True), torch.cuda.Event(enable_timing=True))
+        ev[0].record()
+        ev[1].record()
+        _lib.call("rcmvs_warp_variance_planes_timed_fwd", *args, ctypes.c_void_p(ev[0].cuda_event), ctypes.c_void_p(ev[1].cuda_event), _stream())
+        K1_EVENTS.append(ev)
+        return var, planes
+    _lib.call("rcmvs_warp_variance_planes_fwd", *args, _stream())
+    return var, planes
 
 
 def warp_variance_win(feats, rot, trans, planes, ndepth, variant=5):
```

After: 1006 ref-scenes/s. About the same (-0.1%).
